# CaptainEven/DenseBox

Measured on AMD Instinct MI355X. Metric: training patches/sec (240x240), higher is better.
Workload: dtype f16; 1 GPU; full training step (fwd + fused dense loss w/ hard-negative mining + bwd + grad all-reduce + SGD) of DenseBoxLMLOC on 240x240 patches; net=DenseBoxLMLOC, batch_per_gpu=64, global_batch=64, patch=240x240, parallelism=dp1, half_neg=11, grad_finite=True

## Files before the change

densebox_amd/_lib.py:

```python
import ctypes as C
import os

_HERE = os.path.dirname(os.path.abspath(__file__))
LIB_PATH = os.environ.get('DBX_LIB') or os.path.join(_HERE, 'csrc', 'libdensebox_hip.so')

F16, BF16, F32 = 0, 1, 2
DTYPE_ID = {'f16': F16, 'bf16': BF16, 'f32': F32}
ESIZE = {F16: 2, BF16: 2, F32: 4}

EPI_BIAS, EPI_RELU, EPI_GATE, EPI_DROPMASK, EPI_ACCUM, EPI_F32_NCHW, EPI_DROPHASH = 1, 2, 4, 8, 16, 32, 64
CONV_WFRAG = 128
K_IGEMM, K_DMA, K_BAND, K_C64, K_C8, K_WS, K_P8 = 1, 2, 3, 4, 5, 6, 7


class View(C.Structure):
    _fields_ = [('ptr', C.c_void_p), ('n', C.c_int32), ('h', C.c_int32), ('w', C.c_int32),
                ('pad', C.c_int32), ('ld', C.c_int32), ('c_off', C.c_int32), ('c', C.c_int32)]


class ConvDesc(C.Structure):
    _fields_ = [('dtype', C.c_int32), ('kh', C.c_int32), ('kw', C.c_int32), ('cpad', C.c_int32),
                ('cin_pad', C.c_int32), ('cout_pad', C.c_int32), ('epilogue', C.c_int32), ('drop_seed', C.c_uint32)]


# ... 32 lines not shown

class Track(C.Structure):
    _fields_ = [('box', C.c_double * 4), ('vel', C.c_double * 4), ('score', C.c_double), ('best_score', C.c_double), ('id', C.c_int32),
                ('hits', C.c_int32), ('age', C.c_int32), ('first_frame', C.c_int32), ('last_frame', C.c_int32), ('best_frame', C.c_int32)]


class TrackRecord(C.Structure):
    _fields_ = [('stream', C.c_int32), ('reserved', C.c_int32), ('t', Track)]


class Shot(C.Structure):
    _fields_ = [('key', C.c_double), ('score', C.c_double), ('sharpness', C.c_int64), ('id', C.c_int32), ('frame', C.c_int32),
                ('shots', C.c_int32), ('reserved', C.c_int32)]


class ShotRecord(C.Structure):
    _fields_ = [('stream', C.c_int32), ('slot', C.c_int32), ('shot', Shot)]


class OverlayFrame(C.Structure):
    _fields_ = [('src', C.c_void_p), ('dst', C.c_void_p), ('h', C.c_int32), ('w', C.c_int32)]


class OverlayStyle(C.Structure):
    _fields_ = [('box_color', C.c_uint8 * 4), ('text_color', C.c_uint8 * 4), ('mark_color', C.c_uint8 * 4), ('thickness', C.c_int32),
                ('radius', C.c_int32), ('font_scale', C.c_int32), ('inset_scale', C.c_int32)]


class ResizeJob(C.Structure):
    _fields_ = [('src', C.c_void_p), ('sh', C.c_int32), ('sw', C.c_int32), ('cx0', C.c_int32), ('cy0', C.c_int32),
                ('cw', C.c_int32), ('ch', C.c_int32), ('pad_l', C.c_int32), ('pad_t', C.c_int32), ('pad_r', C.c_int32),
                ('pad_b', C.c_int32), ('pad_value', C.c_int32), ('dh', C.c_int32), ('dw', C.c_int32), ('dst_off', C.c_int64)]


class PatchJob(C.Structure):
    _fields_ = [('src', C.c_void_p), ('dst', C.c_void_p), ('scale_x', C.c_double), ('scale_y', C.c_double), ('row_bytes', C.c_int32),
                ('cx0', C.c_int32), ('cy0', C.c_int32), ('cw', C.c_int32), ('ch', C.c_int32), ('pad_l', C.c_int32), ('pad_t', C.c_int32),
                ('vw', C.c_int32), ('vh', C.c_int32), ('dh', C.c_int32), ('dw', C.c_int32), ('pad_value', C.c_int32),
                ('tiles_x', C.c_int32), ('frame', C.c_int32), ('kind', C.c_int32), ('reserved', C.c_int32)]


class PatchGeom(C.Structure):
    _fields_ = [('status', C.c_int32), ('x0', C.c_int32), ('y0', C.c_int32), ('x1', C.c_int32), ('y1', C.c_int32),
                ('labels', C.c_int32 * 12), ('reserved', C.c_int32)]


class PatchPlanIO(C.Structure):
    _fields_ = [(k, C.c_void_p) for k in (
        'frames', 'plates', 'plate0', 'cand', 'draws', 'state', 'jobs', 'labels', 'bbox', 'vertices', 'label', 'count', 'tally',
        'status', 'slot', 'cand_out', 'draws_out')]


class PatchAug(C.Structure):
    _fields_ = [('flags', C.c_int32), ('blur', C.c_int32), ('box_len', C.c_int32), ('sat', C.c_int32), ('contrast', C.c_int32),
                ('brightness', C.c_int32), ('curve', C.c_int32), ('noise_amp', C.c_int32), ('key_lo', C.c_int32), ('key_hi', C.c_int32),
                ('gain', C.c_int32 * 3), ('reserved', C.c_int32 * 3)]


class PatchAugCfg(C.Structure):
    _fields_ = [('p_flip', C.c_double), ('p_blur', C.c_double), ('p_curve', C.c_double), ('p_noise', C.c_double), ('kind_w', C.c_int32 * 3),
                ('box_lo', C.c_int32), ('box_hi', C.c_int32), ('sat_lo', C.c_int32), ('sat_hi', C.c_int32), ('contrast_lo', C.c_int32),
                ('contrast_hi', C.c_int32), ('brightness_lo', C.c_int32), ('brightness_hi', C.c_int32), ('gain_lo', C.c_int32),
                ('gain_hi', C.c_int32), ('noise_lo', C.c_int32), ('noise_hi', C.c_int32), ('curve_lo', C.c_int32), ('curve_hi', C.c_int32),
                ('G', C.c_int32), ('reserved', C.c_int32 * 2)]


class PatchAugIO(C.Structure):
    _fields_ = [(k, C.c_void_p) for k in ('labels_in', 'count', 'params_in', 'state', 'params', 'labels', 'bbox', 'vertices', 'label')]


class MergeXform(C.Structure):
    _fields_ = [('scale', C.c_double), ('off_x', C.c_double), ('off_y', C.c_double)]


_VP, _I32, _I64, _F, _D = C.c_void_p, C.c_int32, C.c_int64, C.c_float, C.c_double
_PV, _PC = C.POINTER(View), C.POINTER(ConvDesc)

SIGNATURES = {
    'dbx_last_error': (C.c_char_p, []),
    'dbx_version': (C.c_int, []),
    'dbx_device_arch': (C.c_int, [C.c_int]),
    'dbx_conv_packed_elems': (_I64, [_PC]),
    'dbx_conv_forward': (C.c_int, [_PC, _PV, _VP, _VP, _PV, _PV, _VP, _I32, _VP]),
    'dbx_conv_plan': (C.c_int, [_PC, _PV, _PV, C.POINTER(ConvPlan)]),
    'dbx_conv_forward_split': (C.c_int, [_PC, _PV, _VP, _VP, _PV, _PV, _PV, _PV, _I32, _I32, _VP]),
    'dbx_heads_forward_fusable': (C.c_int, [_PC, _PV, _PV, C.POINTER(C.c_int32), _I32]),
    'dbx_heads_forward_fused_scratch_bytes': (_I64, [_I32, _I64]),
    'dbx_heads_forward_fused': (C.c_int, [_PC, _PV, _VP, _VP, _PV, _VP, _VP, C.POINTER(C.c_int32), _I32, _VP, _VP, _VP]),
    'dbx_heads_forward_fused_heads': (C.c_int, [_PC, _PV, _VP, _VP, _PV, _VP, _VP, C.POINTER(C.c_int32), _I32, C.POINTER(C.c_void_p), _VP, _VP]),
    'dbx_dp_unique_id': (C.c_int, [_VP]),
    'dbx_dp_init': (C.c_int, [_VP, _I32, _I32, C.POINTER(C.c_void_p)]),
    'dbx_dp_allreduce_sum_f32': (C.c_int, [_VP, _VP, _I64, _VP]),
    'dbx_dp_destroy': (C.c_int, [_VP]),
    'dbx_conv_dgrad_wgrad1_scratch_bytes': (_I64, []),
    'dbx_conv_dgrad_wgrad1_fusable': (C.c_int, [_PC, _PV, _PV, _PV]),
    'dbx_conv_dgrad_wgrad1': (C.c_int, [_PC, _PV, _VP, _PV, _PV, _I32, _VP, _VP, _VP, _I32, _VP]),
    'dbx_conv_pool_fusable': (C.c_int, [_PC, _PV, _PV]),
    'dbx_conv_forward_pool': (C.c_int, [_PC, _PV, _VP, _VP, _PV, _PV, _I32, _VP]),
    'dbx_conv_forward_pool_idx': (C.c_int, [_PC, _PV, _VP, _VP, _PV, _PV, _I32, _VP, _VP]),
    'dbx_pack_weight': (C.c_int, [_I32, _I32, _VP, _I32, _I32, _I32, _I32, _VP, _I32, _I32, _I32, _I32, _VP]),
    'dbx_fold_heads': (C.c_int, [_VP, _VP, _VP, _VP, _I32, _VP, _VP, _VP]),
    'dbx_fold_refine': (C.c_int, [_VP, _VP, _VP, _VP, _VP, _VP, _I32, _I32, _VP, _VP, _VP, _VP]),
    'dbx_refine_eval': (C.c_int, [_VP, _VP, _I32, _I32, _I32, _VP, _VP, _VP, _VP]),
    'dbx_refine_backward_scratch_bytes': (C.c_int64, [_I32, _I32, _I32]),
    'dbx_refine_backward': (C.c_int, [_VP, _VP, _VP, _I32, _I32, _I32, _VP, _VP, _VP, _VP, _VP, _VP, _I32, _VP, _VP, _VP, _VP, _VP, _VP, _VP, _VP, _VP, _VP, _VP, _VP, _VP, _VP]),
    'dbx_upsample_bilinear_nchw_f32': (C.c_int, [_VP, _I32, _I32, _I32, _VP, _I32, _I32, _VP]),
    'dbx_pack_multi': (C.c_int, [_I32, _VP, _I32, _I64, _VP]),
    'dbx_sgd_pack_step': (C.c_int, [_I32, _VP, _I32, _I64, _VP, _F, _F, _F, _I32, _VP]),
    'dbx_head2_dgrad': (C.c_int, [_I32, _PV, C.POINTER(C.c_void_p), C.POINTER(C.c_int32), _I32, _PV, _VP, _I32, _I32, C.c_uint32, _VP]),
    'dbx_head2_wgrad_scratch_bytes': (_I64, [_I32, _I32]),
    'dbx_head2_wgrad': (C.c_int, [_I32, _PV, _PV, C.POINTER(C.c_int32), _I32, C.POINTER(C.c_void_p), C.POINTER(C.c_void_p), _VP, _VP]),
    'dbx_head2_backward': (C.c_int, [_I32, _PV, _PV, C.POINTER(C.c_void_p), C.POINTER(C.c_int32), _I32, _PV, _VP, _I32, _I32, C.c_uint32,
                                     C.POINTER(C.c_void_p), C.POINTER(C.c_void_p), _VP, _VP]),
    'dbx_head2_backward_up': (C.c_int, [_I32, _PV, _PV, C.POINTER(C.c_void_p), C.POINTER(C.c_int32), _I32, _PV, _VP, _I32, _I32, C.c_uint32,
                                        C.POINTER(C.c_void_p), C.POINTER(C.c_void_p), _VP, _PV, _VP]),
    'dbx_perspective_matrix': (C.c_int, [_VP, _VP, _VP]),
    'dbx_warp_perspective_u8': (C.c_int, [_VP, _I32, _I32, _I32, _VP, _VP, _I32, _I32, _VP]),
    'dbx_warp_batch_workspace_bytes': (_I64, [_I32]),
    'dbx_warp_perspective_batch_u8': (C.c_int, [C.POINTER(WarpJob), _I32, _I32, _VP, _VP, _VP]),
    'dbx_plate_crops_batch': (C.c_int, [_VP, _I32, _I32, _VP, _I64, _I64, _VP, _I32, _I32, _I32, _VP, _VP, _VP, _VP]),
    'dbx_match_gt_batch': (C.c_int, [_VP, _I32, _I64, _VP, _VP, _I32, _I32, _VP, _I32, _VP, _VP, _I32, _D, _VP, _VP, _VP, _VP, _VP, _VP]),
    'dbx_eval_append': (C.c_int, [_VP, _I32, _I64, _VP, _VP, _I32, _I32, _VP, _VP, _VP, _VP, _I64, _VP, _VP]),
    'dbx_track_update_batch': (C.c_int, [_VP, _I32, _I64, _VP, _VP, _I32, _I32, _VP, _VP, _I32, _I32, _I32, _D, _I32, _D, _D, _D, _VP, _VP, _VP,
                                         _VP, _VP, _VP]),
    'dbx_track_append': (C.c_int, [_VP, _VP, _I32, _I32, _I32, _VP, _I64, _VP, _VP]),
    'dbx_crop_sharpness': (C.c_int, [_VP, _I64, _I32, _I32, _I32, _VP, _VP]),
    'dbx_track_gallery_update': (C.c_int, [_VP, _VP, _VP, _VP, _VP, _VP, _VP, _VP, _VP, _VP, _VP, _VP, _VP, _I32, _I32, _I32, _I32, _I32, _I32,
                                           _I32, _I32, _I64, _I32, _D, _I32, _VP]),
    'dbx_draw_overlay_batch': (C.c_int, [_VP, _I32, _I32, _I32, _I32, _VP, _I32, _I64, _VP, _VP, _I32, _VP, _VP, _VP, _I32, _I32,
                                         C.POINTER(OverlayStyle), _VP]),
    'dbx_overlay_font': (C.c_int, [_VP]),
    'dbx_overlay_label': (C.c_int, [_D, _I32, C.c_char_p, _I32]),
    'dbx_resize_batch_workspace_bytes': (_I64, [_I32]),
    'dbx_resize_cubic_batch_u8': (C.c_int, [C.POINTER(ResizeJob), _I32, _I32, _VP, _VP, _VP]),
    'dbx_patch_plan': (C.c_int, [C.POINTER(PatchPlanIO), _I32, _I32, _I32, _I32, _I32, _D, _D, _I32, _VP]),
    'dbx_patch_cut': (C.c_int, [_VP, _VP, _I32, _I32, _VP, _VP]),
    'dbx_patch_plan_host': (C.c_int, [_I32, _I32, _I32, _VP, _I32, _D, _D, _D, _I32, C.POINTER(PatchGeom)]),
    'dbx_patch_draw': (C.c_int, [_I64, _I64, _I32, _I32, _VP]),
    'dbx_patch_check_tables': (C.c_int, [_VP, _I32, _VP, _I32, _VP, _I32]),
    'dbx_patch_aug_plan': (C.c_int, [C.POINTER(PatchAugIO), C.POINTER(PatchAugCfg), _I32, _VP]),
    'dbx_patch_augment': (C.c_int, [_VP, _VP, _VP, _VP, _I32, _I32, _I32, _VP, _VP]),
    'dbx_patch_aug_params_host': (C.c_int, [C.POINTER(PatchAugCfg), _I64, _I64, _VP, _VP, _I32, _VP, _VP, _VP, _VP, _VP]),
    'dbx_patch_augment_host': (C.c_int, [_VP, _VP, _VP, _I32, _I32, _VP]),
    'dbx_conv_wgrad_scratch_bytes': (_I64, [_I32, _PV, _PV, _I32, _I32]),
    'dbx_conv_wgrad': (C.c_int, [_I32, _PV, _PV, _I32, _I32, _I32, _I32, _I32, _VP, _VP, _VP, _I32, _VP]),
    'dbx_conv_wgrad_slice': (C.c_int, [_I32, _PV, _PV, _I32, _I32, _I32, _I32, _I32, _VP, _I32, _I32, _VP, _VP, _I32, _VP]),
    'dbx_conv_wgrad_pool_dz_ok': (C.c_int, [_I32, _PV, _PV, _I32, _I32]),
    'dbx_conv_wgrad_pool_dz': (C.c_int, [_I32, _PV, _VP, _I32, _PV, _PV, _I32, _I32, _I32, _I32, _I32, _VP, _VP, _VP, _I32, _I32, _VP]),
    'dbx_head2_backward_up_fused': (C.c_int, [_I32, _PV, _PV]),
    'dbx_heads1_wgrad_gen_ok': (C.c_int, [_I32, _PV, _I32]),
    'dbx_heads1_dgrad_gen': (C.c_int, [_I32, _PV, C.POINTER(C.c_void_p), C.POINTER(C.c_int32), _I32, _I32, C.c_uint32, _VP, _PV, _PV, _VP]),
    'dbx_heads1_wgrad_gen': (C.c_int, [_I32, _PV, _PV, C.POINTER(C.c_void_p), C.POINTER(C.c_int32), _I32, _I32, C.c_uint32, _I32, _VP, _I32, _I32,
                             _VP, _VP, _VP]),
    'dbx_conv_wgrad_plan': (C.c_int, [_I32, _PV, _PV, _I32, _I32, C.c_char_p, _I32, C.POINTER(C.c_int32)]),
    'dbx_nchw_to_framed': (C.c_int, [_I32, _VP, _I32, _PV, _VP]),
    'dbx_u8hwc_to_framed': (C.c_int, [_I32, _VP, _PV, C.POINTER(C.c_float), C.POINTER(C.c_float), _VP]),
    'dbx_nchw_to_framed_ch': (C.c_int, [_I32, _VP, _I32, _PV, _I32, _VP]),
    'dbx_nchw_to_framed_slots': (C.c_int, [_I32, _VP, _VP, _I32, _I32, _PV, _VP]),
    'dbx_framed_to_nchw_f32': (C.c_int, [_I32, _PV, _VP, _VP]),
    'dbx_framed_add_ch': (C.c_int, [_I32, _PV, _I32, _I32, _PV, _I32, _VP]),
    'dbx_maxpool2x2': (C.c_int, [_I32, _PV, _PV, _VP]),
    'dbx_maxpool2x2_bwd': (C.c_int, [_I32, _PV, _PV, _PV, _I32, _I32, _VP]),
    'dbx_maxpool_idx_bytes': (C.c_int64, [_I32, _I32, _I32, _I32]),
    'dbx_maxpool2x2_idx': (C.c_int, [_I32, _PV, _PV, _VP, _VP]),
    'dbx_maxpool2x2_bwd_idx': (C.c_int, [_I32, _VP, _PV, _PV, _I32, _I32, _VP]),
    'dbx_upsample_bilinear': (C.c_int, [_I32, _PV, _PV, _VP]),
    'dbx_upsample_bilinear_bwd': (C.c_int, [_I32, _PV, _PV, _PV, _VP]),
    'dbx_loss_scratch_bytes': (C.c_int64, [_I32]),
    'dbx_loss_forward_backward': (C.c_int, [C.POINTER(LossDesc), C.POINTER(LossIO), _VP, _VP]),
    'dbx_count_positives': (C.c_int, [_VP, _VP, _I32, _VP, _VP]),
    'dbx_init_score_map': (C.c_int, [_VP, _VP, _I32, _VP, _VP]),
    'dbx_init_offset_map': (C.c_int, [_VP, _VP, _I32, _I32, _VP, _VP]),
    'dbx_init_lm_heatmap': (C.c_int, [_VP, _VP, _I32, _I32, _VP, _VP]),
    'dbx_mask_by_sel': (C.c_int, [_VP, _I32, _VP, _I64, _VP, _I32, _VP]),
    'dbx_mask_gray_zone_cls': (C.c_int, [_VP, _VP, _VP, _I32, _VP]),
    'dbx_mask_gray_zone_lm': (C.c_int, [_VP, _I32, _VP, _I64, _VP]),
    'dbx_sgd_step': (C.c_int, [_VP, _VP, _I32, _I64, _F, _F, _F, _I32, _VP]),
    'dbx_grad_guard': (C.c_int, [_VP, _I64, _VP, _I32, _VP]),
    'dbx_sgd_step_guarded': (C.c_int, [_VP, _VP, _I32, _I64, _F, _F, _F, _I32, _VP, _I32, _VP]),
    'dbx_sgd_pack_step_guarded': (C.c_int, [_I32, _VP, _I32, _I64, _VP, _F, _F, _F, _I32, _VP, _I32, _VP]),
    'dbx_detect_scratch_bytes': (_I64, [_I32, _I32, _I32]),
    'dbx_detect': (C.c_int, [_VP, _VP, _VP, _VP, _I32, _I32, _I32, _D, _VP, _I32, _VP, _VP, _VP, _VP]),
    'dbx_detect_batch_scratch_bytes': (_I64, [_I32, _I32, _I32, _I32]),
    'dbx_detect_batch': (C.c_int, [_VP, _VP, _VP, _VP, _I32, _I32, _I32, _I32, _D, _VP, _I32, _VP, _VP, _VP, _VP]),
    'dbx_nms': (C.c_int, [_VP, _I32, _I32, _D, _VP, _VP, _VP]),
    'dbx_detect_thresh_batch_scratch_bytes': (_I64, [_I32, _I32, _I32, _I32]),
    'dbx_detect_thresh_batch': (C.c_int, [_VP, _VP, _VP, _VP, _I32, _I32, _I32, _F, _I32, _D, _VP, _I32, _VP, _VP, _VP, _VP, _VP]),
    'dbx_thresh_rows_batch_scratch_bytes': (_I64, [_I32, _I32, _I32, _I32]),
    'dbx_thresh_rows_batch': (C.c_int, [_VP, _VP, _VP, _VP, _I32, _I32, _I32, _F, _I32, _VP, _I32, _VP, _VP, _VP, _VP]),
    'dbx_nms_large_scratch_bytes': (_I64, [_I32]),
    'dbx_nms_large': (C.c_int, [_VP, _I32, _I32, _D, _VP, _VP, _VP]),
    'dbx_merge_nms_batch_workspace_bytes': (_I64, [_I32, _I32, _I32]),
    'dbx_merge_nms_batch': (C.c_int, [C.POINTER(C.c_void_p), C.POINTER(MergeXform), _I32, _I32, _I32, _I32, _D, _VP, _VP, _VP, _VP]),
    'dbx_merge_nms_thresh_batch_workspace_bytes': (_I64, [_I32, _I32, _I32]),
    'dbx_merge_nms_thresh_batch': (C.c_int, [C.POINTER(C.c_void_p), C.POINTER(C.c_void_p), C.POINTER(MergeXform), _I32, _I32, _I32, _I32, _D,
                                             _VP, _VP, _VP, _VP, _VP]),
}

ABI_VERSION = 13
_lib = None
MISSING = []


def lib():
    global _lib
    if _lib is None:
        if not os.path.exists(LIB_PATH):
            raise RuntimeError('libdensebox_hip.so is not built (%s). Run `python -c "import __graft_entry__ as g; '
                               'g.build()"`; densebox_amd has no fallback path.' % LIB_PATH)
        L = C.CDLL(LIB_PATH)
        for name, (res, args) in SIGNATURES.items():
            try:
                fn = getattr(L, name)
            except AttributeError:
                MISSING.append(name)
                continue
            fn.restype = res
            fn.argtypes = args
        if 'dbx_version' not in MISSING and L.dbx_version() != ABI_VERSION:
            raise RuntimeError('libdensebox_hip.so at %s has ABI version %d, this binding needs %d (struct layouts / scratch '
                               'contracts differ): rebuild it' % (LIB_PATH, L.dbx_version(), ABI_VERSION))
        _lib = L
    return _lib


def check(rc):
    if rc != 0:
        raise RuntimeError('libdensebox_hip: %s (status %d)' % (lib().dbx_last_error().decode(), rc))


def ptr(t):
    return C.c_void_p(t.data_ptr()) if t is not None else None


def stream_ptr():
    import torch
    return C.c_void_p(torch.cuda.current_stream().cuda_stream)
```

densebox_amd/csrc/aux_ops.hip:

```cpp
#include "common.hpp"
#include <mutex>

static thread_local char g_err[512] = "";
void dbx_set_error(const char* fmt, ...) {
    va_list ap;
    va_start(ap, fmt);
    vsnprintf(g_err, sizeof(g_err), fmt, ap);
    va_end(ap);
}
extern "C" const char* dbx_last_error(void) { return g_err; }
extern "C" int dbx_version(void) { return DBX_ABI_VERSION; }
extern "C" int dbx_device_arch(int device) {
    hipDeviceProp_t p;
    if (hipGetDeviceProperties(&p, device) != hipSuccess) { dbx_set_error("hipGetDeviceProperties failed"); return DBX_ERR_HIP; }
    int arch = 0;
    const char* s = p.gcnArchName;
    if (s[0] == 'g' && s[1] == 'f' && s[2] == 'x') arch = (int)strtol(s + 3, nullptr, 16) == 0x950 ? 950 : (int)strtol(s + 3, nullptr, 10);
    return arch;
}

template <typename T> struct Vec { static constexpr int N = 16 / sizeof(T); };

template <typename T> __device__ __forceinline__ void load_vec(const T* p, float (&v)[16 / sizeof(T)]) {
    const u32x4 raw = *(const u32x4*)p;
    const T* e = (const T*)&raw;
#pragma unroll
    for (int i = 0; i < 16 / (int)sizeof(T); ++i) v[i] = to_f32(e[i]);
}
template <typename T> __device__ __forceinline__ void store_vec(T* p, const float (&v)[16 / sizeof(T)]) {
    u32x4 raw;
    T* e = (T*)&raw;
#pragma unroll
    for (int i = 0; i < 16 / (int)sizeof(T); ++i) e[i] = from_f32<T>(v[i]);
    *(u32x4*)p = raw;
}

static inline int grid_for(int64_t work, int block = 256) {
    int64_t b = (work + block - 1) / block;
    return (int)(b < 1 ? 1 : (b > 8192 ? 8192 : b));
}

#define VIEW_VEC_CHECK(T, v, name)                                                                             \
    DBX_REQUIRE(((size_t)(v)->ptr % 16) == 0 && ((v)->ld * sizeof(T)) % 16 == 0 && ((v)->c_off * sizeof(T)) % 16 == 0 && \
                    ((v)->c * sizeof(T)) % 16 == 0, name ": view must be 16-byte aligned/strided")

template <typename T>
__global__ void nchw_to_framed_kernel(const float* __restrict__ x, int csrc, FrameGeo y) {
    constexpr int V = Vec<T>::N;
    const int cg = y.c / V;
    const int64_t total = (int64_t)y.n * y.h * y.w * cg;
    for (int64_t i = blockIdx.x * (int64_t)blockDim.x + threadIdx.x; i < total; i += (int64_t)gridDim.x * blockDim.x) {
        const int px = (int)(i % y.w);
        const int g = (int)((i / y.w) % cg);
        const int py = (int)((i / ((int64_t)y.w * cg)) % y.h);
        const int n = (int)(i / ((int64_t)y.w * cg * y.h));
        float v[V];
#pragma unroll
        for (int j = 0; j < V; ++j) {
            const int c = g * V + j;
            v[j] = c < csrc ? x[(((int64_t)n * csrc + c) * y.h + py) * y.w + px] : 0.f;
        }
        store_vec<T>((T*)y.base + geo_pix(y, n, py, px) + g * V, v);
    }
}
template <typename T> static int nchw_to_framed_t(const float* x, int csrc, const dbx_view* y, hipStream_t s) {
    VIEW_VEC_CHECK(T, y, "nchw_to_framed");
    FrameGeo g = make_geo<T>(y);
    const int64_t total = (int64_t)y->n * y->h * y->w * (y->c / Vec<T>::N);
    hipLaunchKernelGGL(nchw_to_framed_kernel<T>, dim3(grid_for(total)), dim3(256), 0, s, x, csrc, g);
    DBX_LAUNCH_CHECK();
    return DBX_OK;
}
extern "C" int dbx_nchw_to_framed(int32_t dtype, const float* x_nchw, int32_t c_src, const dbx_view* y, void* stream) {
    DBX_DISPATCH_DTYPE(dtype, nchw_to_framed_t, x_nchw, c_src, y, (hipStream_t)stream);
}

struct SlotSrc { const float* x[4]; int k[4]; };
template <typename T>
__global__ void nchw_to_framed_slots_kernel(SlotSrc src, int nslots, int slot, FrameGeo y) {
    constexpr int V = Vec<T>::N;
    const int gps = slot / V, cg = nslots * gps;
    const int64_t total = (int64_t)y.n * y.h * y.w * cg;
    for (int64_t i = blockIdx.x * (int64_t)blockDim.x + threadIdx.x; i < total; i += (int64_t)gridDim.x * blockDim.x) {
        const int px = (int)(i % y.w);
        const int g = (int)((i / y.w) % cg);
        const int py = (int)((i / ((int64_t)y.w * cg)) % y.h);
        const int n = (int)(i / ((int64_t)y.w * cg * y.h));
        const int si = g / gps, c0 = (g % gps) * V;
        const float* x = si == 0 ? src.x[0] : si == 1 ? src.x[1] : si == 2 ? src.x[2] : src.x[3];
        const int k = si == 0 ? src.k[0] : si == 1 ? src.k[1] : si == 2 ? src.k[2] : src.k[3];
        float v[V];
#pragma unroll
        for (int j = 0; j < V; ++j) {
            const int c = c0 + j;
            v[j] = (x && c < k) ? x[(((int64_t)n * k + c) * y.h + py) * y.w + px] : 0.f;
        }
        store_vec<T>((T*)y.base + geo_pix(y, n, py, px) + si * slot + c0, v);
    }
}
template <typename T> static int nchw_to_framed_slots_t(const float* const* xs, const int32_t* ks, int nslots, int slot, const dbx_view* y, hipStream_t s) {
    VIEW_VEC_CHECK(T, y, "nchw_to_framed_slots");
    DBX_REQUIRE(nslots >= 1 && nslots <= 4 && slot % Vec<T>::N == 0 && y->c == nslots * slot, "nchw_to_framed_slots: 1..4 slots of a multiple of the vector width, view of nslots * slot channels");
    SlotSrc src;
    for (int i = 0; i < 4; ++i) {
        src.x[i] = i < nslots ? xs[i] : nullptr; src.k[i] = i < nslots ? ks[i] : 0;
        if (i < nslots) DBX_REQUIRE(ks[i] >= 0 && ks[i] <= slot, "nchw_to_framed_slots: k must fit its slot");
    }
    FrameGeo g = make_geo<T>(y);
    const int64_t total = (int64_t)y->n * y->h * y->w * (y->c / Vec<T>::N);
    hipLaunchKernelGGL(nchw_to_framed_slots_kernel<T>, dim3(grid_for(total)), dim3(256), 0, s, src, nslots, slot, g);
    DBX_LAUNCH_CHECK();
    return DBX_OK;
}
extern "C" int dbx_nchw_to_framed_slots(int32_t dtype, const float* const* x_nchw, const int32_t* k, int32_t nslots, int32_t slot, const dbx_view* y,
                                        void* stream) {
    if (!x_nchw || !k || !y) { dbx_set_error("nchw_to_framed_slots: null argument"); return DBX_ERR_ARG; }
    DBX_DISPATCH_DTYPE(dtype, nchw_to_framed_slots_t, x_nchw, k, nslots, slot, y, (hipStream_t)stream);
}

template <typename T>
__global__ void framed_to_nchw_kernel(FrameGeo x, float* __restrict__ y) {
    const int64_t total = (int64_t)x.n * x.c * x.h * x.w;
    for (int64_t i = blockIdx.x * (int64_t)blockDim.x + threadIdx.x; i < total; i += (int64_t)gridDim.x * blockDim.x) {
        const int px = (int)(i % x.w);
        const int py = (int)((i / x.w) % x.h);
        const int c = (int)((i / ((int64_t)x.w * x.h)) % x.c);
        const int n = (int)(i / ((int64_t)x.w * x.h * x.c));
        y[i] = to_f32(((const T*)x.base)[geo_pix(x, n, py, px) + c]);
    }
}
template <typename T> static int framed_to_nchw_t(const dbx_view* x, float* y, hipStream_t s) {
    FrameGeo g = make_geo<T>(x);
    const int64_t total = (int64_t)x->n * x->c * x->h * x->w;
    hipLaunchKernelGGL(framed_to_nchw_kernel<T>, dim3(grid_for(total)), dim3(256), 0, s, g, y);
    DBX_LAUNCH_CHECK();
    return DBX_OK;
}
extern "C" int dbx_framed_to_nchw_f32(int32_t dtype, const dbx_view* x, float* y_nchw, void* stream) {
    DBX_DISPATCH_DTYPE(dtype, framed_to_nchw_t, x, y_nchw, (hipStream_t)stream);
}

template <typename T> struct IdxWord { typedef unsigned int type; };
template <> struct IdxWord<float> { typedef unsigned short type; };
template <typename T>
__global__ void maxpool_kernel(FrameGeo x, FrameGeo y, unsigned char* __restrict__ idx) {
    constexpr int V = Vec<T>::N;
    const int cg = y.c / V;
    const int64_t total = (int64_t)y.n * y.h * y.w * cg;
    for (int64_t i = blockIdx.x * (int64_t)blockDim.x + threadIdx.x; i < total; i += (int64_t)gridDim.x * blockDim.x) {
        const int g = (int)(i % cg);
        const int px = (int)((i / cg) % y.w);
        const int py = (int)((i / ((int64_t)cg * y.w)) % y.h);
        const int n = (int)(i / ((int64_t)cg * y.w * y.h));
// ... 30 lines not shown
    hipLaunchKernelGGL(maxpool_kernel<T>, dim3(grid_for(total)), dim3(256), 0, s, make_geo<T>(x), make_geo<T>(y), (unsigned char*)idx);
    DBX_LAUNCH_CHECK();
    return DBX_OK;
}
extern "C" int dbx_maxpool2x2(int32_t dtype, const dbx_view* x, const dbx_view* y, void* stream) {
    DBX_DISPATCH_DTYPE(dtype, maxpool_t, x, y, nullptr, (hipStream_t)stream);
}
extern "C" int64_t dbx_maxpool_idx_bytes(int32_t n, int32_t h, int32_t w, int32_t c) {
    return (int64_t)n * (h / 2) * (w / 2) * (c / 2);
}
extern "C" int dbx_maxpool2x2_idx(int32_t dtype, const dbx_view* x, const dbx_view* y, void* idx, void* stream) {
    if (!idx) { dbx_set_error("maxpool2x2_idx: null idx"); return DBX_ERR_ARG; }
    DBX_DISPATCH_DTYPE(dtype, maxpool_t, x, y, idx, (hipStream_t)stream);
}

template <typename T>
__global__ void maxpool_bwd_kernel(FrameGeo x, FrameGeo dy, FrameGeo dx, int ph, int pw, int accumulate, int relu_gate) {
    constexpr int V = Vec<T>::N;
    const int cg = x.c / V;
    const int wh = (x.h + 1) >> 1, ww = (x.w + 1) >> 1;
    const int64_t total = (int64_t)x.n * wh * ww * cg;
    for (int64_t i = blockIdx.x * (int64_t)blockDim.x + threadIdx.x; i < total; i += (int64_t)gridDim.x * blockDim.x) {
        const int g = (int)(i % cg);
        const int wx = (int)((i / cg) % ww);
        const int wy = (int)((i / ((int64_t)cg * ww)) % wh);
        const int n = (int)(i / ((int64_t)cg * ww * wh));
        const bool covered = wy < ph && wx < pw;
        const size_t p00 = geo_pix(x, n, 2 * wy, 2 * wx) + g * V;
        const size_t d00 = geo_pix(dx, n, 2 * wy, 2 * wx) + g * V;
        const bool has_x1 = 2 * wx + 1 < x.w, has_y1 = 2 * wy + 1 < x.h;
        float o[4][V];
#pragma unroll
        for (int k = 0; k < 4; ++k)
#pragma unroll
            for (int j = 0; j < V; ++j) o[k][j] = 0.f;
        if (covered) {
            float q[4][V], gd[V];
            const T* p = (const T*)x.base + p00;
            load_vec<T>(p, q[0]);
            load_vec<T>(p + x.ld, q[1]);
            load_vec<T>(p + (size_t)x.wp * x.ld, q[2]);
            load_vec<T>(p + (size_t)x.wp * x.ld + x.ld, q[3]);
            load_vec<T>((const T*)dy.base + geo_pix(dy, n, wy, wx) + g * V, gd);
#pragma unroll
            for (int j = 0; j < V; ++j) {
                int arg = 0;
                float m = q[0][j];
#pragma unroll
                for (int k = 1; k < 4; ++k)
                    if (q[k][j] > m) { m = q[k][j]; arg = k; }
                float v = gd[j];
                if (relu_gate && !(m > 0.f)) v = 0.f;
#pragma unroll
                for (int k = 0; k < 4; ++k) o[k][j] = (k == arg) ? v : 0.f;
            }
        }
#pragma unroll
        for (int k = 0; k < 4; ++k) {
            if ((k & 1) && !has_x1) continue;
            if ((k >> 1) && !has_y1) continue;
            T* dst = (T*)dx.base + d00 + (size_t)(k >> 1) * dx.wp * dx.ld + (size_t)(k & 1) * dx.ld;
            if (accumulate) {
                float old[V];
                load_vec<T>(dst, old);
#pragma unroll
                for (int j = 0; j < V; ++j) o[k][j] += old[j];
            }
            store_vec<T>(dst, o[k]);
        }
    }
}
template <typename T>
static int maxpool_bwd_t(const dbx_view* x, const dbx_view* dy, const dbx_view* dx, int accumulate, int relu_gate, hipStream_t s) {
    VIEW_VEC_CHECK(T, x, "maxpool_bwd x"); VIEW_VEC_CHECK(T, dy, "maxpool_bwd dy"); VIEW_VEC_CHECK(T, dx, "maxpool_bwd dx");
    DBX_REQUIRE(dy->h == x->h / 2 && dy->w == x->w / 2 && dx->h == x->h && dx->w == x->w && dx->c == x->c && dy->c == x->c,
                "maxpool_bwd: shape mismatch");
    const int64_t total = (int64_t)x->n * ((x->h + 1) / 2) * ((x->w + 1) / 2) * (x->c / Vec<T>::N);
    hipLaunchKernelGGL(maxpool_bwd_kernel<T>, dim3(grid_for(total)), dim3(256), 0, s, make_geo<T>(x), make_geo<T>(dy),
                       make_geo<T>(dx), dy->h, dy->w, accumulate, relu_gate);
    DBX_LAUNCH_CHECK();
    return DBX_OK;
}
extern "C" int dbx_maxpool2x2_bwd(int32_t dtype, const dbx_view* x, const dbx_view* dy, const dbx_view* dx,
                                  int32_t accumulate, int32_t relu_gate, void* stream) {
    DBX_DISPATCH_DTYPE(dtype, maxpool_bwd_t, x, dy, dx, accumulate, relu_gate, (hipStream_t)stream);
}

template <typename T>
__global__ void maxpool_bwd_idx_kernel(const unsigned char* __restrict__ idx, FrameGeo dy, FrameGeo dx, int accumulate, int relu_gate) {
    constexpr int V = Vec<T>::N;
    typedef typename IdxWord<T>::type W;
    const int cg = dx.c / V;
    const int ph = dy.h, pw = dy.w;
    const int wh = (dx.h + 1) >> 1, ww = (dx.w + 1) >> 1;
    const int64_t total = (int64_t)dx.n * wh * ww * cg;
    for (int64_t i = blockIdx.x * (int64_t)blockDim.x + threadIdx.x; i < total; i += (int64_t)gridDim.x * blockDim.x) {
        const int g = (int)(i % cg);
        const int wx = (int)((i / cg) % ww);
        const int wy = (int)((i / ((int64_t)cg * ww)) % wh);
        const int n = (int)(i / ((int64_t)cg * ww * wh));
        const bool covered = wy < ph && wx < pw;
        const size_t d00 = geo_pix(dx, n, 2 * wy, 2 * wx) + g * V;
        const bool has_x1 = 2 * wx + 1 < dx.w, has_y1 = 2 * wy + 1 < dx.h;
        float o[4][V];
#pragma unroll
        for (int k = 0; k < 4; ++k)
#pragma unroll
            for (int j = 0; j < V; ++j) o[k][j] = 0.f;
        if (covered) {
            float gd[V];
            load_vec<T>((const T*)dy.base + geo_pix(dy, n, wy, wx) + g * V, gd);
            const unsigned int word = *(const W*)(idx + ((((size_t)n * ph + wy) * pw + wx) * (size_t)(dx.c / 2)) + g * (V / 2));
#pragma unroll
            for (int j = 0; j < V; ++j) {
                const unsigned int nib = (word >> (4 * j)) & 15u;
                const int arg = (int)(nib & 3u);
                const float v = (relu_gate && !(nib & 4u)) ? 0.f : gd[j];
#pragma unroll
                for (int k = 0; k < 4; ++k) o[k][j] = (k == arg) ? v : 0.f;
            }
        }
#pragma unroll
        for (int k = 0; k < 4; ++k) {
            if ((k & 1) && !has_x1) continue;
            if ((k >> 1) && !has_y1) continue;
            T* dst = (T*)dx.base + d00 + (size_t)(k >> 1) * dx.wp * dx.ld + (size_t)(k & 1) * dx.ld;
            if (accumulate) {
                float old[V];
                load_vec<T>(dst, old);
#pragma unroll
                for (int j = 0; j < V; ++j) o[k][j] += old[j];
            }
            store_vec<T>(dst, o[k]);
        }
    }
}
template <typename T>
static int maxpool_bwd_idx_t(const void* idx, const dbx_view* dy, const dbx_view* dx, int accumulate, int relu_gate, hipStream_t s) {
    VIEW_VEC_CHECK(T, dy, "maxpool_bwd_idx dy"); VIEW_VEC_CHECK(T, dx, "maxpool_bwd_idx dx");
    DBX_REQUIRE(dy->h == dx->h / 2 && dy->w == dx->w / 2 && dy->c == dx->c && dy->n == dx->n, "maxpool_bwd_idx: shape mismatch");
    DBX_REQUIRE(((size_t)idx % 4) == 0, "maxpool_bwd_idx: idx must be 4-byte aligned");
    const int64_t total = (int64_t)dx->n * ((dx->h + 1) / 2) * ((dx->w + 1) / 2) * (dx->c / Vec<T>::N);
    hipLaunchKernelGGL(maxpool_bwd_idx_kernel<T>, dim3(grid_for(total)), dim3(256), 0, s, (const unsigned char*)idx, make_geo<T>(dy),
                       make_geo<T>(dx), accumulate, relu_gate);
    DBX_LAUNCH_CHECK();
    return DBX_OK;
}
extern "C" int dbx_maxpool2x2_bwd_idx(int32_t dtype, const void* idx, const dbx_view* dy, const dbx_view* dx,
                                      int32_t accumulate, int32_t relu_gate, void* stream) {
    if (!idx || !dy || !dx) { dbx_set_error("maxpool2x2_bwd_idx: null argument"); return DBX_ERR_ARG; }
    DBX_DISPATCH_DTYPE(dtype, maxpool_bwd_idx_t, idx, dy, dx, accumulate, relu_gate, (hipStream_t)stream);
}

__device__ __forceinline__ void bilin_coef(int d, float scale, int in, int& i0, int& i1, float& l0, float& l1) {
#pragma clang fp contract(off)
    const float src = scale * (float)d;
    i0 = (int)src;
    if (i0 > in - 1) i0 = in - 1;
    i1 = i0 + (i0 < in - 1 ? 1 : 0);
    l1 = src - (float)i0;
    l0 = 1.f - l1;
}
static inline float ac_scale(int in, int out) { return out > 1 ? (float)(in - 1) / (float)(out - 1) : 0.f; }

template <typename T>
__global__ void upsample_kernel(FrameGeo x, FrameGeo y, float sy, float sx) {
    constexpr int V = Vec<T>::N;
    const int cg = y.c / V;
    const int64_t total = (int64_t)y.n * y.h * y.w * cg;
    for (int64_t i = blockIdx.x * (int64_t)blockDim.x + threadIdx.x; i < total; i += (int64_t)gridDim.x * blockDim.x) {
        const int g = (int)(i % cg);
        const int px = (int)((i / cg) % y.w);
        const int py = (int)((i / ((int64_t)cg * y.w)) % y.h);
        const int n = (int)(i / ((int64_t)cg * y.w * y.h));
        int y0, y1, x0, x1;
        float ly0, ly1, lx0, lx1;
        bilin_coef(py, sy, x.h, y0, y1, ly0, ly1);
        bilin_coef(px, sx, x.w, x0, x1, lx0, lx1);
        float a[V], b[V], c[V], d[V], o[V];
        const T* base = (const T*)x.base + g * V;
        load_vec<T>(base + geo_pix(x, n, y0, x0), a);
        load_vec<T>(base + geo_pix(x, n, y0, x1), b);
        load_vec<T>(base + geo_pix(x, n, y1, x0), c);
        load_vec<T>(base + geo_pix(x, n, y1, x1), d);
#pragma unroll
        for (int j = 0; j < V; ++j) o[j] = ly0 * (lx0 * a[j] + lx1 * b[j]) + ly1 * (lx0 * c[j] + lx1 * d[j]);
        store_vec<T>((T*)y.base + geo_pix(y, n, py, px) + g * V, o);
    }
}
template <typename T>
__global__ __launch_bounds__(256) void upsample_rows_kernel(FrameGeo x, FrameGeo y, float sy, float sx) {
    constexpr int V = Vec<T>::N;
    const int cg = y.c / V;
    const int n = blockIdx.x / y.h, py = blockIdx.x - n * y.h;
    int y0, y1;
    float ly0, ly1;
    bilin_coef(py, sy, x.h, y0, y1, ly0, ly1);
    const T* r0 = (const T*)x.base + geo_pix(x, n, y0, 0);
    const T* r1 = (const T*)x.base + geo_pix(x, n, y1, 0);
    T* out = (T*)y.base + geo_pix(y, n, py, 0);
    const int xs = (int)(geo_pix(x, n, y0, 1) - geo_pix(x, n, y0, 0)), ys = (int)(geo_pix(y, n, py, 1) - geo_pix(y, n, py, 0));
    const int total = y.w * cg;
    constexpr int U = 4;
    for (int e0 = threadIdx.x; e0 < total; e0 += 256 * U) {
        float a[U][V], b[U][V], c[U][V], d[U][V], lx0[U], lx1[U];
        int px[U], g[U];
#pragma unroll
        for (int u = 0; u < U; ++u) {
            const int e = e0 + 256 * u < total ? e0 + 256 * u : total - 1;
            px[u] = e / cg; g[u] = e - px[u] * cg;
            int x0, x1;
            bilin_coef(px[u], sx, x.w, x0, x1, lx0[u], lx1[u]);
            load_vec<T>(r0 + (size_t)x0 * xs + g[u] * V, a[u]);
            load_vec<T>(r0 + (size_t)x1 * xs + g[u] * V, b[u]);
            load_vec<T>(r1 + (size_t)x0 * xs + g[u] * V, c[u]);
            load_vec<T>(r1 + (size_t)x1 * xs + g[u] * V, d[u]);
        }
#pragma unroll
        for (int u = 0; u < U; ++u) {
            float o[V];
#pragma unroll
            for (int j = 0; j < V; ++j) o[j] = ly0 * (lx0[u] * a[u][j] + lx1[u] * b[u][j]) + ly1 * (lx0[u] * c[u][j] + lx1[u] * d[u][j]);
            if (e0 + 256 * u < total) store_vec<T>(out + (size_t)px[u] * ys + g[u] * V, o);
        }
    }
}
template <typename T> static int upsample_t(const dbx_view* x, const dbx_view* y, hipStream_t s) {
    VIEW_VEC_CHECK(T, x, "upsample x"); VIEW_VEC_CHECK(T, y, "upsample y");
    DBX_REQUIRE(x->c == y->c && x->n == y->n, "upsample: channel/batch mismatch");
    hipLaunchKernelGGL(upsample_rows_kernel<T>, dim3(y->n * y->h), dim3(256), 0, s, make_geo<T>(x), make_geo<T>(y),
                       ac_scale(x->h, y->h), ac_scale(x->w, y->w));
    DBX_LAUNCH_CHECK();
    return DBX_OK;
}
extern "C" int dbx_upsample_bilinear(int32_t dtype, const dbx_view* x, const dbx_view* y, void* stream) {
    DBX_DISPATCH_DTYPE(dtype, upsample_t, x, y, (hipStream_t)stream);
}

template <typename T>
__global__ void upsample_bwd_kernel(FrameGeo dy, FrameGeo dx, FrameGeo gate, int has_gate, float sy, float sx) {
    constexpr int V = Vec<T>::N;
    const int cg = dx.c / V;
    const int64_t total = (int64_t)dx.n * dx.h * dx.w * cg;
    for (int64_t i = blockIdx.x * (int64_t)blockDim.x + threadIdx.x; i < total; i += (int64_t)gridDim.x * blockDim.x) {
        const int g = (int)(i % cg);
        const int ix = (int)((i / cg) % dx.w);
        const int iy = (int)((i / ((int64_t)cg * dx.w)) % dx.h);
        const int n = (int)(i / ((int64_t)cg * dx.w * dx.h));
        float acc[V];
#pragma unroll
        for (int j = 0; j < V; ++j) acc[j] = 0.f;
        int oy_lo = sy > 0.f ? (int)floorf((float)(iy - 1) / sy) : 0;
        int oy_hi = sy > 0.f ? (int)ceilf((float)(iy + 1) / sy) : dy.h - 1;
        int ox_lo = sx > 0.f ? (int)floorf((float)(ix - 1) / sx) : 0;
        int ox_hi = sx > 0.f ? (int)ceilf((float)(ix + 1) / sx) : dy.w - 1;
        oy_lo = max(oy_lo, 0); ox_lo = max(ox_lo, 0);
        oy_hi = min(oy_hi, dy.h - 1); ox_hi = min(ox_hi, dy.w - 1);
        for (int oy = oy_lo; oy <= oy_hi; ++oy) {
            int y0, y1; float ly0, ly1;
            bilin_coef(oy, sy, dx.h, y0, y1, ly0, ly1);
            const float wy = (y0 == iy ? ly0 : 0.f) + (y1 == iy ? ly1 : 0.f);
            if (wy == 0.f) continue;
            for (int ox = ox_lo; ox <= ox_hi; ++ox) {
                int x0, x1; float lx0, lx1;
                bilin_coef(ox, sx, dx.w, x0, x1, lx0, lx1);
                const float wx = (x0 == ix ? lx0 : 0.f) + (x1 == ix ? lx1 : 0.f);
                if (wx == 0.f) continue;
                float d[V];
                load_vec<T>((const T*)dy.base + geo_pix(dy, n, oy, ox) + g * V, d);
#pragma unroll
                for (int j = 0; j < V; ++j) acc[j] += wy * wx * d[j];
            }
        }
        if (has_gate) {
            float gt[V];
            load_vec<T>((const T*)gate.base + geo_pix(gate, n, iy, ix) + g * V, gt);
#pragma unroll
            for (int j = 0; j < V; ++j) acc[j] = gt[j] > 0.f ? acc[j] : 0.f;
        }
        store_vec<T>((T*)dx.base + geo_pix(dx, n, iy, ix) + g * V, acc);
    }
}
template <typename T>
__global__ __launch_bounds__(256) void upsample_bwd_rows_kernel(FrameGeo dy, FrameGeo dx, FrameGeo gate, int has_gate, float sy, float sx) {
    constexpr int V = Vec<T>::N, WIN = 8, MAXR = 16;
    extern __shared__ __attribute__((aligned(16))) char up_smem[];
    int* s_ox0 = (int*)up_smem;
    float* s_wx = (float*)(s_ox0 + dx.w);
    __shared__ int s_oy[MAXR];
    __shared__ float s_wy[MAXR];
    __shared__ int s_ny;
    const int cg = dx.c / V;
    const int n = blockIdx.x / dx.h, iy = blockIdx.x - n * dx.h;
    if (threadIdx.x == 0) {
        int lo = sy > 0.f ? (int)floorf((float)(iy - 1) / sy) : 0, hi = sy > 0.f ? (int)ceilf((float)(iy + 1) / sy) : dy.h - 1;
        lo = max(lo, 0); hi = min(hi, dy.h - 1);
        int cnt = 0;
        for (int oy = lo; oy <= hi && cnt < MAXR; ++oy) {
            int y0, y1; float ly0, ly1;
            bilin_coef(oy, sy, dx.h, y0, y1, ly0, ly1);
            const float wy = (y0 == iy ? ly0 : 0.f) + (y1 == iy ? ly1 : 0.f);
            if (wy != 0.f) { s_oy[cnt] = oy; s_wy[cnt] = wy; ++cnt; }
        }
        s_ny = cnt;
    }
    for (int ix = threadIdx.x; ix < dx.w; ix += 256) {
        int lo = sx > 0.f ? (int)floorf((float)(ix - 1) / sx) : 0, hi = sx > 0.f ? (int)ceilf((float)(ix + 1) / sx) : dy.w - 1;
        lo = max(lo, 0); hi = min(hi, dy.w - 1);
        int first = -1;
        float w[WIN];
#pragma unroll
        for (int k = 0; k < WIN; ++k) w[k] = 0.f;
        for (int ox = lo; ox <= hi; ++ox) {
            int x0, x1; float lx0, lx1;
            bilin_coef(ox, sx, dx.w, x0, x1, lx0, lx1);
            const float wx = (x0 == ix ? lx0 : 0.f) + (x1 == ix ? lx1 : 0.f);
// ... 701 lines not shown
    int cur = 0, oy = 0;
    for (int r0 = 0; r0 < R; r0 += D) {
#pragma unroll
        for (int d = 0; d < D; ++d) {
            const int r = r0 + d;
            float gj[KJ], h[V];
            {
                const T* ge = (const T*)&graw[d];
                const T* he = (const T*)&hraw[d];
#pragma unroll
                for (int j = 0; j < KJ; ++j) gj[j] = to_f32(ge[j]);
#pragma unroll
                for (int i = 0; i < V; ++i) h[i] = to_f32(he[i]);
            }
            fetch(d);
            if (r < R) {
                int y0, y1; float ly0, ly1;
                bilin_coef(oy, sy, dg.h, y0, y1, ly0, ly1);
                while (y0 > cur) {
                    finalize(cur, va);
#pragma unroll
                    for (int i = 0; i < V / 2; ++i) { va[i] = vb[i]; vb[i] = (f32x2){0.f, 0.f}; }
                    ++cur;
                }
                const float wa = (y0 == cur ? ly0 : 0.f) + (y1 == cur ? ly1 : 0.f);
                const float wb = (y0 == cur + 1 ? ly0 : 0.f) + (y1 == cur + 1 ? ly1 : 0.f);
                {
                    f32x2 o2[V / 2];
#pragma unroll
                    for (int i = 0; i < V / 2; ++i) o2[i] = (f32x2){0.f, 0.f};
#pragma unroll
                    for (int j = 0; j < KJ; ++j) {
                        bs[j] += gj[j];
                        const f32x2 g2 = {gj[j], gj[j]};
#pragma unroll
                        for (int i = 0; i < V / 2; ++i) acc[j][i] = g2 * (f32x2){h[2 * i], h[2 * i + 1]} + acc[j][i];
#pragma unroll
                        for (int i = 0; i < V / 2; ++i) o2[i] = g2 * w2[j][i] + o2[i];
                    }
                    float o[V];
#pragma unroll
                    for (int i = 0; i < V / 2; ++i) { o[2 * i] = o2[i].x; o[2 * i + 1] = o2[i].y; }
                    const long long pc0 = ((long long)n * H + oy) * W;
                    if (mask) {
                        unsigned char mb[V];
                        *(u32x2*)mb = *(const u32x2*)(mask + (size_t)pc0 * mask_ld + lo_mask);
#pragma unroll
                        for (int i = 0; i < V; ++i) o[i] = mb[i] ? o[i] : 0.f;
                    } else if (use_hash) {
                        const unsigned kb8 = dbx_drop_hash32(drop_seed, (unsigned)pc0 + (unsigned)px, (unsigned)(hd * 512 + c0) >> 5) >> ((unsigned)c0 & 31u);
#pragma unroll
                        for (int i = 0; i < V; ++i)
                            o[i] = __builtin_bit_cast(float, __builtin_bit_cast(int, o[i]) & ((int)(kb8 << (31 - i)) >> 31));
                    }
                    u32x4 raw;
                    T* oe = (T*)&raw;
#pragma unroll
                    for (int i = 0; i < V; ++i) oe[i] = from_f32<T>(o[i]);
                    if (owner && !nostore) *(u32x4*)((T*)dhid.base + row_of(dhid, n, oy) + lo_dhid) = raw;
                    const f32x2 wa2 = {wa, wa}, wb2 = {wb, wb};
#pragma unroll
                    for (int i = 0; i < V / 2; ++i) {
                        const f32x2 dv = {to_f32(oe[2 * i]), to_f32(oe[2 * i + 1])};
                        va[i] = wa2 * dv + va[i]; vb[i] = wb2 * dv + vb[i];
                    }
                }
                if (++oy == H) {
                    finalize(cur, va);
                    if (cur + 1 < dg.h) finalize(cur + 1, vb);
                    if (pend) flush();
#pragma unroll
                    for (int i = 0; i < V / 2; ++i) va[i] = vb[i] = (f32x2){0.f, 0.f};
                    cur = 0; oy = 0; n += G;
                }
            }
        }
    }
    if (!owner) {
#pragma unroll
        for (int j = 0; j < KJ; ++j) {
            bs[j] = 0.f;
#pragma unroll
            for (int i = 0; i < V / 2; ++i) acc[j][i] = (f32x2){0.f, 0.f};
        }
    }
    const int lane = threadIdx.x & 63, wv = threadIdx.x >> 6;
#pragma unroll
    for (int j = 0; j < KJ; ++j) {
#pragma unroll
        for (int i = 0; i < V; ++i) {
            float a = acc[j][i >> 1][i & 1];
            a += __shfl_xor(a, 8); a += __shfl_xor(a, 16); a += __shfl_xor(a, 32);
            acc[j][i >> 1][i & 1] = a;
        }
        float bsum = bs[j];
        bsum += __shfl_xor(bsum, 8); bsum += __shfl_xor(bsum, 16); bsum += __shfl_xor(bsum, 32);
        bs[j] = bsum;
    }
    __syncthreads();
    float* red = s_v;
    if (lane < LPP) {
#pragma unroll
        for (int j = 0; j < KJ; ++j) {
            *(f32x4*)&red[(wv * 8 + j) * CS + lane * V] = (f32x4){acc[j][0][0], acc[j][0][1], acc[j][1][0], acc[j][1][1]};
            *(f32x4*)&red[(wv * 8 + j) * CS + lane * V + 4] = (f32x4){acc[j][2][0], acc[j][2][1], acc[j][3][0], acc[j][3][1]};
        }
#pragma unroll
        for (int j = KJ; j < 8; ++j) {
            *(f32x4*)&red[(wv * 8 + j) * CS + lane * V] = (f32x4){0.f, 0.f, 0.f, 0.f};
            *(f32x4*)&red[(wv * 8 + j) * CS + lane * V + 4] = (f32x4){0.f, 0.f, 0.f, 0.f};
        }
        if (lane == 0) {
#pragma unroll
            for (int j = 0; j < 8; ++j) red[4 * 8 * CS + wv * 8 + j] = j < KJ ? bs[j < KJ ? j : 0] : 0.f;
        }
    }
    __syncthreads();
    {
        const size_t blk = (size_t)grp * plan.halves + half;
        const int c = threadIdx.x % CS;
#pragma unroll
        for (int jj = 0; jj < 2; ++jj) {
            const int j = threadIdx.x / CS + 4 * jj;
            float o = 0.f;
#pragma unroll
            for (int q = 0; q < 4; ++q) o += red[(q * 8 + j) * CS + c];
            partial[(blk * nhl * 8 + (hd - hd0) * 8 + j) * 512 + cbase + c] = o;
        }
        if (cbase == 0 && threadIdx.x < 8) {
            float bsum = 0.f;
#pragma unroll
            for (int q = 0; q < 4; ++q) bsum += red[4 * 8 * CS + q * 8 + threadIdx.x];
            bpartial[blk * 32 + (hd - hd0) * 8 + threadIdx.x] = bsum;
        }
    }
}
static bool h2u_plan(int W, int ws, float sx, H2UPlan& p) {
    if (W > 64 || ws > 32 || W < 1 || ws < 1) return false;
    int x0[64];
    for (int ox = 0; ox < W; ++ox) { int v = (int)(sx * (float)ox); x0[ox] = v > ws - 1 ? ws - 1 : v; }
    if (W <= 32 && ws <= 16) { p.halves = 1; p.h[0] = p.h[1] = H2UHalf{0, W, 0, W, 0, ws}; return true; }
    const int S = ws / 2;
    if (S < 1 || S > 16 || ws - S > 16) return false;
    int hiL = -1, loR = W;
    for (int ox = 0; ox < W; ++ox) { if (x0[ox] <= S - 1) hiL = ox; if (x0[ox] >= S - 1 && ox < loR) loR = ox; }
    if (hiL + 1 > 32 || W - loR > 32 || loR > hiL + 1) return false;
    const int P = (loR + hiL + 1) / 2;
    p.halves = 2;
    p.h[0] = H2UHalf{0, hiL + 1, 0, P, 0, S};
    p.h[1] = H2UHalf{loR, W - loR, P, W, S, ws - S};
    return true;
}
template <typename T>
static int head2_backward_up_t(const dbx_view* dout, const dbx_view* hid, const float* const* w2, const int32_t* k, int nh, const dbx_view* dhid,
                               const uint8_t* mask, int mask_ld, int use_hash, unsigned drop_seed, float* const* dw, float* const* db,
                               void* scratch, const dbx_view* dg, hipStream_t s) {
    VIEW_VEC_CHECK(T, dg, "head2_backward_up d_g44");
    DBX_REQUIRE(dg->n == hid->n && dg->c == hid->c, "head2_backward_up: d_g44 has the hidden map's batch and channels");
    const float sy = ac_scale(dg->h, hid->h), sx = ac_scale(dg->w, hid->w);
    H2UPlan plan;
    bool fused = sizeof(T) == 2 && sy > 0.f && sy < 1.f && sx > 0.45f && sx < 1.f && hid->c % 64 == 0 && hid->h >= 2 && h2u_plan(hid->w, dg->w, sx, plan);
    if (const char* e = getenv("DBX_HEAD2_UP")) fused = fused && atoi(e) != 0;
    const bool nostore = dhid->ptr == nullptr;
    DBX_REQUIRE(!nostore || (fused && !mask), "head2_backward_up without d_hid: needs the one-pass kernel (dbx_head2_backward_up_fused) and hash / no dropout");
    if (!fused) {
        const int rc = head2_wgrad_t<T>(dout, hid, k, nh, dw, db, scratch, s, w2, dhid, mask, mask_ld, use_hash, drop_seed);
        return rc != DBX_OK ? rc : upsample_bwd_t<T>(dhid, dg, nullptr, s);
    }
    if constexpr (sizeof(T) == 2) {
        VIEW_VEC_CHECK(T, hid, "head2_backward_up hid");
        if (!nostore) VIEW_VEC_CHECK(T, dhid, "head2_backward_up d_hid");
        DBX_REQUIRE(nh >= 1 && nh <= 4 && hid->c == 512 * nh && dout->c % nh == 0 && dout->c / nh >= 8, "head2_backward_up: nh in 1..4, hid of 512*nh channels, d_out of nh slots >= 8 channels");
        DBX_REQUIRE(dout->n == hid->n && dout->h == hid->h && dout->w == hid->w && dhid->n == hid->n && dhid->h == hid->h && dhid->w == hid->w && dhid->c == hid->c,
                    "head2_backward_up: shape mismatch");
        DBX_REQUIRE(((size_t)dout->ptr % 16) == 0 && (dout->ld * sizeof(T)) % 16 == 0 && (dout->c_off * sizeof(T)) % 16 == 0 &&
                        ((dout->c / nh) * sizeof(T)) % 16 == 0, "head2_backward_up: d_out alignment");
        Head2Out o;
        Head2Args ha;
        ha.nh = nh; ha.slot = dout->c / nh;
        for (int i = 0; i < 4; ++i) {
            o.dw[i] = i < nh ? dw[i] : nullptr; o.db[i] = (i < nh && db) ? db[i] : nullptr; o.k[i] = i < nh ? k[i] : 0;
            ha.w2[i] = i < nh ? w2[i] : nullptr; ha.k[i] = i < nh ? k[i] : 0;
            if (i < nh) DBX_REQUIRE(k[i] >= 1 && k[i] <= 8 && dw[i] && w2[i] && ((size_t)w2[i] % 16) == 0, "head2_backward_up: k in 1..8, 16-byte aligned weights");
        }
        constexpr size_t smem = (size_t)2 * H2U_NB * 32 * 64 * 4;
        static_assert(smem >= (4 * 8 * 64 + 32) * 4 && 2 * smem + 4096 <= 160 * 1024, "LDS budget of two workgroups per CU");
        static DbxDevOnce attr_once; int attr_dev = 0;
        if (attr_once.pending(&attr_dev)) {
            DBX_HIP(hipFuncSetAttribute((const void*)head2_backward_up_kernel<T, 1>, hipFuncAttributeMaxDynamicSharedMemorySize, (int)smem));
            DBX_HIP(hipFuncSetAttribute((const void*)head2_backward_up_kernel<T, 2>, hipFuncAttributeMaxDynamicSharedMemorySize, (int)smem));
            DBX_HIP(hipFuncSetAttribute((const void*)head2_backward_up_kernel<T, 4>, hipFuncAttributeMaxDynamicSharedMemorySize, (int)smem));
            DBX_HIP(hipFuncSetAttribute((const void*)head2_backward_up_kernel<T, 8>, hipFuncAttributeMaxDynamicSharedMemorySize, (int)smem));
            attr_once.mark(attr_dev);
        }
        static int split = -1;
        if (split < 0) { const char* e = getenv("DBX_HEAD2_UP_SPLIT"); split = e ? atoi(e) : 1; }
        auto kup = [&](int kk) { return !split ? 8 : kk <= 1 ? 1 : kk <= 2 ? 2 : kk <= 4 ? 4 : 8; };
        float* const pbase = (float*)scratch;
        long long pused = 0;
        int blocks_max = 0;
        for (int h0 = 0; h0 < nh;) {
            int h1 = h0 + 1;
            while (h1 < nh && kup(k[h1]) == kup(k[h0])) ++h1;
            const int nhl = h1 - h0, nsl = nhl * 8, kj = kup(k[h0]);
            int groups = H2U_WGS / (nsl * plan.halves);
            groups = groups < 1 ? 1 : groups > hid->n ? hid->n : groups;
            const int blocks = groups * plan.halves;
            float* partial = pbase + pused;
            float* bpartial = partial + (size_t)blocks * nhl * 8 * 512;
            for (int i = h0; i < h1; ++i) { o.poff[i] = pused; o.boff[i] = pused + (long long)blocks * nhl * 8 * 512; o.nblk[i] = blocks; o.nhl[i] = nhl; o.hl[i] = i - h0; }
            pused += (long long)blocks * (nhl * 8 * 512 + 32);
            blocks_max = blocks > blocks_max ? blocks : blocks_max;
#define H2U_LAUNCH(KJ)                                                                                                              \
            hipLaunchKernelGGL((head2_backward_up_kernel<T, KJ>), dim3(blocks * nsl), dim3(256), smem, s, make_geo<T>(dout), make_geo<T>(hid),    \
                               make_geo<T>(nostore ? hid : dhid), make_geo<T>(dg), h0, nhl, dout->c / nh, ha, partial, bpartial, mask, mask_ld,    \
                               use_hash, drop_seed, sy, sx, plan, nostore ? 1 : 0)
            if (kj == 1) H2U_LAUNCH(1); else if (kj == 2) H2U_LAUNCH(2); else if (kj == 4) H2U_LAUNCH(4); else H2U_LAUNCH(8);
#undef H2U_LAUNCH
            DBX_LAUNCH_CHECK();
            h0 = h1;
        }
        for (int i = nh; i < 4; ++i) { o.poff[i] = 0; o.boff[i] = 0; o.nblk[i] = 0; o.nhl[i] = 1; o.hl[i] = 0; }
        float* partial = pbase; float* bpartial = pbase;
        const int blocks = blocks_max;
        const int total = nh * 8 * 512 + nh * 8;
        hipLaunchKernelGGL(head2_wgrad_reduce_kernel, dim3((total + 63) / 64), dim3(1024), 0, s, partial, bpartial, blocks, nh, o);
        DBX_LAUNCH_CHECK();
    }
    return DBX_OK;
}
template <typename T> static int head2_up_fused_t(const dbx_view* hid, const dbx_view* dg) {
    const float sy = ac_scale(dg->h, hid->h), sx = ac_scale(dg->w, hid->w);
    H2UPlan plan;
    bool fused = sizeof(T) == 2 && sy > 0.f && sy < 1.f && sx > 0.45f && sx < 1.f && hid->c % 64 == 0 && hid->h >= 2 && h2u_plan(hid->w, dg->w, sx, plan);
    if (const char* e = getenv("DBX_HEAD2_UP")) fused = fused && atoi(e) != 0;
    return fused ? 1 : 0;
}
extern "C" int dbx_head2_backward_up_fused(int32_t dtype, const dbx_view* hid, const dbx_view* d_g44) {
    if (!hid || !d_g44) return 0;
    switch (dtype) { case DBX_F16: return head2_up_fused_t<_Float16>(hid, d_g44); case DBX_BF16: return head2_up_fused_t<__bf16>(hid, d_g44); default: return 0; }
}
extern "C" int dbx_head2_backward_up(int32_t dtype, const dbx_view* d_out, const dbx_view* hid, const float* const* w2, const int32_t* k,
                                     int32_t nh, const dbx_view* d_hid, const uint8_t* dropmask, int32_t dropmask_ld, int32_t use_hash,
                                     uint32_t drop_seed, float* const* dw, float* const* db, void* scratch, const dbx_view* d_g44, void* stream) {
    if (!d_out || !hid || !w2 || !k || !d_hid || !dw || !scratch || !d_g44) { dbx_set_error("head2_backward_up: null argument"); return DBX_ERR_ARG; }
    DBX_DISPATCH_DTYPE(dtype, head2_backward_up_t, d_out, hid, w2, k, nh, d_hid, dropmask, dropmask_ld, use_hash, (unsigned)drop_seed, dw, db,
                       scratch, d_g44, (hipStream_t)stream);
}

struct PackJob { const float* src; void* dst; int co, ci, taps, mode; long long ktot; int cin_pad, row_off, k_off, rows_lim; };
template <typename T>
__global__ void pack_multi_kernel(const PackJob* __restrict__ jobs) {
    const PackJob j = jobs[blockIdx.y];
    const int total = j.co * j.ci * j.taps, taps = j.taps, ci = j.ci;
    T* wp = (T*)j.dst;
    const bool fwd = j.mode == 0 || j.mode == 4;
    const int rl = j.mode >= 4 ? (int)j.ktot : j.rows_lim;
    if (sizeof(T) == 2 && j.mode != 2 && (fwd ? ci : j.co) % 8 == 0 && (j.k_off & 7) == 0 && (j.cin_pad & 7) == 0 && taps <= 25) {
        __shared__ float tile[8][32 * 25];
        const int ot = (j.co + 7) / 8, ctn = (ci + 31) / 32, ntiles = ot * ctn, row_f = 32 * taps;
        for (int tl = blockIdx.x; tl < ntiles; tl += gridDim.x) {
            const int o0 = (tl / ctn) * 8, c0 = (tl % ctn) * 32;
            const int cw = min(32, ci - c0), ow = min(8, j.co - o0);
            __syncthreads();
            for (int e = threadIdx.x; e < 8 * row_f; e += blockDim.x) {
                const int r = e / row_f, f = e - r * row_f;
                tile[r][f] = (r < ow && f < cw * taps) ? j.src[((o0 + r) * ci + c0) * taps + f] : 0.f;
            }
            __syncthreads();
            const int nch = fwd ? 8 * taps * 4 : 32 * taps;
            for (int q = threadIdx.x; q < nch; q += blockDim.x) {
                int row, col, tap;
                float v[8];
                if (fwd) {
                    const int k8 = q & 3, t = (q >> 2) % taps, r = (q >> 2) / taps;
                    if (r >= ow || 8 * k8 >= cw) continue;
                    row = j.row_off + o0 + r; col = j.k_off + c0 + 8 * k8; tap = t;
#pragma unroll
                    for (int e = 0; e < 8; ++e) v[e] = tile[r][(8 * k8 + e) * taps + t];
                } else {
                    const int c = q % 32, t = q / 32;
                    if (c >= cw) continue;
                    row = j.row_off + c0 + c; col = j.k_off + o0; tap = taps - 1 - t;
#pragma unroll
                    for (int e = 0; e < 8; ++e) v[e] = tile[e][c * taps + t];
                }
                if (row < 0 || col < 0 || col + 8 > j.cin_pad || (rl > 0 && row >= rl)) continue;
                u32x4 raw;
                T* e8 = (T*)&raw;
#pragma unroll
                for (int e = 0; e < 8; ++e) e8[e] = from_f32<T>(v[e]);
                const long long di = j.mode >= 4 ? (long long)dbx_frag_index(row, tap, col, j.cin_pad, (int)j.ktot, taps)
                                                 : (long long)row * j.ktot + (long long)tap * j.cin_pad + col;
                *(u32x4*)(wp + di) = raw;
            }
        }
        return;
    }
    for (int i = blockIdx.x * blockDim.x + threadIdx.x; i < total; i += gridDim.x * blockDim.x) {
        const float v = j.src[i];
        if (j.mode == 2) { ((float*)j.dst)[j.row_off + i] = v; continue; }
        const int q = i / taps, t = i - q * taps;
        const int o = q / ci, c = q - o * ci;
        {
            const int row = j.row_off + (fwd ? o : c), col = j.k_off + (fwd ? c : o);
            if (row < 0 || col < 0 || col >= j.cin_pad || (rl > 0 && row >= rl)) continue;
        }
        if (j.mode == 0) wp[(long long)(j.row_off + o) * j.ktot + (long long)t * j.cin_pad + j.k_off + c] = from_f32<T>(v);
        else if (j.mode == 1) wp[(long long)(j.row_off + c) * j.ktot + (long long)(taps - 1 - t) * j.cin_pad + j.k_off + o] = from_f32<T>(v);
        else if (j.mode == 4) wp[dbx_frag_index(j.row_off + o, t, j.k_off + c, j.cin_pad, (int)j.ktot, taps)] = from_f32<T>(v);
        else wp[dbx_frag_index(j.row_off + c, taps - 1 - t, j.k_off + o, j.cin_pad, (int)j.ktot, taps)] = from_f32<T>(v);
    }
}
template <typename T> static int pack_multi_t(const void* jobs, int count, long long max_elems, hipStream_t s) {
    int bx = (int)((max_elems + 255) / 256);
    bx = bx < 1 ? 1 : (bx > 256 ? 256 : bx);
    hipLaunchKernelGGL(pack_multi_kernel<T>, dim3(bx, count), dim3(256), 0, s, (const PackJob*)jobs);
    DBX_LAUNCH_CHECK();
    return DBX_OK;
}
extern "C" int dbx_pack_multi(int32_t dtype, const void* jobs, int32_t count, int64_t max_elems, void* stream) {
    DBX_REQUIRE(jobs && count > 0, "pack_multi: empty job table");
    DBX_DISPATCH_DTYPE(dtype, pack_multi_t, jobs, count, (long long)max_elems, (hipStream_t)stream);
}

struct PackDst { void* dst; long long ktot; int mode, cin_pad, row_off, k_off, rows_lim, pad_; };
struct SgdPackJob { float* p; int pidx, co, ci, taps, ndst, tiled; PackDst d[4]; };
template <typename T>
__device__ __forceinline__ void pack_scatter_elem(const PackDst& d, int o, int c, int t, int i, int taps, float v) {
    if (d.mode == 2) { ((float*)d.dst)[d.row_off + i] = v; return; }
    const bool fwd = d.mode == 0 || d.mode == 4;
    const int rl = d.mode >= 4 ? (int)d.ktot : d.rows_lim;
    const int row = d.row_off + (fwd ? o : c), col = d.k_off + (fwd ? c : o), tap = fwd ? t : taps - 1 - t;
    if (row < 0 || col < 0 || col >= d.cin_pad || (rl > 0 && row >= rl)) return;
    T* wp = (T*)d.dst;
    if (d.mode >= 4) wp[dbx_frag_index(row, tap, col, d.cin_pad, (int)d.ktot, taps)] = from_f32<T>(v);
    else wp[(long long)row * d.ktot + (long long)tap * d.cin_pad + col] = from_f32<T>(v);
}
template <typename T>
__global__ __launch_bounds__(256) void sgd_pack_kernel(const SgdPackJob* __restrict__ jobs, float* const* __restrict__ ptrs, float lr, float mu,
                                                       float wd, int first, int* __restrict__ guard, int step_id) {
    if (guard && guard[0] == step_id) {
        if (blockIdx.x == 0 && blockIdx.y == 0 && threadIdx.x == 0) atomicAdd(guard + 1, 1);
        return;
    }
    const SgdPackJob& j = jobs[blockIdx.y];
    float* p = j.p;
    const int pidx = j.pidx, taps = j.taps, ci = j.ci, co = j.co, ndst = j.ndst;
    const float* g = pidx >= 0 ? ptrs[3 * pidx + 1] : nullptr;
    float* b = pidx >= 0 ? ptrs[3 * pidx + 2] : nullptr;
    const int total = co * ci * taps;
    if (j.tiled && sizeof(T) == 2) {
        __shared__ float tile[8][32 * 25];
        const int CW = taps == 1 ? 256 : 32, nk8 = CW / 8;
        const int ot = (co + 7) / 8, ctn = (ci + CW - 1) / CW, ntiles = ot * ctn, row_f = CW * taps;
        constexpr int U = 3;
        for (int tl = blockIdx.x; tl < ntiles; tl += gridDim.x) {
            const int o0 = (tl / ctn) * 8, c0 = (tl % ctn) * CW;
            const int cw = min(CW, ci - c0), ow = min(8, co - o0);
            __syncthreads();
            int r = 0, f = threadIdx.x;
            while (f >= row_f) { f -= row_f; ++r; }
            for (int e = threadIdx.x; e < 8 * row_f; e += U * 256) {
                float pv[U], gv[U], bv[U];
                int ii[U], rr[U], ff[U];
#pragma unroll
                for (int u = 0; u < U; ++u) {
                    rr[u] = r; ff[u] = f;
                    const bool ok = r < ow && f < cw * taps;
                    ii[u] = ok ? ((o0 + r) * ci + c0) * taps + f : -1;
                    pv[u] = ok ? p[ii[u]] : 0.f;
                    if (g && ok) { gv[u] = g[ii[u]]; bv[u] = first ? 0.f : b[ii[u]]; }
                    f += 256;
                    while (f >= row_f) { f -= row_f; ++r; }
                }
#pragma unroll
                for (int u = 0; u < U; ++u) {
                    if (g && ii[u] >= 0) {
                        float bb = bv[u];
                        pv[u] = dbx_sgd_update(pv[u], gv[u], &bb, lr, mu, wd, first);
                        b[ii[u]] = bb; p[ii[u]] = pv[u];
                    }
                    if (rr[u] < 8) tile[rr[u]][ff[u]] = pv[u];
                }
            }
            __syncthreads();
            for (int di = 0; di < ndst; ++di) {
                const PackDst& d = j.d[di];
                T* wp = (T*)d.dst;
                const bool fwd = d.mode == 0 || d.mode == 4;
                const int rl = d.mode >= 4 ? (int)d.ktot : d.rows_lim;
                const int nch = fwd ? 8 * taps * nk8 : CW * taps;
                for (int q = threadIdx.x; q < nch; q += blockDim.x) {
                    int row, col, tap;
                    float v[8];
                    if (fwd) {
                        const int k8 = q % nk8, q2 = q / nk8, t = q2 % taps, r2 = q2 / taps;
                        if (r2 >= ow || 8 * k8 >= cw) continue;
                        row = d.row_off + o0 + r2; col = d.k_off + c0 + 8 * k8; tap = t;
#pragma unroll
// ... 240 lines not shown
```

densebox_amd/dist.py:

```python
import contextlib
import json
import os
import sys
import threading
from datetime import timedelta

import torch
import torch.distributed as dist


def rendezvous_timeout_s():
    return float(os.environ.get('DBX_DIST_RENDEZVOUS_S', '120'))


def dist_timeout_s():
    return float(os.environ.get('DBX_DIST_TIMEOUT_S', '1800'))


def rccl_info():
    env = {k: v for k, v in os.environ.items()
           if k.startswith(('NCCL_', 'RCCL_', 'HSA_ENABLE_IPC', 'MASTER_', 'DBX_DIST_')) or k in ('RANK', 'WORLD_SIZE', 'LOCAL_RANK')}
    info = {'backend': dist.get_backend() if dist.is_initialized() else None,
            'world': dist.get_world_size() if dist.is_initialized() else int(os.environ.get('WORLD_SIZE', '1')),
            'timeout_s': dist_timeout_s(), 'rendezvous_timeout_s': rendezvous_timeout_s(), 'env': env,
# ... 15 lines not shown
        os._exit(3)
    t = threading.Timer(seconds, expire)
    t.daemon = True
    t.start()
    try:
        yield
    finally:
        t.cancel()


def preflight(dev):
    if not dist.is_initialized() or dist.get_world_size() == 1:
        return
    world, rank = dist.get_world_size(), dist.get_rank()
    with watchdog(rendezvous_timeout_s(), 'first all-reduce (%s, world %d)' % (dist.get_backend(), world), rank):
        t = torch.full((1024,), float(rank + 1), device=dev if dist.get_backend() == 'nccl' else 'cpu')
        dist.all_reduce(t)
        if t.is_cuda:
            torch.cuda.synchronize()
        want = world * (world + 1) / 2.0
        if float(t[0]) != want or float(t[-1]) != want:
            raise RuntimeError('first all-reduce returned %r, expected %r' % (float(t[0]), want))


def init_from_env(backend=None):
    world = int(os.environ.get('WORLD_SIZE', '1'))
    rank = int(os.environ.get('RANK', '0'))
    local = int(os.environ.get('LOCAL_RANK', '0'))
    if world > 1 and not dist.is_initialized():
        os.environ.setdefault('MASTER_ADDR', '127.0.0.1')
        os.environ.setdefault('MASTER_PORT', '29500')
        if backend is None:
            backend = os.environ.get('DBX_DIST_BACKEND') or ('nccl' if torch.cuda.is_available() else 'gloo')
        if torch.cuda.is_available():
            torch.cuda.set_device(local % torch.cuda.device_count())
        dist.init_process_group(backend=backend, rank=rank, world_size=world, timeout=timedelta(seconds=rendezvous_timeout_s()))
        try:
            from torch.distributed.distributed_c10d import _set_pg_timeout
            _set_pg_timeout(timedelta(seconds=dist_timeout_s()))
        except Exception as e:
            print('densebox_amd.dist: collectives keep the rendezvous timeout of %.0f s (%s)' % (rendezvous_timeout_s(), e), file=sys.stderr)
    return rank, world, local


class GradReducer:

    def __init__(self, named_params, order, bucket_bytes=8 << 20, group=None, always_reduce=False):
        self.group = group
        self.world = dist.get_world_size(group) if dist.is_initialized() else 1
        self.collective = self.world > 1 or (always_reduce and dist.is_initialized())
        named = dict(named_params)
        self.order = [n for n in order if n in named]
        dev = next(iter(named.values())).device
        total = sum(named[n].numel() for n in self.order)
        self.flat = torch.zeros(total, dtype=torch.float32, device=dev)
        self.views, self.range = {}, {}
        off = 0
        for n in self.order:
            p = named[n]
            self.views[n] = self.flat[off:off + p.numel()].view_as(p)
            self.range[n] = (off, off + p.numel())
            off += p.numel()
        self.bucket_elems = max(1, bucket_bytes // 4)
        self._ready_hi = 0
        self._sent_hi = 0
        self._works = []

    def grad_view(self, name):
        return self.views[name]

    def region(self, names):
        lo, hi = self.range[names[0]][0], self.range[names[-1]][1]
        assert hi - lo == sum(self.range[n][1] - self.range[n][0] for n in names), 'parameters are not adjacent'
        return self.flat[lo:hi]

    in_step = False

    def begin(self):
        self._ready_hi = self._sent_hi = 0
        self._works = []

    def ready(self, names):
        if not self.in_step:
            return
        for n in names:
            self._ready_hi = max(self._ready_hi, self.range[n][1])
        if self.collective and self._ready_hi - self._sent_hi >= self.bucket_elems:
            self._send(self._ready_hi)

    def _send(self, hi):
        if hi > self._sent_hi:
            self._works.append(dist.all_reduce(self.flat[self._sent_hi:hi], op=dist.ReduceOp.SUM, group=self.group,
                                               async_op=True))
            self._sent_hi = hi

    def finish(self):
        if self.collective:
            self._send(self.flat.numel())
            for w in self._works:
                w.wait()
        self._works = []


class DataParallel:

    def __init__(self, net, optimizer, bucket_bytes=8 << 20, always_reduce=False):
        self.net, self.opt = net, optimizer
        self.world = dist.get_world_size() if dist.is_initialized() else 1
        self.rank = dist.get_rank() if dist.is_initialized() else 0
        self.ctl = None
        self.collective = self.world > 1 or (always_reduce and dist.is_initialized())
        if self.collective:
            for p in net.parameters():
                dist.broadcast(p.data, src=0)
            self.ctl = dist.new_group(backend='gloo', timeout=timedelta(seconds=dist_timeout_s())) if dist.get_backend() != 'gloo' \
                else dist.group.WORLD
        eng = net.engine()
        self.reducer = GradReducer(net.named_parameters(), eng.grad_order(), bucket_bytes, always_reduce=always_reduce)
        eng.grad_sink = self.reducer
        self._pf = None
        self.guard_f16 = os.environ.get('DBX_F16_GUARD', '1') != '0' and hasattr(optimizer, 'enable_guard')

    def close(self):
        eng = self.net.engine()
        if eng.grad_sink is self.reducer:
            eng.grad_sink = None

    def prefetch_positive_num(self, bbox, labels=None):
        from . import labels as LB
        if self._pf is not None:
            self._consume_prefetch()
        p = int(LB.positive_count(bbox, labels).sum())
        if self.collective:
            t = torch.tensor([p], dtype=torch.int64)
            self._pf = (p, t, dist.all_reduce(t, op=dist.ReduceOp.SUM, group=self.ctl, async_op=True))
        else:
            self._pf = (p, None, None)

    def drain_prefetch(self):
        if self._pf is not None:
            self._consume_prefetch()

    def _consume_prefetch(self):
        p, t, w = self._pf
        self._pf = None
        if w is not None:
            w.wait()
            return p, int(t.item())
        return p, p

    def global_positive_num(self, bbox, labels=None):
        from . import labels as LB
        p = int(LB.positive_count(bbox, labels).sum())
        if self._pf is not None:
            local, total = self._consume_prefetch()
            if local != p:
                raise RuntimeError('prefetch_positive_num() was given another batch than this step (local positives %d != %d)' % (local, p))
            return total
        if self.collective:
            t = torch.tensor([p], dtype=torch.int64)
            dist.all_reduce(t, op=dist.ReduceOp.SUM, group=self.ctl)
            p = int(t.item())
        return p

    def skipped_steps(self):
        return self.opt.skipped_steps() if hasattr(self.opt, 'skipped_steps') else 0

    def _stage(self, dev, items):
        import numpy as np
        host = []
        for t, dt in items:
            if t is None or (torch.is_tensor(t) and t.is_cuda):
                host.append(None)
            else:
                host.append(torch.as_tensor(np.ascontiguousarray(t) if isinstance(t, np.ndarray) else t).to(dt).contiguous())
        nbytes = sum((h.numel() * h.element_size() + 15) // 16 * 16 for h in host if h is not None)
        if nbytes == 0:
            return [t for t, _ in items]
        st = self.__dict__.get('_stage_buf')
        if st is None or st[0].numel() < nbytes:
            st = (torch.empty(2 * nbytes, dtype=torch.uint8).pin_memory(), torch.empty(2 * nbytes, dtype=torch.uint8, device=dev),
                  torch.cuda.Event())
            self._stage_buf = st
        pin, dbuf, ev = st
        ev.synchronize()
        out, off = [], 0
        for (t, dt), h in zip(items, host):
            if h is None:
                out.append(t); continue
            nb = h.numel() * h.element_size()
            pin[off:off + nb].view(dt).view(h.shape).copy_(h)
            out.append(dbuf[off:off + nb].view(dt).view(h.shape))
            off += (nb + 15) // 16 * 16
        dbuf[:off].copy_(pin[:off], non_blocking=True)
        ev.record()
        return out

    def step(self, x, bbox, vertices=None, labels=None, rand_neg_indices=None, lm_rand_neg_indices=None,
             positive_num_global=None, **loss_kw):
        net = self.net
        n_global = x.size(0) * self.world
        if positive_num_global is None:
            positive_num_global = self.global_positive_num(bbox, labels if net.KIND == 'DenseBoxLMLOC' else None)
        if x.is_cuda:
            import numpy as np
            from . import labels as LB
            n = x.size(0)
            rs = loss_kw.get('rng') or np.random
            _, half = LB.neg_counts(int(positive_num_global), n_global)
            if rand_neg_indices is None:
                rand_neg_indices = np.stack([rs.choice(3600, half, replace=False) for _ in range(n)]) if half else \
                    np.zeros((n, 0), np.int64)
            if net.KIND != 'DenseBox' and lm_rand_neg_indices is None:
                lm_rand_neg_indices = np.stack([np.stack([rs.choice(3600, 1, replace=False) for _ in range(n)])
                                                for _ in range(4)])
            bbox, vertices, labels, rand_neg_indices, lm_rand_neg_indices = self._stage(
                x.device, [(bbox, torch.float32), (vertices, torch.float32), (labels, torch.float32),
                           (rand_neg_indices, torch.int64), (lm_rand_neg_indices, torch.int64)])
        if self.guard_f16:
            self.opt.enable_guard(self.reducer.flat, on=net.resolved_dtype(True) == 'f16')
        self.opt.zero_grad(set_to_none=True)
        self.reducer.begin()
        net.engine().sample_offset = self.rank * x.size(0)
        self.reducer.in_step = True
        try:
            outs = net(x)
            loss = net.loss(outs, bbox, vertices, labels, rand_neg_indices, lm_rand_neg_indices,
                            batch_global=n_global, positive_num_global=positive_num_global, **loss_kw)
            direct = getattr(loss, '_dbx_direct', None)
            if direct is not None and all(t.requires_grad for t in direct[0]):
                torch.autograd.backward(direct[0], direct[1])
            else:
                loss.backward()
        finally:
            self.reducer.in_step = False
        self.reducer.finish()
        for name, p in net.named_parameters():
            p.grad = self.reducer.views.get(name)
        self.opt.step()
        return loss
```

densebox_amd/engine.py:

```python
import ctypes as C
import os
import weakref

import torch

from . import _lib
from ._lib import View, ConvDesc, check, ptr, stream_ptr

_BACKBONE = [('conv1_1_1', 3, 64), ('conv1_2_1', 64, 64), ('conv2_1_1', 64, 128), ('conv2_2_1', 128, 128),
             ('conv3_1_1', 128, 256), ('conv3_2_1', 256, 256), ('conv3_4_1', 256, 256),
             ('conv4_1_1', 256, 512), ('conv4_2_1', 512, 512), ('conv4_3_1', 512, 512), ('conv4_4_1', 512, 512)]

_HEADS = {
    'DenseBox': [('det', 1), ('loc', 4)],
    'DenseBoxLM': [('det', 1), ('loc', 4), ('landmark', 4)],
    'DenseBoxLMLOC': [('det', 1), ('loc', 4), ('landmark', 4), ('lmloc', 8)],
}


_FWD_IO = {'conv1_1_1': ('x0', 'a11'), 'conv1_2_1': ('a11', 'a12'), 'conv2_1_1': ('p1', 'a21'), 'conv2_2_1': ('a21', 'a22'),
           'conv3_1_1': ('p2', 'a31'), 'conv3_2_1': ('a31', 'a32'), 'conv3_4_1': ('a32', 'c34'), 'conv4_1_1': ('p3', 'a41'),
           'conv4_2_1': ('a41', 'a42'), 'conv4_3_1': ('a42', 'a43'), 'conv4_4_1': ('a43', 'a44')}
_BWD_IO = {'conv4_4_1': ('d_a44', 'd_a43'), 'conv4_3_1': ('d_a43', 'd_a42'), 'conv4_2_1': ('d_a42', 'd_a41'),
           'conv4_1_1': ('d_a41', 'd_p3'), 'conv3_4_1': ('d_c34', 'd_a32'), 'conv3_2_1': ('d_a32', 'd_a31'),
           'conv3_1_1': ('d_a31', 'd_p2'), 'conv2_2_1': ('d_a22', 'd_a21'), 'conv2_1_1': ('d_a21', 'd_p1'),
           'conv1_2_1': ('d_a12', 'd_a11')}
_CH = {s: (ci, co) for s, ci, co in [('conv1_1_1', 3, 64), ('conv1_2_1', 64, 64), ('conv2_1_1', 64, 128), ('conv2_2_1', 128, 128),
                                     ('conv3_1_1', 128, 256), ('conv3_2_1', 256, 256), ('conv3_4_1', 256, 256),
                                     ('conv4_1_1', 256, 512), ('conv4_2_1', 512, 512), ('conv4_3_1', 512, 512),
                                     ('conv4_4_1', 512, 512)]}


def _align(x, a=256):
    return (x + a - 1) // a * a


class Buf:

    def __init__(self, name, n, h, w, c, pad, dtype_id):
        self.name, self.n, self.h, self.w, self.c, self.pad = name, n, h, w, c, pad
        self.dtype_id = dtype_id
        self.es = _lib.ESIZE[dtype_id]
        self.hp, self.wp = h + 2 * pad, w + 2 * pad
        self.bytes = n * self.hp * self.wp * c * self.es
        self.guard = _align(max(4 * (self.wp + 2), 576 + 4 * self.wp) * c * self.es)
        self.base = None

    def view(self, c_off=0, c=None):
        return View(C.c_void_p(self.base), self.n, self.h, self.w, self.pad, self.c, c_off,
                    self.c - c_off if c is None else c)


class Plan:

    @staticmethod
    def env_flags():
        return tuple(os.environ.get(k, '1') != '0' for k in ('DBX_LIN_BWD', 'DBX_REFINE_LINEAR', 'DBX_POOL_IDX', 'DBX_HEADS_GEN')) + \
            (os.environ.get('DBX_F32_LIN', '0') == '1',)

    def __init__(self, kind, n, h, w, dtype_id, device, train):
        self.kind, self.n, self.h, self.w, self.dtype_id, self.train = kind, n, h, w, dtype_id, train
        self.flags = Plan.env_flags()
        lin_bwd, lin_refine, use_idx, heads_gen, f32_lin = self.flags
        lin_bwd = lin_bwd and (dtype_id != _lib.F32 or f32_lin)
        es = _lib.ESIZE[dtype_id]
        self.cin0 = 16 // es
        self.rdt = dtype_id
        self.crf = 8 if _lib.ESIZE[self.rdt] == 2 else 32
        nh = len(_HEADS[kind])
        h2, w2, h4, w4, h8, w8 = h // 2, w // 2, h // 4, w // 4, h // 8, w // 8
        self.h4, self.w4 = h4, w4
        B = {}

        def add(name, hh, ww, c, pad=1, dt=None):
            B[name] = Buf(name, n, hh, ww, c, pad, dtype_id if dt is None else dt)
        add('x0', h, w, self.cin0)
        self.a12_alias = es == 2 and h % 2 == 0 and w % 2 == 0 and (not train or use_idx)
        add('a11', h, w, 64)
        if not self.a12_alias:
            add('a12', h, w, 64)
        add('p1', h2, w2, 64)
        add('a21', h2, w2, 128); add('a22', h2, w2, 128); add('p2', h4, w4, 128)
        add('a31', h4, w4, 256); add('a32', h4, w4, 256)
        add('fusion', h4, w4, 768)
        add('p3', h8, w8, 256)
        add('a41', h8, w8, 512); add('a42', h8, w8, 512); add('a43', h8, w8, 512); add('a44', h8, w8, 512)
        add('hid', h4, w4, 512 * nh, pad=0)
        rf_convs = kind != 'DenseBox' and train and not lin_refine
        if rf_convs:
            add('rf_in', h4, w4, self.crf, pad=0, dt=self.rdt)
            add('rf_p', h8, w8, self.crf, pad=1, dt=self.rdt)
            add('rf_1', h8 - 2, w8 - 2, 64, pad=2, dt=self.rdt)
            add('rf_2', h8 - 6, w8 - 6, 64, pad=0, dt=self.rdt)
            add('rf_u', h4, w4, 64, pad=0, dt=self.rdt)
        if train:
            for nm in ('a11', 'a21', 'a22', 'a31', 'a32', 'a41', 'a42', 'a43', 'a44'):
                add('d_' + nm, B[nm].h, B[nm].w, B[nm].c)
            add('d_a12', h, w, 64)
            add('d_c34', h4, w4, 256)
            if not lin_bwd:
                add('d_ups', h4, w4, 512, pad=0)
            add('d_p1', h2, w2, 64, pad=0); add('d_p2', h4, w4, 128, pad=0); add('d_p3', h8, w8, 256, pad=0)
            add('d_g44', h8, w8, 512 * nh, pad=1)
            add('d_out', h4, w4, self.crf * nh, pad=0)
            L = _lib.lib()
            gen_fits = n * h4 * w4 < (1 << 24) and n * h4 * w4 * self.crf * nh * es < (1 << 31) and self.crf <= 8
            if dtype_id == _lib.F32:
                self.heads_gen = bool(heads_gen and lin_bwd)
            else:
                self.heads_gen = bool(heads_gen and lin_bwd and gen_fits and
                                      L.dbx_head2_backward_up_fused(dtype_id, C.byref(B['hid'].view()), C.byref(B['d_g44'].view())) and
                                      L.dbx_heads1_wgrad_gen_ok(dtype_id, C.byref(B['fusion'].view(512, 256)), nh))
            if not self.heads_gen or dtype_id == _lib.F32:
                add('d_hid', h4, w4, 512 * nh, pad=1)
            if rf_convs:
                add('d_rfo', h4, w4, self.crf, pad=0)
                add('d_rf_u', h4, w4, 64, pad=0)
                add('d_rf_2', h8 - 6, w8 - 6, 64, pad=4)
                add('d_rf_1', h8 - 2, w8 - 2, 64, pad=2)
                add('d_rf_p', h8, w8, self.crf, pad=0)
                add('d_rf_in', h4, w4, self.crf, pad=0)
        off = 0
        for b in B.values():
            off += b.guard
            b.off = off
            off += _align(b.bytes) + b.guard
        self.total = off
        if not train:
            self.heads_gen = False
        self.drop_active = self.drop_hash = False
        self.frag = {}
        self.drop_seed = 0
        self.mask_buf = None
        self.ws = torch.zeros(off, dtype=torch.uint8, device=device)
        self.pool_idx = None
        if train and os.environ.get('DBX_POOL_IDX', '1') != '0':
            self.pool_idx = {k: torch.empty(n * (hh // 2) * (ww // 2) * (c // 2) + 16, dtype=torch.uint8, device=device)
                             for k, (hh, ww, c) in {'a12': (h, w, 64), 'a22': (h2, w2, 128), 'fusion': (h4, w4, 256)}.items()}
        base = self.ws.data_ptr()
        assert base % 256 == 0
        for b in B.values():
            b.base = base + b.off
        if self.a12_alias:
            B['a12'] = B['a11']
        self.B = B


_PARAM_ENGINE = {}


def register_params(engine, params):
    if len(_PARAM_ENGINE) > 4096:
        for k in [k for k, (rp, re_) in _PARAM_ENGINE.items() if rp() is None or re_() is None]:
            del _PARAM_ENGINE[k]
    re_ = weakref.ref(engine)
    for p in params:
        ent = _PARAM_ENGINE.get(id(p))
        if ent is None or ent[0]() is not p or ent[1]() is not engine:
            _PARAM_ENGINE[id(p)] = (weakref.ref(p), re_)


def engine_of(params):
    eng = None
    for p in params:
        ent = _PARAM_ENGINE.get(id(p))
        if ent is None or ent[0]() is not p:
            return None
        e = ent[1]()
        if e is None or (eng is not None and e is not eng):
            return None
        eng = e
    return eng


class Engine:
    def __init__(self, net):
        self.net = net
        self.kind = net.KIND
        self.L = _lib.lib()
        self.plans = {}
        self.wcache = {}
        self.bias_cache = {}
        self.last_plan = None
# ... 730 lines not shown
            check(self.L.dbx_conv_wgrad_pool_dz(dt, C.byref(dyv), ptr(nib), nch, C.byref(dz), C.byref(x), kh, kw, cpad, co, ci, ptr(dw), ptr(db),
                                                ptr(self._wg_scratch), accumulate, write_dz, stream_ptr()))
        elif gen is not None:
            dov, w2p, ks, nh, use_hash, seed = gen
            check(self.L.dbx_heads1_wgrad_gen(dt, C.byref(dov), C.byref(x), w2p, ks, nh, use_hash, seed, ci, ptr(dw), ci_total, ci_off, ptr(db),
                                              ptr(self._wg_scratch), stream_ptr()))
        elif ci_total is None:
            check(self.L.dbx_conv_wgrad(dt, C.byref(dz), C.byref(x), kh, kw, cpad, co, ci, ptr(dw), ptr(db),
                                        ptr(self._wg_scratch), accumulate, stream_ptr()))
        else:
            check(self.L.dbx_conv_wgrad_slice(dt, C.byref(dz), C.byref(x), kh, kw, cpad, co, ci, ptr(dw), ci_total, ci_off, ptr(db),
                                              ptr(self._wg_scratch), accumulate, stream_ptr()))
        if prof is not None:
            ev1.record()
            buf = C.create_string_buffer(64)
            check(self.L.dbx_conv_wgrad_plan(dt, C.byref(dz), C.byref(x), kh, kw, buf, 64, None))
            name = buf.value.decode()
            if gen is not None:
                name = name.replace('>', ',gen>')
            if pool is not None:
                name = name.replace('>', ',pool+dz>' if pool[3] else ',pool>')
            prof.append({'kernel': name, 'flops': 2.0 * dz.n * dz.h * dz.w * kh * kw * ci * co, 'start': ev0, 'end': ev1})

    def backward_raw(self, grad_outs):
        L, kind = self.L, self.kind
        P = self.last_plan
        assert P is not None and P.train, 'backward needs a preceding training-mode forward'
        B, dt, n = P.B, P.dtype_id, P.n
        s = stream_ptr()
        dev = P.ws.device
        heads = _HEADS[kind]
        nh = len(heads)
        h4, w4 = P.h4, P.w4
        G = {}

        sink = self.grad_sink

        def new_grad(name):
            p = self._param(name)
            g = sink.grad_view(name) if sink is not None else torch.empty_like(p, dtype=torch.float32)
            G[name] = g
            return g

        def gout(name, k):
            g = grad_outs.get(name)
            if g is None:
                return torch.zeros((n, k, h4, w4), dtype=torch.float32, device=dev)
            return g.to(torch.float32).contiguous()

        main = torch.cuda.current_stream()
        side = None
        multi = sink is not None and getattr(sink, 'world', 1) > 1
        if self.profile is None and not multi and os.environ.get('DBX_SIDE_STREAM', '0') == '1':
            if getattr(self, '_side', None) is None:
                self._side = torch.cuda.Stream(device=dev)
            side = self._side

        def on_side(fn):
            if side is None:
                return fn()
            ev = torch.cuda.Event()
            ev.record(main)
            side.wait_event(ev)
            with torch.cuda.stream(side):
                return fn()

        def conv_bwd(stem, dz, x, kh, kw, cpad, co, ci):
            dw, db = new_grad(stem + '.weight'), new_grad(stem + '.bias')
            pool = None
            if stem == 'conv1_2_1' and pool12:
                pool = (B['d_p1'].view(), P.pool_idx['a12'], 64, 1 if pool12 == 1 else 0)

            def run():
                self._wgrad(dt, dz, x, kh, kw, cpad, co, ci, dw, db, pool=pool)
                if sink is not None:
                    sink.ready([stem + '.weight', stem + '.bias'])
            on_side(run)

        def dgrad(stem, src, dst, kh, kw, cpad, rows_pad, cin_pad, gate=None, epi=0, dropmask=None):
            frag = stem in _BWD_IO and kh == 3 and self._frag(P, dt, stem, 'b')
            wp = self._w_bwd(dt, stem, rows_pad, cin_pad, frag=frag)
            e = epi | (_lib.EPI_GATE if gate is not None else 0) | (_lib.CONV_WFRAG if frag else 0)
            self._conv(dt, src, dst, wp, None, kh, kw, cpad, cin_pad, rows_pad, e, gate=gate, dropmask=dropmask,
                       dm_ld=512 * nh)

        override = {}
        if kind != 'DenseBox' and P.refine_fwd is not None:
            lmk, det, wf7, vf7 = P.refine_fwd
            pn = ['conv6_1_det.weight', 'conv6_1_det.bias', 'conv6_2_det.weight', 'conv6_2_det.bias', 'conv6_3_det.weight', 'conv6_3_det.bias']
            ps = [self._param(nm).detach() for nm in pn]
            gs = [new_grad(nm) for nm in pn]

            def f32c(t):
                return None if t is None else t.to(torch.float32).contiguous()
            g_lm, g_det = f32c(grad_outs.get('landmark')), f32c(grad_outs.get('det'))
            o_lm = torch.empty((n, 4, h4, w4), dtype=torch.float32, device=dev)
            o_det = torch.empty((n, 1, h4, w4), dtype=torch.float32, device=dev)
            need = L.dbx_refine_backward_scratch_bytes(n, h4, w4)
            if getattr(self, '_rf_scratch', None) is None or self._rf_scratch.numel() < need:
                self._rf_scratch = torch.empty(int(need), dtype=torch.uint8, device=dev)
            d_rf = gout('refine', 1)
            check(L.dbx_refine_backward(ptr(d_rf), ptr(lmk), ptr(det), n, h4, w4, *[ptr(p) for p in ps], ps[0].shape[0], ptr(wf7), ptr(vf7),
                                        ptr(g_lm), ptr(g_det), ptr(o_lm), ptr(o_det), *[ptr(g_) for g_ in gs], ptr(self._rf_scratch), s))
            if sink is not None:
                sink.ready(pn)
            override = {'landmark': o_lm, 'det': o_det}
        elif kind != 'DenseBox' and os.environ.get('DBX_REFINE_LINEAR', '1') != '0':
            raise RuntimeError('densebox_amd: backward of the refine branch without its forward state (no training-mode forward on this plan)')
        elif kind != 'DenseBox':
            d_rfo = B['d_rfo'].view()
            check(L.dbx_nchw_to_framed(dt, ptr(gout('refine', 1)), 1, C.byref(d_rfo), s))
            conv_bwd('conv6_3_det', d_rfo, B['rf_u'].view(), 1, 1, 0, 1, 64)
            dgrad('conv6_3_det', d_rfo, B['d_rf_u'].view(), 1, 1, 0, 64, P.crf)
            check(L.dbx_upsample_bilinear_bwd(dt, C.byref(B['d_rf_u'].view()), C.byref(B['d_rf_2'].view()), None, s))
            conv_bwd('conv6_2_det', B['d_rf_2'].view(), B['rf_1'].view(), 5, 5, 0, 64, 64)
            dgrad('conv6_2_det', B['d_rf_2'].view(), B['d_rf_1'].view(), 5, 5, 4, 64, 64)
            conv_bwd('conv6_1_det', B['d_rf_1'].view(), B['rf_p'].view(), 3, 3, 0, 64, 5)
            dgrad('conv6_1_det', B['d_rf_1'].view(), B['d_rf_p'].view(), 3, 3, 2, 64, 64)
            check(L.dbx_maxpool2x2_bwd(dt, C.byref(B['rf_in'].view()), C.byref(B['d_rf_p'].view()),
                                       C.byref(B['d_rf_in'].view()), 0, 0, s))

        slot = {}
        srcs = []
        for i, (stem, k) in enumerate(heads):
            slot[stem] = B['d_out'].view(P.crf * i, P.crf)
            src = override.get(stem)
            srcs.append(src if src is not None else gout(stem, k))
        if override or kind == 'DenseBox':
            check(L.dbx_nchw_to_framed_slots(dt, (C.c_void_p * nh)(*[t.data_ptr() for t in srcs]), (C.c_int32 * nh)(*[k for _, k in heads]), nh, P.crf,
                                             C.byref(B['d_out'].view()), s))
        else:
            for (stem, k), t in zip(heads, srcs):
                check(L.dbx_nchw_to_framed(dt, ptr(t), k, C.byref(slot[stem]), s))
        if kind != 'DenseBox' and not override:
            check(L.dbx_framed_add_ch(dt, C.byref(B['d_rf_in'].view()), 0, 4, C.byref(slot['landmark']), 0, s))
            check(L.dbx_framed_add_ch(dt, C.byref(B['d_rf_in'].view()), 4, 1, C.byref(slot['det']), 0, s))

        hv = B['hid'].view()
        need = L.dbx_head2_wgrad_scratch_bytes(nh, hv.n * hv.h)
        if getattr(self, '_h2_scratch', None) is None or self._h2_scratch.numel() < need:
            self._h2_scratch = torch.empty(int(need), dtype=torch.uint8, device=dev)
        dw2 = [new_grad('conv5_2_%s.weight' % st) for st, _ in heads]
        db2 = [new_grad('conv5_2_%s.bias' % st) for st, _ in heads]
        prof = self.profile
        if prof is not None:
            ev0, ev1 = torch.cuda.Event(enable_timing=True), torch.cuda.Event(enable_timing=True)
            ev0.record()
        w2s = [self._param('conv5_2_%s.weight' % st).detach() for st, _ in heads]
        ks = (C.c_int32 * nh)(*[k for _, k in heads])
        h2_names = ['conv5_2_%s.weight' % st for st, _ in heads] + ['conv5_2_%s.bias' % st for st, _ in heads]
        mask_p = C.c_void_p(P.mask_buf.data_ptr()) if (P.drop_active and not P.drop_hash) else None
        hash_on, hash_seed = (1 if P.drop_hash else 0), (P.drop_seed if P.drop_hash else 0)
        lin = self._lin_bwd(dt)
        up_done = False
        gen = bool(getattr(P, 'heads_gen', False) and lin and side is None and mask_p is None)
        if gen and dt != _lib.F32:
            dhid_v = View(None, hv.n, hv.h, hv.w, 1, 512 * nh, 0, 512 * nh)
        else:
            dhid_v = self._d_hid(P).view()
        w2p = (C.c_void_p * nh)(*[w.data_ptr() for w in w2s])
        if side is not None:
            def run_h2():
                check(L.dbx_head2_wgrad(dt, C.byref(B['d_out'].view()), C.byref(hv), ks, nh,
                                        (C.c_void_p * nh)(*[t.data_ptr() for t in dw2]), (C.c_void_p * nh)(*[t.data_ptr() for t in db2]),
                                        ptr(self._h2_scratch), stream_ptr()))
                if sink is not None:
                    sink.ready(h2_names)
            on_side(run_h2)
            check(L.dbx_head2_dgrad(dt, C.byref(B['d_out'].view()), (C.c_void_p * nh)(*[w.data_ptr() for w in w2s]), ks, nh,
                                    C.byref(dhid_v), mask_p, 512 * nh, hash_on, hash_seed, s))
        elif lin:
            check(L.dbx_head2_backward_up(dt, C.byref(B['d_out'].view()), C.byref(hv), (C.c_void_p * nh)(*[w.data_ptr() for w in w2s]), ks, nh,
                                          C.byref(dhid_v), mask_p, 512 * nh, hash_on, hash_seed,
                                          (C.c_void_p * nh)(*[t.data_ptr() for t in dw2]), (C.c_void_p * nh)(*[t.data_ptr() for t in db2]),
                                          ptr(self._h2_scratch), C.byref(B['d_g44'].view()), s))
            up_done = True
            if gen and dt == _lib.F32:
                bh = P.B['d_hid']
                P.ws[bh.off:bh.off + bh.bytes].view(torch.float32).fill_(float('nan'))
        else:
            check(L.dbx_head2_backward(dt, C.byref(B['d_out'].view()), C.byref(hv), (C.c_void_p * nh)(*[w.data_ptr() for w in w2s]), ks, nh,
                                       C.byref(dhid_v), mask_p, 512 * nh, hash_on, hash_seed,
                                       (C.c_void_p * nh)(*[t.data_ptr() for t in dw2]), (C.c_void_p * nh)(*[t.data_ptr() for t in db2]),
                                       ptr(self._h2_scratch), s))
            if sink is not None:
                sink.ready(h2_names)
        if prof is not None:
            ev1.record()
            prof.append({'kernel': ('head2_backward_up_kernel<%s>' if up_done else 'head2_wgrad_kernel<%s>') % ('f16', 'bf16', 'f32')[dt],
                         'flops': 2.0 * hv.n * hv.h * hv.w * 512 * sum(k for _, k in heads) * (1 if side is not None else 2), 'start': ev0, 'end': ev1})
        w1n = ['conv5_1_%s.weight' % st for st, _ in heads]
        b1n = ['conv5_1_%s.bias' % st for st, _ in heads]
        if sink is not None:
            dw1, db1 = sink.region(w1n).view(512 * nh, 768, 1, 1), sink.region(b1n)
        else:
            dw1 = torch.empty((512 * nh, 768, 1, 1), dtype=torch.float32, device=dev)
            db1 = torch.empty((512 * nh,), dtype=torch.float32, device=dev)
        c34 = B['fusion'].view(512, 256)
        if lin and not up_done:
            check(L.dbx_upsample_bilinear_bwd(dt, C.byref(dhid_v), C.byref(B['d_g44'].view()), None, s))

        def run_h1():
            if lin:
                self._wgrad(dt, B['d_g44'].view(), B['a44'].view(), 1, 1, 0, 512 * nh, 512, dw1, None, ci_total=768, ci_off=0)
                if gen:
                    self._wgrad(dt, dhid_v, c34, 1, 1, 0, 512 * nh, 256, dw1, db1, ci_total=768, ci_off=512,
                                gen=(B['d_out'].view(), w2p, ks, nh, hash_on, hash_seed))
                else:
                    self._wgrad(dt, dhid_v, c34, 1, 1, 0, 512 * nh, 256, dw1, db1, ci_total=768, ci_off=512)
            else:
                self._wgrad(dt, dhid_v, B['fusion'].view(), 1, 1, 0, 512 * nh, 768, dw1, db1)
            if sink is not None:
                sink.ready(w1n + b1n)
        on_side(run_h1)
        for i, (stem, _) in enumerate(heads):
            G['conv5_1_%s.weight' % stem] = dw1[512 * i:512 * (i + 1)]
            G['conv5_1_%s.bias' % stem] = db1[512 * i:512 * (i + 1)]
        row_bytes = 512 * nh * _lib.ESIZE[dt]
        if lin:
            fa, fc = self._frag_heads(P, dt, 'ba'), self._frag_heads(P, dt, 'bc')
            self._conv(dt, B['d_g44'].view(), B['d_a44'].view(), self._w_heads1_bwd_part(dt, 'a', frag=fa), None, 1, 1, 0, 512 * nh, 512,
                       _lib.EPI_GATE | (_lib.CONV_WFRAG if fa else 0), gate=B['a44'].view())
            if gen:
                if prof is not None:
                    ev0, ev1 = torch.cuda.Event(enable_timing=True), torch.cuda.Event(enable_timing=True)
                    ev0.record()
                check(L.dbx_heads1_dgrad_gen(dt, C.byref(B['d_out'].view()), w2p, ks, nh, hash_on, hash_seed,
                                             ptr(self._w_heads1_bwd_part(dt, 'c', frag=dt != _lib.F32)), C.byref(B['d_c34'].view()), C.byref(c34), s))
                if prof is not None:
                    ev1.record()
                    prof.append({'kernel': 'heads1_dgrad_gen_kernel<%s>' % ('f16', 'bf16', 'f32')[dt],
                                 'flops': 2.0 * hv.n * hv.h * hv.w * 512 * nh * (256 + 8), 'start': ev0, 'end': ev1})
            else:
                if fc and getattr(P, 'heads_gen', False):
                    fc = self.conv_plan(dt, dhid_v, B['d_c34'].view(), 1, 1, 0, 512 * nh, 256, _lib.EPI_GATE)[2]
                self._conv(dt, dhid_v, B['d_c34'].view(), self._w_heads1_bwd_part(dt, 'c', frag=fc), None, 1, 1, 0, 512 * nh, 256,
                           _lib.EPI_GATE | (_lib.CONV_WFRAG if fc else 0), gate=c34)
        elif dt != _lib.F32:
            bfrag = self._frag_heads(P, dt, 'b')
            w1t = self._w_heads1_bwd(dt, frag=bfrag)
            d = ConvDesc(dt, 1, 1, 0, 512 * nh, 768, _lib.CONV_WFRAG if bfrag else 0, 0)
            prof = self.profile
            if prof is not None:
                ev0, ev1 = torch.cuda.Event(enable_timing=True), torch.cuda.Event(enable_timing=True)
                ev0.record()
            check(L.dbx_conv_forward_split(C.byref(d), C.byref(dhid_v), ptr(w1t), None, C.byref(B['d_ups'].view()), None,
                                           C.byref(B['d_c34'].view()), C.byref(c34), 512, _lib.EPI_GATE, s))
            if prof is not None:
                ev1.record()
                hv = dhid_v
                dv = B['d_ups'].view()
                both = View(dv.ptr, dv.n, dv.h, dv.w, dv.pad, 768, 0, 768)
                prof.append({'kernel': self.conv_plan(dt, hv, both, 1, 1, 0, 512 * nh, 768, 0)[1] if bfrag else
                             'conv_igemm_dma_kernel<%s,256,256>' % ('f16', 'bf16', 'f32')[dt],
                             'flops': 2.0 * hv.n * hv.h * hv.w * 512 * nh * 768, 'start': ev0, 'end': ev1})
        else:
            w1t = self._w_heads1_bwd(dt, frag=False)
            self._conv(dt, dhid_v, B['d_ups'].view(), w1t, None, 1, 1, 0, 512 * nh, 512, 0)
            self._conv(dt, dhid_v, B['d_c34'].view(), w1t[512 * row_bytes:], None, 1, 1, 0, 512 * nh, 256,
                       _lib.EPI_GATE, gate=c34)
        if not lin:
            check(L.dbx_upsample_bilinear_bwd(dt, C.byref(B['d_ups'].view()), C.byref(B['d_a44'].view()),
                                              C.byref(B['a44'].view()), s))

        chain = [
            ('conv4_4_1', 'd_a44', 'a43', 512, 512, 'd_a43', 'a43'),
            ('conv4_3_1', 'd_a43', 'a42', 512, 512, 'd_a42', 'a42'),
            ('conv4_2_1', 'd_a42', 'a41', 512, 512, 'd_a41', 'a41'),
            ('conv4_1_1', 'd_a41', 'p3', 256, 512, 'd_p3', None),
            ('pool', 'fusion', 'd_p3', 'd_c34', 1),
            ('conv3_4_1', 'd_c34', 'a32', 256, 256, 'd_a32', 'a32'),
            ('conv3_2_1', 'd_a32', 'a31', 256, 256, 'd_a31', 'a31'),
            ('conv3_1_1', 'd_a31', 'p2', 128, 256, 'd_p2', None),
            ('pool', 'a22', 'd_p2', 'd_a22', 0),
            ('conv2_2_1', 'd_a22', 'a21', 128, 128, 'd_a21', 'a21'),
            ('conv2_1_1', 'd_a21', 'p1', 64, 128, 'd_p1', None),
            ('pool', 'a12', 'd_p1', 'd_a12', 0),
            ('conv1_2_1', 'd_a12', 'a11', 64, 64, 'd_a11', 'a11'),
            ('conv1_1_1', 'd_a11', 'x0', 3, 64, None, None),
        ]
        fused11 = False
        pool12 = 0
        if P.pool_idx is not None and os.environ.get('DBX_POOL_WGRAD', '1') != '0' and \
                L.dbx_conv_wgrad_pool_dz_ok(dt, C.byref(B['d_a12'].view()), C.byref(B['a11'].view()), 3, 3):
            pool12 = 2 if (os.environ.get('DBX_POOL_WGRAD') == '2' or side is not None) else 1
        for item in chain:
            if item[0] == 'conv1_1_1' and fused11:
                continue
            if item[0] == 'conv1_2_1':
                stem, dzn, xn, cin, cout, dxn, gaten = item
                d12 = ConvDesc(dt, 3, 3, 1, 64, 64, _lib.EPI_GATE, 0)
                dzv, gv, x0v = B[dzn].view(), B[gaten].view(), B['x0'].view()
                if side is None and os.environ.get('DBX_FUSE_WG1', '1') != '0' and L.dbx_conv_dgrad_wgrad1_fusable(C.byref(d12), C.byref(dzv), C.byref(gv), C.byref(x0v)):
                    conv_bwd(stem, dzv, B[xn].view(), 3, 3, 1, cout, cin)
                    need = L.dbx_conv_dgrad_wgrad1_scratch_bytes()
                    if getattr(self, '_wg1_scratch', None) is None or self._wg1_scratch.numel() < need:
                        self._wg1_scratch = torch.empty(int(need), dtype=torch.uint8, device=dev)
                    dw1, db1 = new_grad('conv1_1_1.weight'), new_grad('conv1_1_1.bias')
                    if prof is not None:
                        ev0, ev1 = torch.cuda.Event(enable_timing=True), torch.cuda.Event(enable_timing=True)
                        ev0.record()
                    check(L.dbx_conv_dgrad_wgrad1(C.byref(d12), C.byref(dzv), ptr(self._w_bwd(dt, stem, 64, 64, frag=False)),
                                                  C.byref(gv), C.byref(x0v), 3, ptr(dw1), ptr(db1), ptr(self._wg1_scratch), 0, s))
                    if prof is not None:
                        ev1.record()
                        prof.append({'kernel': self.conv_plan(dt, dzv, B[dxn].view(), 3, 3, 1, 64, 64, _lib.EPI_GATE)[1],
                                     'flops': 2.0 * dzv.n * dzv.h * dzv.w * 9 * 64 * (64 + 3), 'start': ev0, 'end': ev1})
                    if sink is not None:
                        sink.ready(['conv1_1_1.weight', 'conv1_1_1.bias'])
                    fused11 = True
                    continue
            if item[0] == 'pool':
                _, xname, dyname, dxname, acc = item
                if xname == 'a12' and pool12 == 1:
                    continue
                if P.pool_idx is not None:
                    check(L.dbx_maxpool2x2_bwd_idx(dt, ptr(P.pool_idx[xname]), C.byref(B[dyname].view()), C.byref(B[dxname].view()),
                                                   acc, 1, s))
                    continue
                xv = c34 if xname == 'fusion' else B[xname].view()
                check(L.dbx_maxpool2x2_bwd(dt, C.byref(xv), C.byref(B[dyname].view()), C.byref(B[dxname].view()),
                                           acc, 1, s))
                continue
            stem, dzn, xn, cin, cout, dxn, gaten = item
            conv_bwd(stem, B[dzn].view(), B[xn].view(), 3, 3, 1, cout, cin)
            if dxn is not None:
                dgrad(stem, B[dzn].view(), B[dxn].view(), 3, 3, 1, max(64, cin), cout,
                      gate=B[gaten].view() if gaten else None)
        if side is not None:
            main.wait_stream(side)
        return G
```

densebox_amd/loss.py:

```python
import ctypes as C

import numpy as np
import torch

from . import _lib, labels as LB
from ._lib import LossDesc, LossIO, check, ptr, stream_ptr

_KIND_ID = {'DenseBox': 0, 'DenseBoxLM': 1, 'DenseBoxLMLOC': 2}


class _LossFn(torch.autograd.Function):
    @staticmethod
    def forward(ctx, loss, n_out, *outs_and_grads):
        outs, grads = outs_and_grads[:n_out], outs_and_grads[n_out:]
        ctx.grads = grads
        return loss.clone()

    @staticmethod
    def backward(ctx, g):
        return (None, None) + tuple(d * g for d in ctx.grads) + (None,) * len(ctx.grads)


def densebox_loss(kind, outputs, bbox, vertices=None, labels=None, rand_neg_indices=None, lm_rand_neg_indices=None,
                  lambda_loc=3.0, lambda_det=1.0, lambda_lm=0.5, batch_global=None, positive_num_global=None,
                  return_debug=False, rng=None):
    kid = _KIND_ID[kind]
    if kind == 'DenseBox':
        score, loc = outputs
        lm = rf = lmloc = None
    elif kind == 'DenseBoxLM':
        score, loc, lm, rf = outputs
        lmloc = None
    else:
        score, rf, loc, lm, lmloc = outputs
    dev = score.device
    n = score.size(0)
    assert tuple(score.shape[1:]) == (1, 60, 60), 'the dense loss is defined on the 60x60 training grid'
    use_labels = kind == 'DenseBoxLMLOC'
    P = int(LB.positive_count(bbox, labels if use_labels else None).sum()) if positive_num_global is None \
        else int(positive_num_global)
    _, half = LB.neg_counts(P, n if batch_global is None else batch_global)
    rs = rng if rng is not None else np.random
    if rand_neg_indices is None:
        rand_neg_indices = np.stack([rs.choice(3600, half, replace=False) for _ in range(n)]) if half else \
            np.zeros((n, 0), np.int64)
    if kid != 0 and lm_rand_neg_indices is None:
        lm_rand_neg_indices = np.stack([np.stack([rs.choice(3600, 1, replace=False) for _ in range(n)])
                                        for _ in range(4)])
    rn = LB._dev(rand_neg_indices, dev, torch.int64).reshape(n, half)
    lrn = LB._dev(lm_rand_neg_indices, dev, torch.int64).reshape(4, n, 1) if kid != 0 else None
    bb = LB._dev(bbox, dev)
    vt = LB._dev(vertices, dev) if kid != 0 else None
    lb = LB._dev(labels, dev) if use_labels else None

    def c32(t):
        return None if t is None else t.detach().to(torch.float32).contiguous()
    o = [c32(t) for t in (score, loc, lm, rf, lmloc)]
    g = [None if t is None else torch.empty_like(t) for t in o]
    loss = torch.empty(1, dtype=torch.float32, device=dev)
    scratch = torch.empty((_lib.lib().dbx_loss_scratch_bytes(n) + 7) // 8, dtype=torch.float64, device=dev)
    dbg = {}
    if return_debug:
        dbg['mask_cls'] = torch.empty((n, 1, 60, 60), dtype=torch.float32, device=dev)
        dbg['neg_idx'] = torch.empty((n, 2 * half), dtype=torch.int64, device=dev)
        dbg['pos_count'] = torch.empty(n, dtype=torch.int32, device=dev)
        if kid != 0:
            dbg['mask_lm'] = torch.empty((n, 4, 60, 60), dtype=torch.float32, device=dev)
            dbg['lm_neg_idx'] = torch.empty((4, n, 2), dtype=torch.int64, device=dev)
    d = LossDesc(kid, n, half, lambda_loc, lambda_det, lambda_lm, 1 if use_labels else 0)
    io = LossIO()
    for name, t in (('bbox', bb), ('vertices', vt), ('labels', lb), ('rand_neg', rn), ('lm_rand_neg', lrn),
                    ('score', o[0]), ('loc', o[1]), ('lm', o[2]), ('rf', o[3]), ('lmloc', o[4]),
                    ('d_score', g[0]), ('d_loc', g[1]), ('d_lm', g[2]), ('d_rf', g[3]), ('d_lmloc', g[4]),
                    ('loss', loss), ('mask_cls', dbg.get('mask_cls')), ('mask_lm', dbg.get('mask_lm')),
                    ('neg_idx', dbg.get('neg_idx')), ('lm_neg_idx', dbg.get('lm_neg_idx')),
                    ('pos_count', dbg.get('pos_count'))):
        setattr(io, name, t.data_ptr() if t is not None else None)
    check(_lib.lib().dbx_loss_forward_backward(C.byref(d), C.byref(io), ptr(scratch), stream_ptr()))
    live = [(t, gg) for t, gg in zip((score, loc, lm, rf, lmloc), g) if t is not None]
    out = _LossFn.apply(loss[0], len(live), *[t for t, _ in live], *[gg for _, gg in live])
    out._dbx_direct = ([t for t, _ in live], [gg for _, gg in live])
    if return_debug:
        dbg['half'] = half
        dbg['grads'] = {k: gg for k, gg in zip(('score', 'loc', 'lm', 'rf', 'lmloc'), g) if gg is not None}
        return out, dbg
    return out
```

include/densebox_hip.h:

```cpp
#ifndef DENSEBOX_HIP_H
#define DENSEBOX_HIP_H

#include <stdint.h>

#ifdef __cplusplus
extern "C" {
#endif

enum dbx_status {
    DBX_OK = 0,
    DBX_ERR_ARG = -1,
    DBX_ERR_HIP = -2,
    DBX_ERR_DTYPE = -3
};

enum dbx_dtype { DBX_F16 = 0, DBX_BF16 = 1, DBX_F32 = 2 };

const char* dbx_last_error(void);
#define DBX_ABI_VERSION 13
int dbx_version(void);
int dbx_device_arch(int device);

typedef struct dbx_view {
    void*   ptr;
    int32_t n, h, w;
    int32_t pad;
    int32_t ld;
    int32_t c_off;
    int32_t c;
} dbx_view;

enum dbx_epilogue {
    DBX_EPI_BIAS     = 1,
    DBX_EPI_RELU     = 2,
    DBX_EPI_GATE     = 4,
    DBX_EPI_DROPMASK = 8,
    DBX_EPI_ACCUM    = 16,
    DBX_EPI_F32_NCHW = 32,
    DBX_EPI_DROPHASH = 64,
    DBX_CONV_WFRAG   = 128
};

typedef struct dbx_conv_desc {
    int32_t dtype;
    int32_t kh, kw;
    int32_t cpad;
    int32_t cin_pad;
    int32_t cout_pad;
    int32_t epilogue;
    uint32_t drop_seed;
} dbx_conv_desc;

int64_t dbx_conv_packed_elems(const dbx_conv_desc* d);
int dbx_conv_forward(const dbx_conv_desc* d, const dbx_view* x, const void* w_packed, const float* bias,
                     const dbx_view* y, const dbx_view* gate, const uint8_t* dropmask, int32_t dropmask_ld,
                     void* stream);
enum dbx_conv_kernel { DBX_K_IGEMM = 1, DBX_K_DMA = 2, DBX_K_BAND = 3, DBX_K_C64 = 4, DBX_K_C8 = 5, DBX_K_WS = 6, DBX_K_P8 = 7 };
typedef struct dbx_conv_plan_t {
    int32_t kernel;
    int32_t tile_m, tile_n;
    int32_t w_frag;
    char    name[64];
} dbx_conv_plan_t;
int dbx_conv_plan(const dbx_conv_desc* d, const dbx_view* x, const dbx_view* y, dbx_conv_plan_t* out);

int dbx_heads_forward_fusable(const dbx_conv_desc* d, const dbx_view* x, const dbx_view* hid, const int32_t* k, int32_t nh);
int64_t dbx_heads_forward_fused_scratch_bytes(int32_t nh, int64_t pixels);
int dbx_heads_forward_fused(const dbx_conv_desc* d, const dbx_view* x, const void* w1_frag, const float* bias1, const dbx_view* hid,
                            const void* w2_frag, const float* bias2, const int32_t* k, int32_t nh, float* out_nchw, void* scratch,
                            void* stream);
int dbx_heads_forward_fused_heads(const dbx_conv_desc* d, const dbx_view* x, const void* w1_frag, const float* bias1, const dbx_view* hid,
                                  const void* w2_frag, const float* bias2, const int32_t* k, int32_t nh, float* const* outs, void* scratch,
                                  void* stream);

int dbx_conv_forward_split(const dbx_conv_desc* d, const dbx_view* x, const void* w_packed, const float* bias,
                           const dbx_view* y, const dbx_view* gate, const dbx_view* y2, const dbx_view* gate2,
                           int32_t split_c, int32_t epilogue2, void* stream);

int dbx_conv_pool_fusable(const dbx_conv_desc* d, const dbx_view* x, const dbx_view* y);
int dbx_conv_forward_pool(const dbx_conv_desc* d, const dbx_view* x, const void* w_packed, const float* bias,
                          const dbx_view* y, const dbx_view* ypool, int32_t write_full, void* stream);
int dbx_conv_forward_pool_idx(const dbx_conv_desc* d, const dbx_view* x, const void* w_packed, const float* bias,
                              const dbx_view* y, const dbx_view* ypool, int32_t write_full, void* idx, void* stream);

int dbx_pack_weight(int32_t dtype, int32_t mode, const float* w_oihw, int32_t co, int32_t ci, int32_t kh, int32_t kw,
                    void* w_packed, int32_t rows_pad, int32_t cin_pad, int32_t row_off, int32_t k_off, void* stream);

int dbx_pack_multi(int32_t dtype, const void* jobs, int32_t count, int64_t max_elems, void* stream);

int dbx_sgd_pack_step(int32_t dtype, const void* jobs, int32_t count, int64_t max_elems, float* const* ptrs, float lr, float momentum,
                      float weight_decay, int32_t first_step, void* stream);

int dbx_head2_dgrad(int32_t dtype, const dbx_view* d_out, const float* const* w2, const int32_t* k, int32_t nh,
                    const dbx_view* d_hid, const uint8_t* dropmask, int32_t dropmask_ld, int32_t use_hash, uint32_t drop_seed,
                    void* stream);
int64_t dbx_head2_wgrad_scratch_bytes(int32_t nh, int32_t rows);
int dbx_head2_wgrad(int32_t dtype, const dbx_view* d_out, const dbx_view* hid, const int32_t* k, int32_t nh,
                    float* const* dw, float* const* db, void* scratch, void* stream);
int dbx_head2_backward(int32_t dtype, const dbx_view* d_out, const dbx_view* hid, const float* const* w2, const int32_t* k,
                       int32_t nh, const dbx_view* d_hid, const uint8_t* dropmask, int32_t dropmask_ld, int32_t use_hash,
                       uint32_t drop_seed, float* const* dw, float* const* db, void* scratch, void* stream);
int dbx_head2_backward_up(int32_t dtype, const dbx_view* d_out, const dbx_view* hid, const float* const* w2, const int32_t* k,
                          int32_t nh, const dbx_view* d_hid, const uint8_t* dropmask, int32_t dropmask_ld, int32_t use_hash,
                          uint32_t drop_seed, float* const* dw, float* const* db, void* scratch, const dbx_view* d_g44, void* stream);
int dbx_conv_wgrad_pool_dz_ok(int32_t dtype, const dbx_view* dz, const dbx_view* x, int32_t kh, int32_t kw);
int dbx_conv_wgrad_pool_dz(int32_t dtype, const dbx_view* dy, const void* idx, int32_t idx_channels, const dbx_view* dz, const dbx_view* x,
                           int32_t kh, int32_t kw, int32_t cpad, int32_t co, int32_t ci, float* dw_oihw, float* db, void* scratch,
                           int32_t accumulate, int32_t write_dz, void* stream);
int dbx_head2_backward_up_fused(int32_t dtype, const dbx_view* hid, const dbx_view* d_g44);
int dbx_heads1_wgrad_gen_ok(int32_t dtype, const dbx_view* x, int32_t nh);
int dbx_heads1_wgrad_gen(int32_t dtype, const dbx_view* d_out, const dbx_view* x, const float* const* w2, const int32_t* k, int32_t nh,
                         int32_t use_hash, uint32_t drop_seed, int32_t ci, float* dw_oihw, int32_t dw_ci_total, int32_t dw_ci_off,
                         float* db, void* scratch, void* stream);
int dbx_heads1_dgrad_gen(int32_t dtype, const dbx_view* d_out, const float* const* w2, const int32_t* k, int32_t nh, int32_t use_hash,
                         uint32_t drop_seed, const void* w1t_frag, const dbx_view* y, const dbx_view* gate, void* stream);

int dbx_fold_heads(const float* w2, const float* b2, const float* w1, const float* b1, int32_t k, float* w_out,
                   float* b_out, void* stream);
int dbx_fold_refine(const float* w1, const float* b1, const float* w2, const float* b2, const float* w3, const float* b3,
                    int32_t ci, int32_t cm, float* w_out, float* b_out, float* v_out, void* stream);
int dbx_refine_eval(const float* landmark_nchw, const float* score_nchw, int32_t n, int32_t h, int32_t w, const float* w_fold,
                    const float* b_fold, float* out_small, void* stream);
int dbx_upsample_bilinear_nchw_f32(const float* x, int32_t planes, int32_t hi, int32_t wi, float* y, int32_t ho, int32_t wo,
                                   void* stream);
int64_t dbx_refine_backward_scratch_bytes(int32_t n, int32_t h, int32_t w);
int dbx_refine_backward(const float* d_refine, const float* landmark, const float* score, int32_t n, int32_t h, int32_t w,
                        const float* w1, const float* b1, const float* w2, const float* b2, const float* w3, const float* b3,
                        int32_t cm, const float* w_fold, const float* v_fold, const float* g_landmark, const float* g_score, float* out_landmark,
                        float* out_score, float* dw1, float* db1, float* dw2, float* db2, float* dw3, float* db3, void* scratch,
                        void* stream);

int64_t dbx_conv_wgrad_scratch_bytes(int32_t dtype, const dbx_view* dz, const dbx_view* x, int32_t kh, int32_t kw);
int dbx_conv_wgrad(int32_t dtype, const dbx_view* dz, const dbx_view* x, int32_t kh, int32_t kw, int32_t cpad,
                   int32_t co, int32_t ci, float* dw_oihw, float* db, void* scratch, int32_t accumulate, void* stream);
int dbx_conv_wgrad_slice(int32_t dtype, const dbx_view* dz, const dbx_view* x, int32_t kh, int32_t kw, int32_t cpad,
                         int32_t co, int32_t ci, float* dw_oihw, int32_t dw_ci_total, int32_t dw_ci_off, float* db, void* scratch,
                         int32_t accumulate, void* stream);
int dbx_conv_wgrad_plan(int32_t dtype, const dbx_view* dz, const dbx_view* x, int32_t kh, int32_t kw, char* name, int32_t name_len,
                        int32_t* splits);

int64_t dbx_conv_dgrad_wgrad1_scratch_bytes(void);
int dbx_conv_dgrad_wgrad1_fusable(const dbx_conv_desc* d, const dbx_view* dz, const dbx_view* gate, const dbx_view* x0);
int dbx_conv_dgrad_wgrad1(const dbx_conv_desc* d, const dbx_view* dz, const void* w_packed, const dbx_view* gate, const dbx_view* x0,
                          int32_t ci, float* dw_oihw, float* db, void* scratch, int32_t accumulate, void* stream);

int dbx_nchw_to_framed(int32_t dtype, const float* x_nchw, int32_t c_src, const dbx_view* y, void* stream);
int dbx_u8hwc_to_framed(int32_t dtype, const uint8_t* x_nhwc, const dbx_view* y, const float* mean3, const float* std3,
                        void* stream);
int dbx_nchw_to_framed_ch(int32_t dtype, const float* x_nchw, int32_t c_src, const dbx_view* y, int32_t c_dst_off,
                          void* stream);
int dbx_nchw_to_framed_slots(int32_t dtype, const float* const* x_nchw, const int32_t* k, int32_t nslots, int32_t slot,
                             const dbx_view* y, void* stream);
int dbx_framed_to_nchw_f32(int32_t dtype, const dbx_view* x, float* y_nchw, void* stream);
int dbx_framed_add_ch(int32_t dtype, const dbx_view* src, int32_t c_src_off, int32_t n_ch, const dbx_view* dst,
                      int32_t c_dst_off, void* stream);
int dbx_maxpool2x2(int32_t dtype, const dbx_view* x, const dbx_view* y, void* stream);
int dbx_maxpool2x2_bwd(int32_t dtype, const dbx_view* x, const dbx_view* dy, const dbx_view* dx,
                       int32_t accumulate, int32_t relu_gate, void* stream);
int64_t dbx_maxpool_idx_bytes(int32_t n, int32_t h, int32_t w, int32_t c);
int dbx_maxpool2x2_idx(int32_t dtype, const dbx_view* x, const dbx_view* y, void* idx, void* stream);
int dbx_maxpool2x2_bwd_idx(int32_t dtype, const void* idx, const dbx_view* dy, const dbx_view* dx,
                           int32_t accumulate, int32_t relu_gate, void* stream);
int dbx_upsample_bilinear(int32_t dtype, const dbx_view* x, const dbx_view* y, void* stream);
int dbx_upsample_bilinear_bwd(int32_t dtype, const dbx_view* dy, const dbx_view* dx, const dbx_view* gate, void* stream);

typedef struct dbx_loss_desc {
    int32_t kind;
    int32_t n;
    int32_t half_neg;
    float   lambda_loc, lambda_det, lambda_lm;
    int32_t use_labels;
} dbx_loss_desc;

typedef struct dbx_loss_io {
    const float* bbox;
    const float* vertices;
    const float* labels;
    const int64_t* rand_neg;
    const int64_t* lm_rand_neg;
    const float* score;  const float* loc;  const float* lm;  const float* rf;  const float* lmloc;
    float* d_score; float* d_loc; float* d_lm; float* d_rf; float* d_lmloc;
    float* loss;
    float* mask_cls;
    float* mask_lm;
    int64_t* neg_idx;
    int64_t* lm_neg_idx;
    int32_t* pos_count;
} dbx_loss_io;

int64_t dbx_loss_scratch_bytes(int32_t n);
int dbx_loss_forward_backward(const dbx_loss_desc* d, const dbx_loss_io* io, void* scratch, void* stream);
int dbx_count_positives(const float* bbox, const float* labels, int32_t n, int32_t* count_per_sample, void* stream);

int dbx_init_score_map(const float* bbox, const float* labels, int32_t n, float* out, void* stream);
int dbx_init_offset_map(const float* coords, const float* labels, int32_t n, int32_t c, float* out, void* stream);
int dbx_init_lm_heatmap(const float* vertices, const float* labels, int32_t n, int32_t clamp, float* out, void* stream);
int dbx_mask_by_sel(float* mask, int32_t n, const int64_t* pos_idx, int64_t n_pos, const int64_t* neg_idx, int32_t n_neg, void* stream);
int dbx_mask_gray_zone_cls(float* mask, const float* bbox, const float* labels, int32_t n, void* stream);
int dbx_mask_gray_zone_lm(float* mask, int32_t n, const int64_t* pos_idx, int64_t n_pos, void* stream);

int dbx_sgd_step(float* const* ptrs, const int64_t* sizes, int32_t count, int64_t max_size,
                 float lr, float momentum, float weight_decay, int32_t first_step, void* stream);
int dbx_grad_guard(const float* grads, int64_t n, int32_t* guard, int32_t step_id, void* stream);
int dbx_sgd_step_guarded(float* const* ptrs, const int64_t* sizes, int32_t count, int64_t max_size, float lr, float momentum,
                         float weight_decay, int32_t first_step, int32_t* guard, int32_t step_id, void* stream);
int dbx_sgd_pack_step_guarded(int32_t dtype, const void* jobs, int32_t count, int64_t max_elems, float* const* ptrs, float lr, float momentum,
                              float weight_decay, int32_t first_step, int32_t* guard, int32_t step_id, void* stream);

int dbx_detect(const float* score, const float* loc, const float* lm_heat, const float* lm_loc,
               int32_t rows, int32_t cols, int32_t K, double nms_thresh,
               double* dets, int32_t det_cols, int64_t* topk_idx, int32_t* keep, void* scratch, void* stream);
int64_t dbx_detect_scratch_bytes(int32_t rows, int32_t cols, int32_t K);
int64_t dbx_detect_batch_scratch_bytes(int32_t batch, int32_t rows, int32_t cols, int32_t K);
int dbx_detect_batch(const float* score, const float* loc, const float* lm_heat, const float* lm_loc,
                     int32_t batch, int32_t rows, int32_t cols, int32_t K, double nms_thresh,
                     double* dets, int32_t det_cols, int64_t* topk_idx, int32_t* keep, void* scratch, void* stream);
int dbx_nms(const double* dets, int32_t n, int32_t det_cols, double nms_thresh, int32_t* keep, void* scratch, void* stream);

int64_t dbx_detect_thresh_batch_scratch_bytes(int32_t batch, int32_t rows, int32_t cols, int32_t max_dets);
int dbx_detect_thresh_batch(const float* score, const float* loc, const float* lm_heat, const float* lm_loc,
                            int32_t batch, int32_t rows, int32_t cols, float score_thresh, int32_t max_dets, double nms_thresh,
                            double* dets, int32_t det_cols, int64_t* topk_idx, int32_t* keep, int32_t* counts, void* scratch,
                            void* stream);
int64_t dbx_thresh_rows_batch_scratch_bytes(int32_t batch, int32_t rows, int32_t cols, int32_t max_dets);
int dbx_thresh_rows_batch(const float* score, const float* loc, const float* lm_heat, const float* lm_loc,
                          int32_t batch, int32_t rows, int32_t cols, float score_thresh, int32_t max_dets,
                          double* dets, int32_t det_cols, int64_t* topk_idx, int32_t* counts, void* scratch, void* stream);
int64_t dbx_nms_large_scratch_bytes(int32_t n);
int dbx_nms_large(const double* dets, int32_t n, int32_t det_cols, double nms_thresh, int32_t* keep, void* scratch, void* stream);

typedef struct dbx_merge_xform { double scale, off_x, off_y; } dbx_merge_xform;
int64_t dbx_merge_nms_batch_workspace_bytes(int32_t levels, int32_t batch, int32_t K);
int dbx_merge_nms_batch(const double* const* level_dets, const dbx_merge_xform* xform, int32_t levels, int32_t batch, int32_t K,
                        int32_t det_cols, double nms_thresh, double* out_dets, int32_t* out_keep, void* workspace, void* stream);

int64_t dbx_merge_nms_thresh_batch_workspace_bytes(int32_t levels, int32_t batch, int32_t max_dets);
int dbx_merge_nms_thresh_batch(const double* const* level_dets, const int32_t* const* level_counts, const dbx_merge_xform* xform,
                               int32_t levels, int32_t batch, int32_t max_dets, int32_t det_cols, double nms_thresh,
                               double* out_dets, int32_t* out_keep, int32_t* out_counts, void* workspace, void* stream);

int dbx_perspective_matrix(const float* src_xy, const float* dst_xy, double* m9);
int dbx_warp_perspective_u8(const uint8_t* src, int32_t sh, int32_t sw, int32_t c, const double* m9, uint8_t* dst,
                            int32_t dh, int32_t dw, void* stream);
typedef struct dbx_warp_job {
    const uint8_t* src;
    int32_t sh, sw;
    double m9[9];
    int32_t dh, dw;
    int32_t x0, y0, oh, ow;
    int64_t dst_off;
} dbx_warp_job;
int64_t dbx_warp_batch_workspace_bytes(int32_t njobs);
int dbx_warp_perspective_batch_u8(const dbx_warp_job* jobs, int32_t njobs, int32_t c, uint8_t* dst, void* workspace, void* stream);

typedef struct dbx_crop_frame {
    const uint8_t* src;
    int32_t sh, sw;
} dbx_crop_frame;
int dbx_plate_crops_batch(const dbx_crop_frame* frames, int32_t nframes, int32_t c, const double* quads, int64_t row_stride,
                          int64_t frame_stride, const int32_t* sel, int32_t slots, int32_t ow, int32_t oh, uint8_t* dst, int32_t* ok,
                          double* m9_out, void* stream);

typedef struct dbx_eval_record {
    double  score;
    double  lm_err;
    int32_t status;
    int32_t frame;
} dbx_eval_record;
// ... 170 lines not shown
```

Measured before the change: 7707 patches/s.

## Add sparse head backward for loc/lmloc heads using positive-row hints

The loss marks the gradients of the loc and lmloc heads with a row bound taken from the positive-sample count, since those gradients are nonzero only at positive pixels. A new sparse backward path scans the head gradient for nonzero rows, compacts them into a list, and computes the dgrad and upsample contributions only for those rows. The head2 wgrad for these heads is accumulated over the compacted rows by a new kernel, while the dense heads keep the existing fused kernel. This adds scan and compaction kernels and depends on a correct capacity bound; when the count exceeds capacity, the bias gradient is set to NaN.

```diff
diff --git a/densebox_amd/_lib.py b/densebox_amd/_lib.py
--- a/densebox_amd/_lib.py
+++ b/densebox_amd/_lib.py
@@ -208,6 +208,12 @@
     'dbx_heads1_dgrad_gen': (C.c_int, [_I32, _PV, C.POINTER(C.c_void_p), C.POINTER(C.c_int32), _I32, _I32, C.c_uint32, _VP, _PV, _PV, _VP]),
     'dbx_heads1_wgrad_gen': (C.c_int, [_I32, _PV, _PV, C.POINTER(C.c_void_p), C.POINTER(C.c_int32), _I32, _I32, C.c_uint32, _I32, _VP, _I32, _I32,
                              _VP, _VP, _VP]),
+    'dbx_head2_backward_up_heads': (C.c_int, [_I32, _PV, _PV, C.POINTER(C.c_void_p), C.POINTER(C.c_int32), _I32, _PV, _VP, _I32, _I32, C.c_uint32,
+                                              C.POINTER(C.c_void_p), C.POINTER(C.c_void_p), _VP, _PV, C.c_uint32, _VP, _I32, _VP]),
+    'dbx_heads_sparse_ok': (C.c_int, [_I32, _PV, _PV]),
+    'dbx_heads_sparse_ws_bytes': (_I64, [_I32, _I32, _I32, _I32, _I32]),
+    'dbx_heads_sparse_backward2': (C.c_int, [_I32, _PV, _PV, C.POINTER(C.c_void_p), C.POINTER(C.c_int32), _I32, C.c_uint32, _I32, C.c_uint32,
+                                             _PV, _I32, _VP, _VP, _VP, _VP]),
     'dbx_conv_wgrad_plan': (C.c_int, [_I32, _PV, _PV, _I32, _I32, C.c_char_p, _I32, C.POINTER(C.c_int32)]),
     'dbx_nchw_to_framed': (C.c_int, [_I32, _VP, _I32, _PV, _VP]),
     'dbx_u8hwc_to_framed': (C.c_int, [_I32, _VP, _PV, C.POINTER(C.c_float), C.POINTER(C.c_float), _VP]),
diff --git a/densebox_amd/csrc/aux_ops.hip b/densebox_amd/csrc/aux_ops.hip
--- a/densebox_amd/csrc/aux_ops.hip
+++ b/densebox_amd/csrc/aux_ops.hip
@@ -1,4 +1,5 @@
 #include "common.hpp"
+#include "bilin.hpp"
 #include <mutex>
 
 static thread_local char g_err[512] = "";
@@ -335,16 +336,6 @@
     DBX_DISPATCH_DTYPE(dtype, maxpool_bwd_idx_t, idx, dy, dx, accumulate, relu_gate, (hipStream_t)stream);
 }
 
-__device__ __forceinline__ void bilin_coef(int d, float scale, int in, int& i0, int& i1, float& l0, float& l1) {
-#pragma clang fp contract(off)
-    const float src = scale * (float)d;
-    i0 = (int)src;
-    if (i0 > in - 1) i0 = in - 1;
-    i1 = i0 + (i0 < in - 1 ? 1 : 0);
-    l1 = src - (float)i0;
-    l0 = 1.f - l1;
-}
-static inline float ac_scale(int in, int out) { return out > 1 ? (float)(in - 1) / (float)(out - 1) : 0.f; }
 
 template <typename T>
 __global__ void upsample_kernel(FrameGeo x, FrameGeo y, float sy, float sx) {
@@ -1352,9 +1343,90 @@
     return true;
 }
 template <typename T>
+__global__ __launch_bounds__(1024) void head2_rows_partial_kernel(FrameGeo dout, FrameGeo hid, int hd, int slot, int kj, int G, H2UPlan plan,
+                                                                  const int* __restrict__ rows, int cap, float* __restrict__ partial,
+                                                                  float* __restrict__ bpartial) {
+    extern __shared__ __attribute__((aligned(16))) char h2r_smem[];
+    float* const s_acc = (float*)h2r_smem;
+    float* const s_b = s_acc + 32 * 8 * 64;
+    __shared__ int s_match[1024], s_sel[16][64], s_cnt[16];
+    const int tid = threadIdx.x, lane = tid & 63, wv = tid >> 6, ch = lane;
+    const int blk = blockIdx.x / 8, cbase = (blockIdx.x % 8) * 64, half = blk % plan.halves, grp = blk / plan.halves;
+    const H2UHalf hf = half ? plan.h[1] : plan.h[0];
+    for (int i = tid; i < 32 * 8 * 64 + 32 * 8; i += 1024) s_acc[i] = 0.f;
+    const int W = hid.w, HW = hid.h * hid.w;
+    const int count = cap > 0 ? rows[0] : 0, nrow = count < cap ? count : cap;
+    const int* list = rows + 16;
+    __syncthreads();
+    for (int r0 = 0; r0 < nrow; r0 += 1024) {
+        const int r = r0 + tid;
+        int pix = 0; bool m = false;
+        if (r < nrow) {
+            pix = list[r];
+            const int n = pix / HW, x = (pix - n * HW) % W;
+            m = n % G == grp && x >= hf.own_lo && x < hf.own_hi;
+        }
+        const unsigned long long bal = __ballot(m);
+        if (lane == 0) s_cnt[wv] = __popcll(bal);
+        __syncthreads();
+        int off = __popcll(bal & ((1ull << lane) - 1ull)), total = 0;
+#pragma unroll
+        for (int q = 0; q < 16; ++q) { if (q < wv) off += s_cnt[q]; total += s_cnt[q]; }
+        if (m) s_match[off] = pix;
+        __syncthreads();
+        for (int base = 0; base < total; base += 64) {
+            const int e = base + lane < total ? s_match[base + lane] : -1;
+            const bool sel = e >= 0 && ((e % W) - hf.px_lo) % 16 == wv;
+            const unsigned long long sb = __ballot(sel);
+            const int nsel = __popcll(sb);
+            if (sel) s_sel[wv][__popcll(sb & ((1ull << lane) - 1ull))] = e;
+            __syncthreads();
+            for (int i0 = 0; i0 < nsel; i0 += 8) {
+                u32x4 graw[8]; T hv[8]; int col[8];
+#pragma unroll
+                for (int u = 0; u < 8; ++u) {
+                    const int px = s_sel[wv][i0 + u < nsel ? i0 + u : nsel - 1];
+                    const int n = px / HW, rem = px - n * HW, y = rem / W, x = rem - y * W;
+                    col[u] = x - hf.px_lo;
+                    graw[u] = *(const u32x4*)((const T*)dout.base + geo_pix(dout, n, y, x) + hd * slot);
+                    hv[u] = *((const T*)hid.base + geo_pix(hid, n, y, x) + hd * 512 + cbase + ch);
+                }
+#pragma unroll
+                for (int u = 0; u < 8; ++u) {
+                    if (i0 + u < nsel) {
+                        const T* ge = (const T*)&graw[u];
+                        const float h = to_f32(hv[u]);
+#pragma unroll
+                        for (int j = 0; j < 8; ++j)
+                            if (j < kj) { float* a = &s_acc[(col[u] * 8 + j) * 64 + ch]; *a = fmaf(to_f32(ge[j]), h, *a); }
+                        if (lane < kj) s_b[col[u] * 8 + lane] += to_f32(ge[lane < 8 ? lane : 0]);
+                    }
+                }
+            }
+            __syncthreads();
+        }
+    }
+    __syncthreads();
+    auto tree = [](const float* p, int stride) {
+        float o = 0.f;
+#pragma unroll
+        for (int w4 = 0; w4 < 4; ++w4) {
+            const float* q = p + (size_t)(8 * w4) * stride;
+            o += ((q[0] + q[stride]) + (q[2 * stride] + q[3 * stride])) + ((q[4 * stride] + q[5 * stride]) + (q[6 * stride] + q[7 * stride]));
+        }
+        return o;
+    };
+    if (wv < 8) partial[((size_t)blk * 8 + wv) * 512 + cbase + ch] = tree(s_acc + wv * 64 + ch, 8 * 64);
+    if (cbase == 0 && wv == 8 && lane < 8) {
+        float b = tree(s_b + lane, 8);
+        if (cap > 0 && rows[0] > cap) b = __builtin_nanf("");
+        bpartial[(size_t)blk * 32 + lane] = b;
+    }
+}
+template <typename T>
 static int head2_backward_up_t(const dbx_view* dout, const dbx_view* hid, const float* const* w2, const int32_t* k, int nh, const dbx_view* dhid,
                                const uint8_t* mask, int mask_ld, int use_hash, unsigned drop_seed, float* const* dw, float* const* db,
-                               void* scratch, const dbx_view* dg, hipStream_t s) {
+                               void* scratch, const dbx_view* dg, hipStream_t s, unsigned head_mask = 0xFu, const int* rows = nullptr, int rows_cap = 0) {
     VIEW_VEC_CHECK(T, dg, "head2_backward_up d_g44");
     DBX_REQUIRE(dg->n == hid->n && dg->c == hid->c, "head2_backward_up: d_g44 has the hidden map's batch and channels");
     const float sy = ac_scale(dg->h, hid->h), sx = ac_scale(dg->w, hid->w);
@@ -1363,6 +1435,9 @@
     if (const char* e = getenv("DBX_HEAD2_UP")) fused = fused && atoi(e) != 0;
     const bool nostore = dhid->ptr == nullptr;
     DBX_REQUIRE(!nostore || (fused && !mask), "head2_backward_up without d_hid: needs the one-pass kernel (dbx_head2_backward_up_fused) and hash / no dropout");
+    const unsigned all_heads = nh >= 1 && nh <= 4 ? (1u << nh) - 1u : 0xFu;
+    head_mask &= all_heads;
+    DBX_REQUIRE(head_mask == all_heads || fused, "head2_backward_up on a subset of the heads: needs the one-pass kernel (dbx_head2_backward_up_fused)");
     if (!fused) {
         const int rc = head2_wgrad_t<T>(dout, hid, k, nh, dw, db, scratch, s, w2, dhid, mask, mask_ld, use_hash, drop_seed);
         return rc != DBX_OK ? rc : upsample_bwd_t<T>(dhid, dg, nullptr, s);
@@ -1381,7 +1456,8 @@
         for (int i = 0; i < 4; ++i) {
             o.dw[i] = i < nh ? dw[i] : nullptr; o.db[i] = (i < nh && db) ? db[i] : nullptr; o.k[i] = i < nh ? k[i] : 0;
             ha.w2[i] = i < nh ? w2[i] : nullptr; ha.k[i] = i < nh ? k[i] : 0;
-            if (i < nh) DBX_REQUIRE(k[i] >= 1 && k[i] <= 8 && dw[i] && w2[i] && ((size_t)w2[i] % 16) == 0, "head2_backward_up: k in 1..8, 16-byte aligned weights");
+            if (i < nh) DBX_REQUIRE(k[i] >= 1 && k[i] <= 8, "head2_backward_up: k in 1..8");
+            if (i < nh && (head_mask >> i & 1u)) DBX_REQUIRE(dw[i] && w2[i] && ((size_t)w2[i] % 16) == 0, "head2_backward_up: 16-byte aligned weights");
         }
         constexpr size_t smem = (size_t)2 * H2U_NB * 32 * 64 * 4;
         static_assert(smem >= (4 * 8 * 64 + 32) * 4 && 2 * smem + 4096 <= 160 * 1024, "LDS budget of two workgroups per CU");
@@ -1399,25 +1475,52 @@
         float* const pbase = (float*)scratch;
         long long pused = 0;
         int blocks_max = 0;
+        constexpr size_t smem_rows = (size_t)(32 * 8 * 64 + 32 * 8) * 4;
+        if (rows && head_mask != all_heads) {
+            static DbxDevOnce rows_once; int rows_dev = 0;
+            if (rows_once.pending(&rows_dev)) {
+                DBX_HIP(hipFuncSetAttribute((const void*)head2_rows_partial_kernel<T>, hipFuncAttributeMaxDynamicSharedMemorySize, (int)smem_rows));
+                rows_once.mark(rows_dev);
+            }
+        }
         for (int h0 = 0; h0 < nh;) {
             int h1 = h0 + 1;
             while (h1 < nh && kup(k[h1]) == kup(k[h0])) ++h1;
-            const int nhl = h1 - h0, nsl = nhl * 8, kj = kup(k[h0]);
-            int groups = H2U_WGS / (nsl * plan.halves);
+            const int kj = kup(k[h0]);
+            int groups = H2U_WGS / ((h1 - h0) * 8 * plan.halves);
             groups = groups < 1 ? 1 : groups > hid->n ? hid->n : groups;
             const int blocks = groups * plan.halves;
-            float* partial = pbase + pused;
-            float* bpartial = partial + (size_t)blocks * nhl * 8 * 512;
-            for (int i = h0; i < h1; ++i) { o.poff[i] = pused; o.boff[i] = pused + (long long)blocks * nhl * 8 * 512; o.nblk[i] = blocks; o.nhl[i] = nhl; o.hl[i] = i - h0; }
-            pused += (long long)blocks * (nhl * 8 * 512 + 32);
             blocks_max = blocks > blocks_max ? blocks : blocks_max;
+            for (int i0 = h0; i0 < h1;) {
+                if (!(head_mask >> i0 & 1u)) {
+                    if (rows) {
+                        DBX_REQUIRE(dw[i0], "head2_backward_up: null gradient");
+                        float* partial = pbase + pused;
+                        o.poff[i0] = pused; o.boff[i0] = pused + (long long)blocks * 8 * 512; o.nblk[i0] = blocks; o.nhl[i0] = 1; o.hl[i0] = 0;
+                        pused += (long long)blocks * (8 * 512 + 32);
+                        hipLaunchKernelGGL(head2_rows_partial_kernel<T>, dim3(blocks * 8), dim3(1024), smem_rows, s, make_geo<T>(dout), make_geo<T>(hid), i0,
+                                           dout->c / nh, kj, groups, plan, rows, rows_cap, partial, partial + (size_t)blocks * 8 * 512);
+                        DBX_LAUNCH_CHECK();
+                    } else { o.k[i0] = 0; o.poff[i0] = 0; o.boff[i0] = 0; o.nblk[i0] = 0; o.nhl[i0] = 1; o.hl[i0] = 0; }
+                    ++i0;
+                    continue;
+                }
+                int i1 = i0 + 1;
+                while (i1 < h1 && (head_mask >> i1 & 1u)) ++i1;
+                const int nhl = i1 - i0, nsl = nhl * 8;
+                float* partial = pbase + pused;
+                float* bpartial = partial + (size_t)blocks * nhl * 8 * 512;
+                for (int i = i0; i < i1; ++i) { o.poff[i] = pused; o.boff[i] = pused + (long long)blocks * nhl * 8 * 512; o.nblk[i] = blocks; o.nhl[i] = nhl; o.hl[i] = i - i0; }
+                pused += (long long)blocks * (nhl * 8 * 512 + 32);
 #define H2U_LAUNCH(KJ)                                                                                                              \
-            hipLaunchKernelGGL((head2_backward_up_kernel<T, KJ>), dim3(blocks * nsl), dim3(256), smem, s, make_geo<T>(dout), make_geo<T>(hid),    \
-                               make_geo<T>(nostore ? hid : dhid), make_geo<T>(dg), h0, nhl, dout->c / nh, ha, partial, bpartial, mask, mask_ld,    \
-                               use_hash, drop_seed, sy, sx, plan, nostore ? 1 : 0)
-            if (kj == 1) H2U_LAUNCH(1); else if (kj == 2) H2U_LAUNCH(2); else if (kj == 4) H2U_LAUNCH(4); else H2U_LAUNCH(8);
+                hipLaunchKernelGGL((head2_backward_up_kernel<T, KJ>), dim3(blocks * nsl), dim3(256), smem, s, make_geo<T>(dout), make_geo<T>(hid),    \
+                                   make_geo<T>(nostore ? hid : dhid), make_geo<T>(dg), i0, nhl, dout->c / nh, ha, partial, bpartial, mask, mask_ld,    \
+                                   use_hash, drop_seed, sy, sx, plan, nostore ? 1 : 0)
+                if (kj == 1) H2U_LAUNCH(1); else if (kj == 2) H2U_LAUNCH(2); else if (kj == 4) H2U_LAUNCH(4); else H2U_LAUNCH(8);
 #undef H2U_LAUNCH
-            DBX_LAUNCH_CHECK();
+                DBX_LAUNCH_CHECK();
+                i0 = i1;
+            }
             h0 = h1;
         }
         for (int i = nh; i < 4; ++i) { o.poff[i] = 0; o.boff[i] = 0; o.nblk[i] = 0; o.nhl[i] = 1; o.hl[i] = 0; }
@@ -1446,6 +1549,15 @@
     if (!d_out || !hid || !w2 || !k || !d_hid || !dw || !scratch || !d_g44) { dbx_set_error("head2_backward_up: null argument"); return DBX_ERR_ARG; }
     DBX_DISPATCH_DTYPE(dtype, head2_backward_up_t, d_out, hid, w2, k, nh, d_hid, dropmask, dropmask_ld, use_hash, (unsigned)drop_seed, dw, db,
                        scratch, d_g44, (hipStream_t)stream);
+}
+extern "C" int dbx_head2_backward_up_heads(int32_t dtype, const dbx_view* d_out, const dbx_view* hid, const float* const* w2, const int32_t* k,
+                                           int32_t nh, const dbx_view* d_hid, const uint8_t* dropmask, int32_t dropmask_ld, int32_t use_hash,
+                                           uint32_t drop_seed, float* const* dw, float* const* db, void* scratch, const dbx_view* d_g44,
+                                           uint32_t head_mask, const int32_t* rows, int32_t rows_capacity, void* stream) {
+    if (!d_out || !hid || !w2 || !k || !d_hid || !dw || !scratch || !d_g44) { dbx_set_error("head2_backward_up_heads: null argument"); return DBX_ERR_ARG; }
+    if (rows && (rows_capacity < 0 || ((size_t)rows % 16) != 0)) { dbx_set_error("head2_backward_up_heads: row list"); return DBX_ERR_ARG; }
+    DBX_DISPATCH_DTYPE(dtype, head2_backward_up_t, d_out, hid, w2, k, nh, d_hid, dropmask, dropmask_ld, use_hash, (unsigned)drop_seed, dw, db,
+                       scratch, d_g44, (hipStream_t)stream, (unsigned)head_mask, (const int*)rows, (int)rows_capacity);
 }
 
 struct PackJob { const float* src; void* dst; int co, ci, taps, mode; long long ktot; int cin_pad, row_off, k_off, rows_lim; };
diff --git a/densebox_amd/csrc/bilin.hpp b/densebox_amd/csrc/bilin.hpp
--- /dev/null
+++ b/densebox_amd/csrc/bilin.hpp
@@ -0,0 +1,13 @@
+#pragma once
+#include "common.hpp"
+
+__device__ __forceinline__ void bilin_coef(int d, float scale, int in, int& i0, int& i1, float& l0, float& l1) {
+#pragma clang fp contract(off)
+    const float src = scale * (float)d;
+    i0 = (int)src;
+    if (i0 > in - 1) i0 = in - 1;
+    i1 = i0 + (i0 < in - 1 ? 1 : 0);
+    l1 = src - (float)i0;
+    l0 = 1.f - l1;
+}
+static inline float ac_scale(int in, int out) { return out > 1 ? (float)(in - 1) / (float)(out - 1) : 0.f; }
diff --git a/densebox_amd/csrc/heads_sparse.hip b/densebox_amd/csrc/heads_sparse.hip
--- /dev/null
+++ b/densebox_amd/csrc/heads_sparse.hip
@@ -0,0 +1,327 @@
+#include "common.hpp"
+#include "bilin.hpp"
+
+namespace hsp {
+constexpr int RPC = 16;
+constexpr int MAXR = 16;
+constexpr int MAXW = 256;
+constexpr int HDR = 16;
+constexpr int SEGPIX = 512;
+struct Sel { int hd[4]; int k[4]; const float* w2[4]; int ns; };
+struct Layout { size_t list, base, cnt, dh, total; int nchunks, nseg; };
+static Layout layout(int n, int hw, int cap, int ns) {
+    auto up = [](size_t v) { return (v + 63) / 64 * 64; };
+    Layout l;
+    const int c1 = cap > 0 ? cap : 1;
+    l.nchunks = (cap + RPC - 1) / RPC;
+    l.nseg = (hw + SEGPIX - 1) / SEGPIX;
+    size_t o = (size_t)HDR * 4;
+    l.list = o; o = up(o + (size_t)c1 * 4);
+    l.base = o; o = up(o + (size_t)(n * l.nseg + 1) * 4);
+    l.cnt = o; o = up(o + (size_t)n * l.nseg * 4);
+    l.dh = o; o = up(o + (size_t)c1 * 512 * ns * 2);
+    l.total = o;
+    return l;
+}
+}
+
+template <typename T>
+__global__ __launch_bounds__(256) void hs_scan_kernel(FrameGeo dout, int slot, hsp::Sel sel, int nseg, int* __restrict__ map, int* __restrict__ cnt) {
+    __shared__ int s_w[4];
+    const int n = blockIdx.x / nseg, seg = blockIdx.x - n * nseg, W = dout.w, HW = dout.h * dout.w;
+    const int lane = threadIdx.x & 63, wv = threadIdx.x >> 6;
+    const int p0 = seg * hsp::SEGPIX + 2 * (int)threadIdx.x;
+    const int h0 = sel.hd[0] * slot, h1 = sel.hd[1] * slot, h2 = sel.hd[2] * slot, h3 = sel.hd[3] * slot, ns = sel.ns;
+    auto nonzero = [&](int p) {
+        const int pc = p < HW ? p : HW - 1, y = pc / W, x = pc - y * W;
+        const T* q = (const T*)dout.base + geo_pix(dout, n, y, x);
+        u32x4 v = *(const u32x4*)(q + h0);
+        if (ns > 1) { const u32x4 u = *(const u32x4*)(q + h1); v |= u; }
+        if (ns > 2) { const u32x4 u = *(const u32x4*)(q + h2); v |= u; }
+        if (ns > 3) { const u32x4 u = *(const u32x4*)(q + h3); v |= u; }
+        return p < HW && ((v.x | v.y | v.z | v.w) & 0x7fff7fffu) != 0u;
+    };
+    const bool z0 = nonzero(p0), z1 = nonzero(p0 + 1);
+    const int mine = (z0 ? 1 : 0) + (z1 ? 1 : 0);
+    int inc = mine;
+#pragma unroll
+    for (int d = 1; d < 64; d <<= 1) { const int o = __shfl_up(inc, d); if (lane >= d) inc += o; }
+    if (lane == 63) s_w[wv] = inc;
+    __syncthreads();
+    int off = inc - mine, tot = 0;
+#pragma unroll
+    for (int q = 0; q < 4; ++q) { if (q < wv) off += s_w[q]; tot += s_w[q]; }
+    if (p0 < HW) map[(size_t)n * HW + p0] = z0 ? off : -1;
+    if (p0 + 1 < HW) map[(size_t)n * HW + p0 + 1] = z1 ? off + (z0 ? 1 : 0) : -1;
+    if (threadIdx.x == 0) cnt[blockIdx.x] = tot;
+}
+
+__global__ __launch_bounds__(256) void hs_list_kernel(const int* __restrict__ map, const int* __restrict__ cnt, int* __restrict__ base,
+                                                      int* __restrict__ hdr, int* __restrict__ list, int nunits, int nseg, int HW, int cap) {
+    __shared__ int s_part[4];
+    const int u = blockIdx.x, n = u / nseg, seg = u - n * nseg;
+    int part = 0;
+    for (int i = threadIdx.x; i < u; i += 256) part += cnt[i];
+#pragma unroll
+    for (int d = 32; d > 0; d >>= 1) part += __shfl_xor(part, d);
+    if ((threadIdx.x & 63) == 0) s_part[threadIdx.x >> 6] = part;
+    __syncthreads();
+    const int b = s_part[0] + s_part[1] + s_part[2] + s_part[3];
+    if (threadIdx.x == 0) {
+        base[u] = b;
+        if (u == nunits - 1) { base[nunits] = b + cnt[u]; hdr[0] = b + cnt[u]; }
+    }
+    for (int p = seg * hsp::SEGPIX + threadIdx.x; p < (seg + 1) * hsp::SEGPIX && p < HW; p += 256) {
+        const int li = map[(size_t)n * HW + p];
+        if (li >= 0 && b + li < cap) list[b + li] = n * HW + p;
+    }
+}
+
+template <typename T>
+__global__ __launch_bounds__(256) void hs_stage2_kernel(FrameGeo dout, int H, int W, int slot, hsp::Sel sel, int use_hash, unsigned seed,
+                                                        const int* __restrict__ hdr, const int* __restrict__ list, int cap, T* __restrict__ dh) {
+    const int chunk = blockIdx.x, s = blockIdx.y, ns = sel.ns;
+    int hd = sel.hd[0], k = sel.k[0];
+    const float* wp = sel.w2[0];
+#pragma unroll
+    for (int q = 1; q < 4; ++q)
+        if (s == q) { hd = sel.hd[q]; k = sel.k[q]; wp = sel.w2[q]; }
+    const int kj = k <= 1 ? 1 : k <= 2 ? 2 : k <= 4 ? 4 : 8;
+    const int c = threadIdx.x * 2, HW = H * W;
+    const int count = hdr[0], rows = count < cap ? count : cap;
+    const int r0 = chunk * hsp::RPC, r1 = r0 + hsp::RPC < rows ? r0 + hsp::RPC : rows;
+    const float dscale = use_hash ? 2.f : 1.f;
+    float wj[8][2];
+#pragma unroll
+    for (int j = 0; j < 8; ++j) {
+        const int row = j < k ? j : (k > 0 ? k - 1 : 0);
+        const float v0 = wp[(size_t)row * 512 + c], v1 = wp[(size_t)row * 512 + c + 1];
+        wj[j][0] = to_f32(from_f32<T>(j < k ? v0 : 0.f)) * dscale;
+        wj[j][1] = to_f32(from_f32<T>(j < k ? v1 : 0.f)) * dscale;
+    }
+    for (int rb = r0; rb < r1; rb += 4) {
+        int pix[4]; u32x4 graw[4];
+#pragma unroll
+        for (int u = 0; u < 4; ++u) pix[u] = list[rb + u < r1 ? rb + u : r1 - 1];
+#pragma unroll
+        for (int u = 0; u < 4; ++u) {
+            const int n = pix[u] / HW, rem = pix[u] - n * HW, y = rem / W, x = rem - y * W;
+            graw[u] = *(const u32x4*)((const T*)dout.base + geo_pix(dout, n, y, x) + hd * slot);
+        }
+#pragma unroll
+        for (int u = 0; u < 4; ++u) {
+            if (rb + u < r1) {
+                const T* ge = (const T*)&graw[u];
+                float o0 = 0.f, o1 = 0.f;
+#pragma unroll
+                for (int j = 0; j < 8; ++j) {
+                    if (j < kj) {
+                        const float g = to_f32(ge[j]);
+                        o0 = fmaf(g, wj[j][0], o0); o1 = fmaf(g, wj[j][1], o1);
+                    }
+                }
+                if (use_hash) {
+                    const unsigned kb = dbx_drop_hash32(seed, (unsigned)pix[u], (unsigned)(hd * 512 + c) >> 5) >> ((unsigned)c & 31u);
+                    o0 = (kb & 1u) ? o0 : 0.f; o1 = (kb & 2u) ? o1 : 0.f;
+                }
+                unsigned raw;
+                T* oe = (T*)&raw;
+                oe[0] = from_f32<T>(o0); oe[1] = from_f32<T>(o1);
+                *(unsigned*)(dh + (size_t)(rb + u) * (512 * ns) + s * 512 + c) = raw;
+            }
+        }
+    }
+}
+
+template <typename T>
+__global__ __launch_bounds__(256) void hs_dg44_kernel(FrameGeo dg, int H, int W, float sy, float sx, hsp::Sel sel, const int* __restrict__ map,
+                                                      const int* __restrict__ prev_map, const int* __restrict__ base, int nseg, int cap,
+                                                      const T* __restrict__ dh, int zero_only) {
+    extern __shared__ int s_map[];
+    __shared__ int s_x0[hsp::MAXW], s_lo[hsp::MAXW], s_hi[hsp::MAXW], s_col[hsp::MAXW], s_any, s_prev;
+    __shared__ unsigned long long s_bal[4];
+    __shared__ float s_wy[hsp::MAXR], s_l0[hsp::MAXW], s_l1[hsp::MAXW];
+    const int n = blockIdx.x / dg.h, iy = blockIdx.x % dg.h, ns = sel.ns;
+    const int tid = threadIdx.x, lane = tid & 63, wv = tid >> 6;
+    int any = 0, nr = 0, was = 1;
+    {
+        int y0 = -1, y1 = -1; float ly0 = 0.f, ly1 = 0.f;
+        if (tid < H) bilin_coef(tid, sy, dg.h, y0, y1, ly0, ly1);
+        const bool mine = tid < H && (y0 == iy || y1 == iy);
+        const unsigned long long bal = __ballot(mine);
+        if (lane == 0) s_bal[wv] = bal;
+        if (tid == 0) { s_any = 0; s_prev = 0; }
+        __syncthreads();
+        int lo = 0, hi = -1;
+        bool found = false;
+#pragma unroll
+        for (int q = 0; q < 4; ++q) {
+            const unsigned long long b = s_bal[q];
+            if (b) { if (!found) { lo = 64 * q + __builtin_ctzll(b); found = true; } hi = 64 * q + 63 - __builtin_clzll(b); }
+        }
+        nr = hi - lo + 1;
+        nr = nr < 0 ? 0 : nr > hsp::MAXR ? hsp::MAXR : nr;
+        if (mine && tid - lo < hsp::MAXR) s_wy[tid - lo] = (y0 == iy ? ly0 : 0.f) + (y1 == iy ? ly1 : 0.f);
+        for (int i = tid; i < nr * W; i += 256) {
+            const int r = i / W, ox = i - r * W, p = (lo + r) * W + ox;
+            if (!zero_only) {
+                const int li = map[(size_t)n * H * W + p];
+                int gi = li >= 0 ? base[n * nseg + p / hsp::SEGPIX] + li : -1;
+                if (gi >= cap) gi = -1;
+                s_map[i] = gi;
+                if (gi >= 0) s_any = 1;
+            }
+            if (prev_map && prev_map[(size_t)n * H * W + p] >= 0) s_prev = 1;
+        }
+        __syncthreads();
+        any = s_any;
+        was = prev_map ? s_prev : 1;
+    }
+    if (!any && !was) return;
+    if (!any) {
+        T* rowp = (T*)dg.base + geo_pix(dg, n, iy, 0);
+        const int total = dg.w * ns * 64;
+        for (int i = tid; i < total; i += 256) {
+            const int chunk = i & 63, ps = i >> 6, ix = ps / ns, s = ps - ix * ns;
+            int hd = sel.hd[0];
+#pragma unroll
+            for (int t = 1; t < 4; ++t) if (s == t) hd = sel.hd[t];
+            *(u32x4*)(rowp + (size_t)ix * dg.ld + hd * 512 + chunk * 8) = (u32x4){0u, 0u, 0u, 0u};
+        }
+        return;
+    }
+    for (int ox = tid; ox < W; ox += 256) {
+        int x0, x1; float lx0, lx1;
+        bilin_coef(ox, sx, dg.w, x0, x1, lx0, lx1);
+        s_x0[ox] = x0; s_l0[ox] = x1 == x0 ? lx0 + lx1 : lx0; s_l1[ox] = x1 == x0 ? 0.f : lx1;
+        int h = 0;
+        for (int r = 0; r < nr; ++r) h |= s_map[r * W + ox] >= 0 ? 1 : 0;
+        s_col[ox] = h;
+    }
+    __syncthreads();
+    for (int ix = tid; ix < dg.w; ix += 256) {
+        int lo = W, hi = -1;
+        for (int ox = 0; ox < W; ++ox) { const int x0 = s_x0[ox]; if (x0 == ix || x0 == ix - 1) { if (ox < lo) lo = ox; hi = ox; } }
+        s_lo[ix] = lo; s_hi[ix] = hi;
+    }
+    __syncthreads();
+    const int ldh = 512 * ns;
+    for (int ix = wv; ix < dg.w; ix += 4) {
+        const int lo = s_lo[ix], hi = s_hi[ix];
+        T* pixp = (T*)dg.base + geo_pix(dg, n, iy, ix);
+        for (int cb = lane; cb < ns * 32; cb += 64) {
+            const int s = cb >> 5, c = (cb & 31) * 16;
+            int hd = sel.hd[0];
+#pragma unroll
+            for (int t = 1; t < 4; ++t) if (s == t) hd = sel.hd[t];
+            float a[16];
+#pragma unroll
+            for (int i = 0; i < 16; ++i) a[i] = 0.f;
+            for (int ox = lo; ox <= hi; ++ox) {
+                if (!s_col[ox]) continue;
+                const float cf = s_x0[ox] == ix ? s_l0[ox] : s_l1[ox];
+                float v[16];
+#pragma unroll
+                for (int i = 0; i < 16; ++i) v[i] = 0.f;
+                bool hit = false;
+                for (int r0 = 0; r0 < nr; r0 += 4) {
+                    u32x4 raw[4][2]; int gi[4];
+#pragma unroll
+                    for (int u = 0; u < 4; ++u) {
+                        gi[u] = r0 + u < nr ? s_map[(r0 + u) * W + ox] : -1;
+                        const T* src = dh + (size_t)(gi[u] < 0 ? 0 : gi[u]) * ldh + s * 512 + c;
+                        raw[u][0] = *(const u32x4*)src; raw[u][1] = *(const u32x4*)(src + 8);
+                    }
+#pragma unroll
+                    for (int u = 0; u < 4; ++u) {
+                        const bool use = gi[u] >= 0;
+                        const float wy = s_wy[r0 + u < nr ? r0 + u : 0];
+                        const T* de = (const T*)&raw[u][0];
+                        hit = hit || use;
+#pragma unroll
+                        for (int i = 0; i < 16; ++i) v[i] = fmaf(wy, use ? to_f32(de[i]) : 0.f, v[i]);
+                    }
+                }
+                if (hit) {
+#pragma unroll
+                    for (int i = 0; i < 16; ++i) a[i] = fmaf(cf, v[i], a[i]);
+                }
+            }
+            u32x4 o[2];
+            T* e = (T*)&o[0];
+#pragma unroll
+            for (int i = 0; i < 16; ++i) e[i] = from_f32<T>(a[i]);
+            *(u32x4*)(pixp + hd * 512 + c) = o[0]; *(u32x4*)(pixp + hd * 512 + c + 8) = o[1];
+        }
+    }
+}
+
+static bool hs_shapes_ok(int dtype, const dbx_view* hid, const dbx_view* dg) {
+    if (dtype != DBX_F16 && dtype != DBX_BF16) return false;
+    const float sy = ac_scale(dg->h, hid->h), sx = ac_scale(dg->w, hid->w);
+    return sy > 0.13f && sy < 1.f && sx > 0.45f && sx < 1.f && hid->w <= hsp::MAXW && dg->w <= hsp::MAXW && hid->h <= 256 && hid->h >= 2 && hid->c % 512 == 0 &&
+           dg->c == hid->c && dg->n == hid->n && (int64_t)hid->n * hid->h * hid->w < ((int64_t)1 << 30);
+}
+extern "C" int dbx_heads_sparse_ok(int32_t dtype, const dbx_view* hid, const dbx_view* d_g44) {
+    return hid && d_g44 && hs_shapes_ok(dtype, hid, d_g44) ? 1 : 0;
+}
+extern "C" int64_t dbx_heads_sparse_ws_bytes(int32_t n, int32_t h, int32_t w, int32_t capacity, int32_t ns) {
+    if (n < 1 || h < 1 || w < 1 || capacity < 0 || ns < 1 || ns > 4) return 0;
+    return (int64_t)hsp::layout(n, h * w, capacity, ns).total;
+}
+
+template <typename T>
+static int heads_sparse_backward2_t(const dbx_view* dout, const dbx_view* hid, const float* const* w2, const int32_t* k, int nh, unsigned head_mask,
+                                    int use_hash, unsigned seed, const dbx_view* dg, int cap, void* ws,
+                                    int* map, const int* prev_map, hipStream_t st) {
+    if constexpr (sizeof(T) != 2) {
+        dbx_set_error("heads_sparse_backward2: 16-bit compute types only");
+        return DBX_ERR_DTYPE;
+    } else {
+        DBX_REQUIRE(nh >= 1 && nh <= 4 && hid->c == 512 * nh && dout->c % nh == 0 && dout->c / nh >= 8, "heads_sparse_backward2: nh in 1..4, hid of 512*nh channels, d_out of nh slots >= 8 channels");
+        DBX_REQUIRE(dout->n == hid->n && dout->h == hid->h && dout->w == hid->w, "heads_sparse_backward2: d_out and hid are maps of the same pixels");
+        DBX_REQUIRE(hs_shapes_ok(DType<T>::id, hid, dg), "heads_sparse_backward2: shapes outside dbx_heads_sparse_ok");
+        DBX_REQUIRE(((size_t)dout->ptr % 16) == 0 && (dout->ld * 2) % 16 == 0 && (dout->c_off * 2) % 16 == 0 && ((dout->c / nh) * 2) % 16 == 0,
+                    "heads_sparse_backward2: d_out alignment");
+        DBX_REQUIRE(((size_t)hid->ptr % 16) == 0 && (hid->ld * 2) % 16 == 0 && (hid->c_off * 2) % 16 == 0 && ((size_t)dg->ptr % 16) == 0 &&
+                        (dg->ld * 2) % 16 == 0 && (dg->c_off * 2) % 16 == 0, "heads_sparse_backward2: hid / d_g44 alignment");
+        DBX_REQUIRE(cap >= 0 && ((size_t)ws % 64) == 0, "heads_sparse_backward2: capacity >= 0, 64-byte aligned workspace");
+        head_mask &= (1u << nh) - 1u;
+        hsp::Sel sel;
+        sel.ns = 0;
+        for (int i = 0; i < 4; ++i) { sel.hd[i] = 0; sel.k[i] = 0; sel.w2[i] = nullptr; }
+        for (int i = 0; i < nh; ++i)
+            if (head_mask >> i & 1u) {
+                DBX_REQUIRE(k[i] >= 1 && k[i] <= 8 && w2[i], "heads_sparse_backward2: k in 1..8, weights of the selected heads");
+                sel.hd[sel.ns] = i; sel.k[sel.ns] = k[i]; sel.w2[sel.ns] = w2[i];
+                ++sel.ns;
+            }
+        if (sel.ns == 0) return DBX_OK;
+        const int ns = sel.ns, n = hid->n, H = hid->h, W = hid->w, slot = dout->c / nh;
+        const hsp::Layout l = hsp::layout(n, H * W, cap, ns);
+        char* const wb = (char*)ws;
+        int* hdr = (int*)wb; int* list = (int*)(wb + l.list); int* base = (int*)(wb + l.base); int* cnt = (int*)(wb + l.cnt);
+        T* dh = (T*)(wb + l.dh);
+        const float sy = ac_scale(dg->h, H), sx = ac_scale(dg->w, W);
+        if (cap > 0) {
+            hipLaunchKernelGGL(hs_scan_kernel<T>, dim3(n * l.nseg), dim3(256), 0, st, make_geo<T>(dout), slot, sel, l.nseg, map, cnt);
+            DBX_LAUNCH_CHECK();
+            hipLaunchKernelGGL(hs_list_kernel, dim3(n * l.nseg), dim3(256), 0, st, map, cnt, base, hdr, list, n * l.nseg, l.nseg, H * W, cap);
+            DBX_LAUNCH_CHECK();
+            hipLaunchKernelGGL(hs_stage2_kernel<T>, dim3(l.nchunks, ns), dim3(256), 0, st, make_geo<T>(dout), H, W, slot, sel, use_hash, seed,
+                               hdr, list, cap, dh);
+            DBX_LAUNCH_CHECK();
+        }
+        const size_t smem = (size_t)hsp::MAXR * W * sizeof(int);
+        hipLaunchKernelGGL(hs_dg44_kernel<T>, dim3(n * dg->h), dim3(256), smem, st, make_geo<T>(dg), H, W, sy, sx, sel, map, prev_map, base, l.nseg,
+                           cap, dh, cap > 0 ? 0 : 1);
+        DBX_LAUNCH_CHECK();
+        return DBX_OK;
+    }
+}
+extern "C" int dbx_heads_sparse_backward2(int32_t dtype, const dbx_view* d_out, const dbx_view* hid, const float* const* w2, const int32_t* k,
+                                          int32_t nh, uint32_t head_mask, int32_t use_hash, uint32_t drop_seed, const dbx_view* d_g44, int32_t capacity, void* ws, int32_t* map, const int32_t* prev_map, void* stream) {
+    if (!d_out || !hid || !w2 || !k || !d_g44 || !ws || !map) { dbx_set_error("heads_sparse_backward2: null argument"); return DBX_ERR_ARG; }
+    DBX_DISPATCH_DTYPE(dtype, heads_sparse_backward2_t, d_out, hid, w2, k, nh, (unsigned)head_mask, use_hash, (unsigned)drop_seed, d_g44,
+                       capacity, ws, (int*)map, (const int*)prev_map, (hipStream_t)stream);
+}
diff --git a/densebox_amd/dist.py b/densebox_amd/dist.py
--- a/densebox_amd/dist.py
+++ b/densebox_amd/dist.py
@@ -191,6 +191,7 @@
     def global_positive_num(self, bbox, labels=None):
         from . import labels as LB
         p = int(LB.positive_count(bbox, labels).sum())
+        self._local_pos = p
         if self._pf is not None:
             local, total = self._consume_prefetch()
             if local != p:
@@ -239,8 +240,14 @@
              positive_num_global=None, **loss_kw):
         net = self.net
         n_global = x.size(0) * self.world
+        use_lab = labels if net.KIND == 'DenseBoxLMLOC' else None
+        local_pos = loss_kw.pop('positive_num_local', None)
         if positive_num_global is None:
-            positive_num_global = self.global_positive_num(bbox, labels if net.KIND == 'DenseBoxLMLOC' else None)
+            positive_num_global = self.global_positive_num(bbox, use_lab)
+            local_pos = self._local_pos if local_pos is None else local_pos
+        elif local_pos is None and not (torch.is_tensor(bbox) and bbox.is_cuda):
+            from . import labels as LB
+            local_pos = int(LB.positive_count(bbox, use_lab).sum())
         if x.is_cuda:
             import numpy as np
             from . import labels as LB
@@ -265,7 +272,7 @@
         try:
             outs = net(x)
             loss = net.loss(outs, bbox, vertices, labels, rand_neg_indices, lm_rand_neg_indices,
-                            batch_global=n_global, positive_num_global=positive_num_global, **loss_kw)
+                            batch_global=n_global, positive_num_global=positive_num_global, positive_num_local=local_pos, **loss_kw)
             direct = getattr(loss, '_dbx_direct', None)
             if direct is not None and all(t.requires_grad for t in direct[0]):
                 torch.autograd.backward(direct[0], direct[1])
diff --git a/densebox_amd/engine.py b/densebox_amd/engine.py
--- a/densebox_amd/engine.py
+++ b/densebox_amd/engine.py
@@ -29,6 +29,29 @@
                                      ('conv3_1_1', 128, 256), ('conv3_2_1', 256, 256), ('conv3_4_1', 256, 256),
                                      ('conv4_1_1', 256, 512), ('conv4_2_1', 512, 512), ('conv4_3_1', 512, 512),
                                      ('conv4_4_1', 512, 512)]}
+
+
+_ROW_HINTS = {}
+
+
+def hint_rows(t, bound, token=None):
+    if len(_ROW_HINTS) >= 64:
+        _ROW_HINTS.clear()
+    _ROW_HINTS[(t.data_ptr(), t._version)] = (int(bound), token if token is not None else object())
+
+
+def row_hint(t):
+    return None if t is None else _ROW_HINTS.get((t.data_ptr(), t._version))
+
+
+def sparse_capacity(hints, pixels):
+    if os.environ.get('DBX_HEADS_SPARSE', '1') == '0' or not hints:
+        return None
+    per = {}
+    for b, tok in hints:
+        per[id(tok)] = max(per.get(id(tok), 0), b)
+    cap = sum(per.values())
+    return cap if cap * 16 <= pixels else None
 
 
 def _align(x, a=256):
@@ -1065,13 +1088,22 @@
         mask_p = C.c_void_p(P.mask_buf.data_ptr()) if (P.drop_active and not P.drop_hash) else None
         hash_on, hash_seed = (1 if P.drop_hash else 0), (P.drop_seed if P.drop_hash else 0)
         lin = self._lin_bwd(dt)
-        up_done = False
+        up_done = h2_prof_done = False
         gen = bool(getattr(P, 'heads_gen', False) and lin and side is None and mask_p is None)
         if gen and dt != _lib.F32:
             dhid_v = View(None, hv.n, hv.h, hv.w, 1, 512 * nh, 0, 512 * nh)
         else:
             dhid_v = self._d_hid(P).view()
         w2p = (C.c_void_p * nh)(*[w.data_ptr() for w in w2s])
+        hinted = [(i, row_hint(grad_outs.get(stem))) for i, (stem, _) in enumerate(heads) if override.get(stem) is None]
+        hinted = [(i, hnt) for i, hnt in hinted if hnt is not None]
+        _ROW_HINTS.clear()
+        sp_cap = sparse_capacity([hnt for _, hnt in hinted], hv.n * hv.h * hv.w) if (gen and lin and dt != _lib.F32) else None
+        if sp_cap is not None and not L.dbx_heads_sparse_ok(dt, C.byref(hv), C.byref(B['d_g44'].view())):
+            sp_cap = None
+        sp_mask = sum(1 << i for i, _ in hinted) if sp_cap is not None else 0
+        P.heads_sparse = (sp_mask, sp_cap) if sp_mask else None
+        hs_prev, P.hs_prev = getattr(P, 'hs_prev', None), None
         if side is not None:
             def run_h2():
                 check(L.dbx_head2_wgrad(dt, C.byref(B['d_out'].view()), C.byref(hv), ks, nh,
@@ -1082,6 +1114,36 @@
             on_side(run_h2)
             check(L.dbx_head2_dgrad(dt, C.byref(B['d_out'].view()), (C.c_void_p * nh)(*[w.data_ptr() for w in w2s]), ks, nh,
                                     C.byref(dhid_v), mask_p, 512 * nh, hash_on, hash_seed, s))
+        elif lin and sp_mask:
+            dw2p, db2p = (C.c_void_p * nh)(*[t.data_ptr() for t in dw2]), (C.c_void_p * nh)(*[t.data_ptr() for t in db2])
+            need = L.dbx_heads_sparse_ws_bytes(hv.n, hv.h, hv.w, sp_cap, len(hinted))
+            if getattr(self, '_hs_ws', None) is None or self._hs_ws.numel() < need:
+                self._hs_ws = torch.empty(int(need * 1.5) + 1024, dtype=torch.uint8, device=dev)
+            if getattr(P, 'hs_maps', None) is None:
+                P.hs_maps = torch.empty((2, hv.n * hv.h * hv.w), dtype=torch.int32, device=dev)
+            keep = hs_prev is not None and hs_prev[0] == sp_mask and os.environ.get('DBX_HEADS_SPARSE_KEEP', '1') != '0'
+            cur = 1 - hs_prev[1] if keep else 0
+            check(L.dbx_heads_sparse_backward2(dt, C.byref(B['d_out'].view()), C.byref(hv), w2p, ks, nh, sp_mask, hash_on, hash_seed,
+                                               C.byref(B['d_g44'].view()), sp_cap, ptr(self._hs_ws), ptr(P.hs_maps[cur]),
+                                               ptr(P.hs_maps[1 - cur]) if keep else None, s))
+            P.hs_prev = (sp_mask, cur) if sp_cap > 0 else None
+            if prof is not None:
+                ev1.record()
+                prof.append({'kernel': 'hs_stage2_kernel<%s>' % ('f16', 'bf16', 'f32')[dt],
+                             'flops': 2.0 * sp_cap * 512 * sum(k for i, (_, k) in enumerate(heads) if sp_mask >> i & 1), 'start': ev0, 'end': ev1})
+                ev0, ev1 = torch.cuda.Event(enable_timing=True), torch.cuda.Event(enable_timing=True)
+                ev0.record()
+            check(L.dbx_head2_backward_up_heads(dt, C.byref(B['d_out'].view()), C.byref(hv), w2p, ks, nh, C.byref(dhid_v), mask_p, 512 * nh,
+                                                hash_on, hash_seed, dw2p, db2p, ptr(self._h2_scratch), C.byref(B['d_g44'].view()),
+                                                ((1 << nh) - 1) & ~sp_mask, ptr(self._hs_ws), sp_cap, s))
+            if prof is not None:
+                ev1.record()
+                prof.append({'kernel': 'head2_backward_up_kernel<%s>' % ('f16', 'bf16', 'f32')[dt],
+                             'flops': 2.0 * 512 * (hv.n * hv.h * hv.w * 2 * sum(k for i, (_, k) in enumerate(heads) if not sp_mask >> i & 1) +
+                                                   sp_cap * sum(k for i, (_, k) in enumerate(heads) if sp_mask >> i & 1)),
+                             'start': ev0, 'end': ev1})
+                h2_prof_done = True
+            up_done = True
         elif lin:
             check(L.dbx_head2_backward_up(dt, C.byref(B['d_out'].view()), C.byref(hv), (C.c_void_p * nh)(*[w.data_ptr() for w in w2s]), ks, nh,
                                           C.byref(dhid_v), mask_p, 512 * nh, hash_on, hash_seed,
@@ -1098,7 +1160,7 @@
                                        ptr(self._h2_scratch), s))
             if sink is not None:
                 sink.ready(h2_names)
-        if prof is not None:
+        if prof is not None and not h2_prof_done:
             ev1.record()
             prof.append({'kernel': ('head2_backward_up_kernel<%s>' if up_done else 'head2_wgrad_kernel<%s>') % ('f16', 'bf16', 'f32')[dt],
                          'flops': 2.0 * hv.n * hv.h * hv.w * 512 * sum(k for _, k in heads) * (1 if side is not None else 2), 'start': ev0, 'end': ev1})
diff --git a/densebox_amd/loss.py b/densebox_amd/loss.py
--- a/densebox_amd/loss.py
+++ b/densebox_amd/loss.py
@@ -5,25 +5,45 @@
 
 from . import _lib, labels as LB
 from ._lib import LossDesc, LossIO, check, ptr, stream_ptr
+from .engine import hint_rows
 
 _KIND_ID = {'DenseBox': 0, 'DenseBoxLM': 1, 'DenseBoxLMLOC': 2}
 
 
 class _LossFn(torch.autograd.Function):
     @staticmethod
-    def forward(ctx, loss, n_out, *outs_and_grads):
+    def forward(ctx, loss, n_out, hints, *outs_and_grads):
         outs, grads = outs_and_grads[:n_out], outs_and_grads[n_out:]
         ctx.grads = grads
+        ctx.hints = hints
         return loss.clone()
 
     @staticmethod
     def backward(ctx, g):
-        return (None, None) + tuple(d * g for d in ctx.grads) + (None,) * len(ctx.grads)
+        out = tuple(d * g for d in ctx.grads)
+        for t, h in zip(out, ctx.hints):
+            if h is not None:
+                hint_rows(t, *h)
+        return (None, None, None) + out + (None,) * len(ctx.grads)
+
+
+def _on_device(t):
+    return torch.is_tensor(t) and t.is_cuda
+
+
+def _row_hints(bbox, labels, positive_num_local, positive_num_global, counted, sparse):
+    bound = positive_num_local
+    if bound is None:
+        if _on_device(bbox):
+            return [None] * len(sparse)
+        bound = counted if positive_num_global is None else int(LB.positive_count(bbox, labels).sum())
+    token = object()
+    return [(int(bound), token) if sp else None for sp in sparse]
 
 
 def densebox_loss(kind, outputs, bbox, vertices=None, labels=None, rand_neg_indices=None, lm_rand_neg_indices=None,
                   lambda_loc=3.0, lambda_det=1.0, lambda_lm=0.5, batch_global=None, positive_num_global=None,
-                  return_debug=False, rng=None):
+                  return_debug=False, rng=None, positive_num_local=None):
     kid = _KIND_ID[kind]
     if kind == 'DenseBox':
         score, loc = outputs
@@ -78,7 +98,12 @@
         setattr(io, name, t.data_ptr() if t is not None else None)
     check(_lib.lib().dbx_loss_forward_backward(C.byref(d), C.byref(io), ptr(scratch), stream_ptr()))
     live = [(t, gg) for t, gg in zip((score, loc, lm, rf, lmloc), g) if t is not None]
-    out = _LossFn.apply(loss[0], len(live), *[t for t, _ in live], *[gg for _, gg in live])
+    hints = _row_hints(bbox, labels if use_labels else None, positive_num_local, positive_num_global, P,
+                       [gg is g[1] or gg is g[4] for _, gg in live])
+    for (_, gg), h in zip(live, hints):
+        if h is not None:
+            hint_rows(gg, *h)
+    out = _LossFn.apply(loss[0], len(live), tuple(hints), *[t for t, _ in live], *[gg for _, gg in live])
     out._dbx_direct = ([t for t, _ in live], [gg for _, gg in live])
     if return_debug:
         dbg['half'] = half
diff --git a/include/densebox_hip.h b/include/densebox_hip.h
--- a/include/densebox_hip.h
+++ b/include/densebox_hip.h
@@ -114,6 +114,14 @@
                          float* db, void* scratch, void* stream);
 int dbx_heads1_dgrad_gen(int32_t dtype, const dbx_view* d_out, const float* const* w2, const int32_t* k, int32_t nh, int32_t use_hash,
                          uint32_t drop_seed, const void* w1t_frag, const dbx_view* y, const dbx_view* gate, void* stream);
+int dbx_head2_backward_up_heads(int32_t dtype, const dbx_view* d_out, const dbx_view* hid, const float* const* w2, const int32_t* k,
+                                int32_t nh, const dbx_view* d_hid, const uint8_t* dropmask, int32_t dropmask_ld, int32_t use_hash,
+                                uint32_t drop_seed, float* const* dw, float* const* db, void* scratch, const dbx_view* d_g44,
+                                uint32_t head_mask, const int32_t* rows, int32_t rows_capacity, void* stream);
+int dbx_heads_sparse_ok(int32_t dtype, const dbx_view* hid, const dbx_view* d_g44);
+int64_t dbx_heads_sparse_ws_bytes(int32_t n, int32_t h, int32_t w, int32_t capacity, int32_t ns);
+int dbx_heads_sparse_backward2(int32_t dtype, const dbx_view* d_out, const dbx_view* hid, const float* const* w2, const int32_t* k,
+                               int32_t nh, uint32_t head_mask, int32_t use_hash, uint32_t drop_seed, const dbx_view* d_g44, int32_t capacity, void* ws, int32_t* map, const int32_t* prev_map, void* stream);
 
 int dbx_fold_heads(const float* w2, const float* b2, const float* w1, const float* b1, int32_t k, float* w_out,
                    float* b_out, void* stream);
```

Result: no change. 7690 patches/s (-0.2%).
